# mlelarge/graph_neural_net

Measured on AMD Instinct MI355X. Metric: graph-pairs/sec FGNN fwd+bwd, N=50 regular pairs, higher is better.
Workload: dtype f32

## Files before the change

graph_neural_net_amd/_lib.py:

```python
import ctypes as C
import os

import torch

_HERE = os.path.dirname(os.path.abspath(__file__))
LIB_PATH = os.environ.get('FGNN_LIB') or os.path.join(_HERE, 'libfgnn_hip.so')

FGNN_H = 32
FGNN_TILE = 32
FGNN_MAX_DEPTH = 3
FGNN_RANGE_WG = 256
FGNN_LSAP_MAX_N = 2048
FGNN_MAX_LEVELS = 64
FGNN_QAP_MAX_N = 256
FGNN_QAPW_MAX_N = 256
FGNN_SPECTRAL_MAX_N = 256
FGNN_SPECTRAL_MAX_POWERS = 8
FGNN_PLANTED_MAX_N = 256
FGNN_SCORE_SPLIT = 4

c_float_p = C.c_void_p


class Slab(C.Structure):
    _fields_ = [('ptr', C.c_void_p), ('gstride', C.c_longlong), ('ldp', C.c_longlong), ('C', C.c_int),
                ('nrm', C.c_void_p), ('beta', C.c_void_p)]


class MlpFwdArgs(C.Structure):
    _fields_ = [('G', C.c_int), ('N', C.c_int), ('depth', C.c_int), ('nmlp', C.c_int),
                ('nvalid', C.c_void_p),
                ('a', Slab), ('b', Slab),
                ('W', (C.c_void_p * FGNN_MAX_DEPTH) * 2),
                ('bias', (C.c_void_p * FGNN_MAX_DEPTH) * 2),
                ('z', C.c_void_p * 2),
                ('ldz', C.c_longlong),
                ('part', C.c_void_p * 2),
                ('cnt', C.c_void_p), ('packed', C.c_void_p), ('xbits', C.c_void_p), ('xdeg', C.c_void_p),
                ('ranges', C.c_void_p), ('cu_share', C.c_int)]


class DwJob(C.Structure):
    _fields_ = [('dy', C.c_void_p), ('d_gstride', C.c_longlong), ('d_ld', C.c_longlong), ('relu_mask', C.c_void_p),
                ('x', C.c_void_p), ('x_gstride', C.c_longlong), ('x_ld', C.c_longlong), ('M', C.c_int), ('K', C.c_int)]


class ChainLayer(C.Structure):
    _fields_ = [('W', C.c_void_p), ('w_ostride', C.c_longlong), ('w_kstride', C.c_longlong), ('bias', C.c_void_p),
                ('M', C.c_int), ('K', C.c_int), ('relu', C.c_int), ('mask', C.c_void_p), ('out', C.c_void_p),
                ('o_gstride', C.c_longlong)]


class ChainArgs(C.Structure):
    _fields_ = [('x', C.c_void_p), ('x_gstride', C.c_longlong), ('x_ld', C.c_longlong), ('depth', C.c_int),
                ('layer', ChainLayer * 3), ('o_ld', C.c_longlong), ('nvalid', C.c_void_p), ('G', C.c_int), ('N', C.c_int)]


class Mlp64Args(C.Structure):
    _fields_ = [('x', C.c_void_p), ('x_gstride', C.c_longlong), ('x_ld', C.c_longlong), ('cin', C.c_int),
                ('xb', C.c_void_p), ('xb_gstride', C.c_longlong), ('xb_ld', C.c_longlong), ('cb', C.c_int),
                ('packed', C.c_void_p), ('nvalid', C.c_void_p), ('G', C.c_int), ('N', C.c_int),
                ('out', C.c_void_p), ('o_gstride', C.c_longlong), ('o_ld', C.c_longlong),
                ('dz', C.c_void_p), ('dz_gstride', C.c_longlong), ('dz_ld', C.c_longlong),
                ('dx', C.c_void_p), ('dx_gstride', C.c_longlong), ('dx_ld', C.c_longlong),
                ('dxb', C.c_void_p), ('dxb_gstride', C.c_longlong), ('dxb_ld', C.c_longlong),
                ('accumulate_dx', C.c_int), ('accumulate_dxb', C.c_int),
                ('wpart', C.c_void_p)]


class Mlp64PackJob(C.Structure):
    _fields_ = [('W', C.c_void_p * 3), ('bias', C.c_void_p * 3), ('cin', C.c_int), ('packed', C.c_void_p)]


class MlpBwdArgs(C.Structure):
    _fields_ = [('G', C.c_int), ('N', C.c_int), ('depth', C.c_int),
                ('nvalid', C.c_void_p),
                ('a', Slab), ('b', Slab),
                ('W', C.c_void_p * FGNN_MAX_DEPTH),
                ('bias', C.c_void_p * FGNN_MAX_DEPTH),
                ('dy', C.c_void_p), ('dgstride', C.c_longlong), ('ldd', C.c_longlong),
                ('z', C.c_void_p), ('zgstride', C.c_longlong), ('ldz', C.c_longlong),
                ('coef', C.c_void_p), ('s12', C.c_void_p), ('znrm', C.c_void_p),
                ('dxa', C.c_void_p), ('dxa_gstride', C.c_longlong), ('dxa_ld', C.c_longlong),
                ('dxb', C.c_void_p), ('dxb_gstride', C.c_longlong), ('dxb_ld', C.c_longlong),
                ('accumulate_a', C.c_int), ('accumulate_b', C.c_int),
                ('wpart', C.c_void_p), ('s12part', C.c_void_p), ('packed', C.c_void_p),
                ('s12tiles', C.c_void_p), ('s12_out', C.c_void_p), ('xbits', C.c_void_p), ('xdeg', C.c_void_p),
                ('ranges', C.c_void_p), ('cu_share', C.c_int)]


class Slab16(C.Structure):
    _fields_ = [('ptr', C.c_void_p), ('gstride', C.c_longlong), ('ldp', C.c_longlong), ('C', C.c_int),
                ('nrm', C.c_void_p), ('beta', C.c_void_p)]


class MlpFwd16Args(C.Structure):
    _fields_ = [('G', C.c_int), ('N', C.c_int), ('ldr', C.c_int), ('depth', C.c_int), ('nmlp', C.c_int),
                ('nvalid', C.c_void_p),
                ('a', Slab16), ('b', Slab16),
                ('z', C.c_void_p * 2), ('ldz', C.c_longlong),
                ('part', C.c_void_p * 2), ('cnt', C.c_void_p), ('packed', C.c_void_p), ('ranges', C.c_void_p)]


class MlpBwd16Args(C.Structure):
    _fields_ = [('G', C.c_int), ('N', C.c_int), ('ldr', C.c_int), ('depth', C.c_int),
                ('nvalid', C.c_void_p),
                ('a', Slab16), ('b', Slab16),
                ('dy', C.c_void_p), ('dgstride', C.c_longlong), ('ldd', C.c_longlong),
                ('z', C.c_void_p), ('zgstride', C.c_longlong), ('ldz', C.c_longlong),
                ('coef', C.c_void_p),
                ('dxa', C.c_void_p), ('dxa_gstride', C.c_longlong), ('dxa_ld', C.c_longlong),
                ('dxb', C.c_void_p), ('dxb_gstride', C.c_longlong), ('dxb_ld', C.c_longlong),
                ('accumulate_a', C.c_int), ('accumulate_b', C.c_int),
                ('wpart', C.c_void_p), ('s12part', C.c_void_p), ('packed', C.c_void_p), ('ranges', C.c_void_p)]


class GradJob(C.Structure):
    _fields_ = [('wpart', C.c_void_p), ('count', C.c_int), ('out', C.c_void_p), ('s12', C.c_void_p),
                ('nrm', C.c_void_p), ('dgn_w', C.c_void_p), ('dgn_b', C.c_void_p), ('rows', C.c_int), ('scale', C.c_float), ('scale_dev', C.c_void_p)]


class PackJob(C.Structure):
    _fields_ = [('kind', C.c_int), ('ca', C.c_int), ('cb', C.c_int), ('depth', C.c_int), ('nmlp', C.c_int),
                ('W', (C.c_void_p * FGNN_MAX_DEPTH) * 2), ('bias', (C.c_void_p * FGNN_MAX_DEPTH) * 2),
                ('out', C.c_void_p)]


class PairgenArgs(C.Structure):
    _fields_ = [('seed', C.c_ulonglong), ('first', C.c_longlong), ('B', C.c_int), ('N', C.c_int),
                ('family', C.c_int), ('noise_model', C.c_int), ('edge_density', C.c_double),
                ('thr_edge', C.c_ulonglong), ('thr_noise1', C.c_ulonglong), ('thr_noise2', C.c_ulonglong),
                ('thr_vertex', C.c_ulonglong), ('swaps_per_edge', C.c_int),
                ('bits1', C.c_void_p), ('bits2', C.c_void_p), ('nvalid', C.c_void_p)]


FGNN_GUARD_MAX_PARTS = 64
FGNN_GUARD_SKIP_NONFINITE = 1
FGNN_GUARD_NONFINITE = 1


class GuardRecord(C.Structure):
    _fields_ = [('max_norm', C.c_double), ('norm', C.c_double), ('coef', C.c_double),
                ('flags', C.c_int), ('skipped', C.c_int), ('arrivals', C.c_int), ('mode', C.c_int),
                ('partial', C.c_double * FGNN_GUARD_MAX_PARTS)]


class EvalRecord(C.Structure):
    _fields_ = [('ce_sum', C.c_double), ('nodes', C.c_longlong), ('correct_lsap', C.c_longlong), ('correct_max', C.c_longlong),
                ('pairs', C.c_longlong), ('steps', C.c_longlong)]


MAX_GRAD_JOBS = 16
MAX_PACK_JOBS = 24
_VP, _LL, _I, _F = C.c_void_p, C.c_longlong, C.c_int, C.c_float

_SIGNATURES = {
    'fgnn_last_error': [],
    'fgnn_version': [],
    'fgnn_tiles_per_graph': [_I],
    'fgnn_mlp_bwd_num_workgroups': [],
    'fgnn_pack_floats': [_I, _I, _I, _I, _I],
    'fgnn_pack_operands': [_VP, _I, _VP],
    'fgnn_mlp_fwd': [C.POINTER(MlpFwdArgs), _VP],
    'fgnn_pack_x3_floats': [_I, _I, _I, _I, _I],
    'fgnn_pack_x3_operands': [_VP, _I, _VP],
    'fgnn_mlp_fwd_x3': [C.POINTER(MlpFwdArgs), _VP],
    'fgnn_debug_mlp_fwd_masks': [C.POINTER(MlpFwdArgs), _VP, _VP, _VP],
    'fgnn_debug_mlp_fwd_x3_masks': [C.POINTER(MlpFwdArgs), _VP, _VP, _VP],
    'fgnn_debug_matmul_variant': [_I],
    'fgnn_gn_finalize': [_VP, _VP, _VP, _VP, _I, _I, _I, _F, _VP, _VP],
    'fgnn_gn_finalize2': [_VP, _VP, _VP, _VP, _VP, _VP, _I, _I, _I, _F, _VP, _VP, _VP],
    'fgnn_gn_plane_supported': [_I],
    'fgnn_gn_plane_fwd': [_VP, _LL, _LL, _VP, _VP, _VP, _I, _I, _I, _F, _VP, _LL, _LL, _VP, _VP],
    'fgnn_gn_plane_bwd': [_VP, _LL, _LL, _VP, _LL, _LL, _VP, _VP, _I, _I, _I, _VP, _LL, _LL, _VP, _VP, _VP, _VP],
    'fgnn_gn_stats': [_VP, _LL, _LL, _VP, _VP, _I, _I, _I, _F, _VP, _VP],
    'fgnn_gn_apply': [_VP, _LL, _LL, _VP, _VP, _VP, _I, _I, _I, _VP, _LL, _LL, _VP],
    'fgnn_ragged_tile_ranges': [_VP, _I, _I, _VP, _VP],
    'fgnn_ragged_tile_ranges_order': [_VP, _I, _I, _VP, _VP, _VP],
    'fgnn_ragged_tile_ranges16': [_VP, _I, _I, _I, _VP, _VP],
    'fgnn_conv1x1_dw_multi': [C.POINTER(DwJob), _I, _VP, _I, _I, _VP, _VP],
    'fgnn_conv_chain_supported': [_I, _I, C.POINTER(C.c_int)],
    'fgnn_conv_chain': [C.POINTER(ChainArgs), _VP],
    'fgnn_mlp64_supported': [_I, _I, _I],
    'fgnn_mlp64_num_workgroups': [],
    'fgnn_mlp64_param_count': [_I],
    'fgnn_mlp64_packed_floats': [_I],
    'fgnn_mlp64_pack': [_VP, _VP, _VP, _VP, _VP, _VP, _I, _VP, _VP],
    'fgnn_mlp64_pack_multi': [C.POINTER(Mlp64PackJob), _I, _VP],
    'fgnn_mlp64_fwd': [C.POINTER(Mlp64Args), _VP],
    'fgnn_mlp64_bwd': [C.POINTER(Mlp64Args), _VP],
    'fgnn_conv1x1': [_VP, _LL, _LL, _VP, _VP, _LL, _LL, _VP, _I, _VP, _I, _I, _I, _I, _VP, _LL, _LL, _VP],
    'fgnn_conv1x1_dw_chunks': [_I, _I],
    'fgnn_conv1x1_dw': [_VP, _LL, _LL, _VP, _VP, _LL, _LL, _VP, _I, _I, _I, _I, _VP, _VP],
    'fgnn_chan_matmul_fwd': [C.POINTER(Slab), C.POINTER(Slab), _VP, _I, _I, _VP, _LL, _LL, _VP],
    'fgnn_chan_matmul_fwd_ord': [C.POINTER(Slab), C.POINTER(Slab), _VP, _I, _I, _VP, _LL, _LL, _VP, _I, _VP],
    'fgnn_chan_matmul_fwd_fin_supported': [_I],
    'fgnn_chan_matmul_fwd_fin': [C.POINTER(Slab), C.POINTER(Slab), _VP, _VP, _VP, _VP, _VP, _F, _VP, _I, _I, _VP, _LL, _LL, _VP],
    'fgnn_chan_matmul_fwd_fin_ord': [C.POINTER(Slab), C.POINTER(Slab), _VP, _VP, _VP, _VP, _VP, _F, _VP, _I, _I, _VP, _LL, _LL, _VP, _I, _VP],
    'fgnn_colmax_fwd': [C.POINTER(Slab), _VP, _I, _I, _VP, _VP, _VP],
    'fgnn_colmax_fwd_fin_supported': [_I],
    'fgnn_colmax_fwd_fin': [C.POINTER(Slab), _VP, _VP, _VP, _F, _VP, _I, _I, _VP, _VP, _VP],
    'fgnn_score_ce_fwd': [_VP, _VP, _VP, _I, _I, _I, _VP, _VP, _VP, _VP],
    'fgnn_score_row_blocks': [_I, _I],
    'fgnn_score_ce_fwd_blocks': [_VP, _VP, _VP, _I, _I, _I, _I, _VP, _VP, _VP, _VP],
    'fgnn_score_ce_bwd': [_VP, _VP, _VP, _VP, _VP, _VP, _I, _I, _I, _VP, _VP, _VP],
    'fgnn_score_ce_fwd_blocks_labels': [_VP, _VP, _VP, _VP, _I, _I, _I, _I, _VP, _VP, _VP, _VP],
    'fgnn_score_ce_bwd_labels': [_VP, _VP, _VP, _VP, _VP, _VP, _VP, _I, _I, _I, _VP, _VP, _VP],
    'fgnn_ce_fwd_labels': [_VP, _VP, _VP, _I, _I, _VP, _VP, _VP],
    'fgnn_ce_bwd_labels': [_VP, _VP, _VP, _VP, _VP, _I, _I, _VP, _VP],
    'fgnn_inv_node_count': [_VP, _I, _VP, _VP],
    'fgnn_score_bwd': [_VP, _VP, _VP, _VP, _I, _I, _I, _VP, _VP, _VP],
    'fgnn_ce_fwd': [_VP, _VP, _I, _I, _VP, _VP, _VP],
    'fgnn_ce_bwd': [_VP, _VP, _VP, _VP, _I, _I, _VP, _VP],
    'fgnn_colmax_bwd': [_VP, _VP, _VP, _I, _I, _I, _VP, _LL, _LL, C.POINTER(Slab), _VP, _VP],
    'fgnn_gn_bwd_stats': [_VP, _LL, _LL, _VP, _LL, _LL, _VP, _VP, _I, _I, _I, _VP, _VP],
    'fgnn_gn_bwd_coef': [_VP, _VP, _VP, _I, _I, _I, _VP, _VP, _VP, _VP],
    'fgnn_gn_bwd_coef_tiles': [_VP, _VP, _VP, _I, _I, _I, _VP, _VP, _VP],
    'fgnn_grad_finalize': [_VP, _I, _I, _I, _I, _VP],
    'fgnn_gn_bwd_apply': [_VP, _LL, _LL, _VP, _LL, _LL, _VP, _VP, _I, _I, _I, _VP, _LL, _LL, _VP],
    'fgnn_mlp_bwd': [C.POINTER(MlpBwdArgs), _VP],
    'fgnn_mlp_bwd_x3': [C.POINTER(MlpBwdArgs), _VP],
    'fgnn_mlp_bwd_pair': [C.POINTER(MlpBwdArgs), C.POINTER(MlpBwdArgs), _VP],
    'fgnn_mlp_bwd_t16': [C.POINTER(MlpBwdArgs), _VP],
    'fgnn_mlp_bwd_t16_supported': [C.POINTER(MlpBwdArgs)],
    'fgnn_mlp_bwd_pair_t16': [C.POINTER(MlpBwdArgs), C.POINTER(MlpBwdArgs), _VP],
    'fgnn_mlp_bwd_pair_x3': [C.POINTER(MlpBwdArgs), C.POINTER(MlpBwdArgs), _VP],
    'fgnn_block1_struct_supported': [_I, _I, _I],
    'fgnn_block1_struct_table_floats': [_I],
    'fgnn_block1_struct_ws_floats': [_I, _I],
    'fgnn_block1_struct_rows': [_I, _I],
    'fgnn_block1_struct_fwd': [_VP, _VP, _I, _I, _VP, _VP, _VP, _VP, _VP, C.c_float, _VP, _VP, _VP, _LL, _LL, _VP, _VP, _VP, _VP, _VP, _VP, _VP],
    'fgnn_block1_struct_bwd': [_VP, _VP, _I, _I, _VP, _VP, _VP, _VP, _VP, _VP, _VP, _VP, _LL, _LL, _VP, _VP, _VP, _VP, _VP, _VP],
    'fgnn_block1_struct_fwd_pack': [_VP, _VP, _I, _I, _VP, _VP, _VP, _VP, _VP, C.c_float, _VP, _VP, _VP, _LL, _LL, _VP, _VP, _VP, _VP, _VP, _VP, _VP, _I, _VP],
    'fgnn_block1_struct_fwd16_pack': [_VP, _VP, _I, _I, _I, _VP, _VP, _VP, _VP, _VP, C.c_float, _VP, _VP, _VP, _LL, _LL, _VP, _VP, _VP, _VP, _VP, _VP, _VP, _I, _VP],
    'fgnn_block1_struct_fwd16': [_VP, _VP, _I, _I, _I, _VP, _VP, _VP, _VP, _VP, C.c_float, _VP, _VP, _VP, _LL, _LL, _VP, _VP, _VP, _VP, _VP, _VP, _VP],
    'fgnn_block1_struct_bwd16': [_VP, _VP, _I, _I, _I, _VP, _VP, _VP, _VP, _VP, _VP, _VP, _VP, _LL, _LL, _VP, _VP, _VP, _VP, _VP, _VP],
    'fgnn_mlp_bwd_coef_tiles_supported': [_I, _I],
    'fgnn_mlp_param_count': [_I, _I],
    'fgnn_reduce_partials': [_VP, _I, _I, _VP, _VP],
    'fgnn_chan_matmul_bwd': [C.POINTER(Slab), C.POINTER(Slab), _VP, _LL, _LL, _VP, _I, _I, _VP, _VP, _LL, _LL, _VP, _VP, _VP],
    'fgnn_chan_matmul_bwd_ord': [C.POINTER(Slab), C.POINTER(Slab), _VP, _LL, _LL, _VP, _I, _I, _VP, _VP, _LL, _LL, _VP, _VP, _VP, _I, _VP],
    'fgnn_sum_scale': [_VP, _I, _I, _F, _VP, _VP],
    'fgnn_adam_step': [_VP, _VP, _VP, _VP, _I, C.c_double, C.c_double, C.c_double, C.c_double, _I, C.c_double, _VP],
    'fgnn_adam_step_dev': [_VP, _VP, _VP, _VP, _I, _VP, _VP, _VP],
    'fgnn_grad_guard': [_VP, _I, _VP, _VP, _VP],
    'fgnn_adam_step_guarded': [_VP, _VP, _VP, _VP, _I, _VP, _VP, _VP, _VP],
    'fgnn_expand_adjacency': [_VP, _VP, _I, _I, _VP, _VP],
    'fgnn_pack_adjacency': [_VP, _VP, _I, _I, _VP, _VP, _VP],
    'fgnn_pack_adjacency_ld': [_VP, _VP, _I, _I, _I, _VP, _VP, _VP],
    'fgnn_pack_adjacency_pair': [_VP, _VP, _VP, _VP, _I, _I, _I, _VP, _VP, _VP, _VP, _VP],
    'fgnn_adjacency_degree': [_VP, _VP, _I, _I, _VP, _VP],
    'fgnn_accuracy_max': [_VP, _VP, _I, _I, _VP, _VP],
    'fgnn_lsap_accuracy': [_VP, _LL, _I, _VP, _I, _I, _VP, _VP, _VP],
    'fgnn_pairgen_supported': [_I, _I, _I],
    'fgnn_pairgen': [C.POINTER(PairgenArgs), _VP],
    'fgnn_pairgen_indexed': [C.POINTER(PairgenArgs), _VP, _VP],
    'fgnn_pairgen_levels': [C.POINTER(PairgenArgs), _VP, _VP, _I, _VP, _VP],
    'fgnn_epoch_index': [C.c_ulonglong, C.c_ulonglong, _LL, _LL, _LL, _VP, _VP],
    'fgnn_qap_objective': [_VP, _VP, _VP, _VP, _I, _I, _VP, _VP, _VP, _VP, _VP],
    'fgnn_qap_improve_cost': [_VP, _VP, _VP, _VP, _I, _I, _VP, _LL, _I, _VP],
    'fgnn_greedy_qap_ws_bytes': [_I, _I],
    'fgnn_greedy_qap': [_VP, _VP, _VP, _VP, _I, _I, _I, _VP, _LL, _VP, _VP, _VP, _VP, _VP],
    'fgnn_greedy_qap_labels': [_VP, _VP, _VP, _VP, _VP, _I, _I, _I, _VP, _LL, _VP, _VP, _VP, _VP, _VP],
    'fgnn_qapw_objective': [_VP, _VP, _LL, _I, _VP, _VP, _I, _I, _VP, _VP, _VP, _VP, _VP, _VP],
    'fgnn_qapw_improve_cost': [_VP, _VP, _LL, _I, _VP, _VP, _I, _I, _VP, _LL, _I, _VP],
    'fgnn_greedy_qapw_ws_bytes': [_I, _I],
    'fgnn_greedy_qapw': [_VP, _VP, _LL, _I, _VP, _VP, _I, _I, _I, _VP, _LL, _VP, _VP, _VP, _VP, _VP],
    'fgnn_greedy_qapw_labels': [_VP, _VP, _LL, _I, _VP, _VP, _VP, _I, _I, _I, _VP, _LL, _VP, _VP, _VP, _VP, _VP],
    'fgnn_planted_perm': [C.c_ulonglong, _LL, _VP, _VP, _I, _I, _VP, _VP],
    'fgnn_relabel_bits': [_VP, _VP, _VP, _I, _I, _VP, _VP],
    'fgnn_relabel_dense': [_VP, _VP, _VP, _I, _I, _I, _I, _VP, _VP],
    'fgnn_count_matches': [_VP, _VP, _VP, _I, _I, _VP, _VP],
    'fgnn_accuracy_max_labels': [_VP, _VP, _VP, _I, _I, _VP, _VP],
    'fgnn_spectral_features': [_VP, _VP, _I, _I, _I, _VP, _I, _VP],
    'fgnn_eval_pairs': [_VP, _VP, _VP, _I, _I, _VP, _LL, _I, _VP, _VP, _VP],
    'fgnn_eval_pairs_labels': [_VP, _VP, _VP, _I, _I, _VP, _LL, _I, _VP, _VP, _VP],
    'fgnn_eval_fold': [_VP, _VP, _VP, _VP, _I, _I, _I, _VP, _VP, _VP, _VP],
    'fgnn_eval_fold_bins': [_VP, _VP, _VP, _VP, _I, _I, _I, _VP, _I, _VP, _VP, _VP, _VP],
    'fgnn_tiles_per_graph16': [_I, _I],
    'fgnn_to_bf16': [_VP, _VP, _I, _I, _I, _I, _VP, _LL, _LL, _VP],
    'fgnn_from_bf16': [_VP, _LL, _LL, _I, _I, _I, _I, _VP, _VP],
    'fgnn_to_bf16_pad': [_VP, _VP, _I, _I, _I, _I, _I, _VP, _LL, _VP],
    'fgnn_pack16_floats': [_I, _I, _I, _I, _I],
    'fgnn_pack16_operands': [_VP, _I, _VP],
    'fgnn_mlp_fwd16': [C.POINTER(MlpFwd16Args), _VP],
    'fgnn_debug_mlp_fwd16_masks': [C.POINTER(MlpFwd16Args), _VP, _VP, _VP],
    'fgnn_gn_finalize_tpg': [_VP, _VP, _VP, _VP, _I, _I, _I, _I, _F, _VP, _VP],
    'fgnn_gn_finalize2_tpg': [_VP, _VP, _VP, _VP, _VP, _VP, _I, _I, _I, _I, _F, _VP, _VP, _VP],
    'fgnn_gn_bwd_coef_tiles_tpg': [_VP, _VP, _VP, _I, _I, _I, _I, _VP, _VP, _VP],
    'fgnn_chan_matmul_fwd16': [C.POINTER(Slab16), C.POINTER(Slab16), _VP, _I, _I, _I, _VP, _LL, _LL, _VP],
    'fgnn_chan_matmul_fwd16_fin': [C.POINTER(Slab16), C.POINTER(Slab16), _VP, _VP, _VP, _VP, _VP, _F, _I, _VP, _I, _I, _I, _VP, _LL,
                                   _LL, _VP],
    'fgnn_chan_matmul_bwd16': [C.POINTER(Slab16), C.POINTER(Slab16), _VP, _LL, _LL, _VP, _I, _I, _I, _VP, _VP, _LL, _LL, _VP, _VP, _VP],
    'fgnn_chan_matmul_bwd16_t': [C.POINTER(Slab16), C.POINTER(Slab16), _VP, _LL, _LL, _VP, _I, _VP, _I, _I, _I, _VP, _VP, _LL, _LL,
                                 _VP, _VP, _VP],
    'fgnn_chan_matmul_bwd16_tc': [C.POINTER(Slab16), C.POINTER(Slab16), _VP, _LL, _LL, _VP, _I, _VP, _I, _I, _I, _VP, _VP, _LL, _LL,
                                  _VP, _VP, _VP, _VP, _VP],
    'fgnn_colmax_bwd16_coef': [_VP, _VP, _VP, _I, _I, _I, _I, _VP, _LL, _LL, C.POINTER(Slab16), _VP, _VP, _VP],
    'fgnn_colmax_fwd16': [C.POINTER(Slab16), _VP, _I, _I, _I, _VP, _VP, _VP],
    'fgnn_colmax_bwd16': [_VP, _VP, _VP, _I, _I, _I, _I, _VP, _LL, _LL, C.POINTER(Slab16), _VP, _VP],
    'fgnn_mlp_bwd16': [C.POINTER(MlpBwd16Args), _VP],
    'fgnn_mlp_bwd16_pair': [C.POINTER(MlpBwd16Args), C.POINTER(MlpBwd16Args), _VP],
}
_RESTYPES = {'fgnn_last_error': C.c_char_p, 'fgnn_block1_struct_ws_floats': C.c_longlong, 'fgnn_greedy_qap_ws_bytes': C.c_longlong,
             'fgnn_greedy_qapw_ws_bytes': C.c_longlong}
EXPORTS = tuple(_SIGNATURES)

_lib = None


def load(allow_missing=False):
    global _lib
    if _lib is not None:
        return _lib
    if not os.path.exists(LIB_PATH):
        raise RuntimeError(
            'graph_neural_net_amd: %s is missing. Build it with '
            '`python -c "import __graft_entry__ as g; g.build()"` or `make -C graph_neural_net_amd/csrc`. '
            'There is no CPU fallback.' % LIB_PATH)
    lib = C.CDLL(LIB_PATH)
    for name, argtypes in _SIGNATURES.items():
        if allow_missing and not hasattr(lib, name):
            continue
        fn = getattr(lib, name)
        fn.argtypes = argtypes
        fn.restype = _RESTYPES.get(name, C.c_int)
    _lib = lib
    return lib


def last_error():
    return load().fgnn_last_error().decode('utf-8', 'replace')


PROFILE = None


def call(name, *args, tag=None):
    if PROFILE is not None:
        e0 = torch.cuda.Event(enable_timing=True)
        e1 = torch.cuda.Event(enable_timing=True)
        e0.record()
        rc = getattr(load(), name)(*args)
        e1.record()
        PROFILE.append((tag or name, e0, e1, name, args))
    else:
        rc = getattr(load(), name)(*args)
    if rc != 0:
        raise RuntimeError('%s failed (rc=%d): %s' % (name, rc, last_error()))


def relaunch(name, args):
    rc = getattr(load(), name)(*args[:-1], stream_ptr())
    if rc != 0:
        raise RuntimeError('%s failed (rc=%d): %s' % (name, rc, last_error()))


def stream_ptr():
    return C.c_void_p(torch.cuda.current_stream().cuda_stream)


def ptr(t):
    if t is None:
        return None
    if not t.is_cuda:
        raise RuntimeError('graph_neural_net_amd: expected a CUDA/HIP tensor, got device %s '
                           '(there is no CPU path)' % (t.device,))
    return C.c_void_p(t.data_ptr())


def make_slab(t, gstride, ldp, channels, nrm=None, beta=None):
    s = Slab()
    s.ptr = t.data_ptr() if t is not None else None
    s.gstride = gstride
    s.ldp = ldp
    s.C = channels
    s.nrm = nrm.data_ptr() if nrm is not None else None
    s.beta = beta.data_ptr() if beta is not None else None
    return s


def make_slab16(t, gstride, ldp, channels, nrm=None, beta=None):
    s = Slab16()
    s.ptr = t.data_ptr() if t is not None else None
    s.gstride = gstride
    s.ldp = ldp
    s.C = channels
    s.nrm = nrm.data_ptr() if nrm is not None else None
    s.beta = beta if isinstance(beta, int) else (beta.data_ptr() if beta is not None else None)
    return s


def tiles_per_graph(n):
    return (n * n + FGNN_TILE - 1) // FGNN_TILE
# ... 5 lines not shown
```

graph_neural_net_amd/csrc/fgnn_bwd32.h:

```cpp
#pragma once
#include "fgnn_common.h"

namespace {

constexpr int BWD_WG = 256;
constexpr int NW = 8;
constexpr int NP = 4;
static_assert(BWD_WG == FGNN_RANGE_WG, "fgnn_ragged_tile_ranges splits for the backward grid");

DEVI float4 coef_from_sums(const float4 n, const float2 sv, float nv) {
    const float m = nv * nv;
    float4 k;
    k.x = n.x;
    k.y = n.y;
    k.z = m > 0.f ? -n.y * sv.y * n.w / m : 0.f;
    k.w = m > 0.f ? -n.y * sv.x / m : 0.f;
    return k;
}
DEVI float4 coef_record(const fgnn_mlp_bwd_args &A, int g, int ch, int nv) {
    if (A.coef) return reinterpret_cast<const float4 *>(A.coef)[(long long)g * FGNN_H + ch];
    const float4 n = reinterpret_cast<const float4 *>(A.znrm)[(long long)g * FGNN_H + ch];
    const float2 sv = reinterpret_cast<const float2 *>(A.s12)[(long long)g * FGNN_H + ch];
    return coef_from_sums(n, sv, (float)nv);
}
DEVI float4 coef_record(const fgnn_mlp_bwd_args &A, int g, int ch) {
    if (A.coef) return reinterpret_cast<const float4 *>(A.coef)[(long long)g * FGNN_H + ch];
    const float4 n = reinterpret_cast<const float4 *>(A.znrm)[(long long)g * FGNN_H + ch];
    const float2 sv = reinterpret_cast<const float2 *>(A.s12)[(long long)g * FGNN_H + ch];
    return coef_from_sums(n, sv, (float)nvalid_of(A.nvalid, g, A.N));
}


struct PairArgs {
    fgnn_mlp_bwd_args m[2];
};

template <int PCOUNT, int NWV>
DEVI void sum_wave_partials(const float *smem, float *wpart) {
    static_assert(PCOUNT % 4 == 0, "partials are summed four at a time");
    float4 *out = reinterpret_cast<float4 *>(wpart + (long long)blockIdx.x * PCOUNT);
    const float4 *part4 = reinterpret_cast<const float4 *>(smem);
    for (int e = threadIdx.x; e < PCOUNT / 4; e += 64 * NWV) {
        float4 a = part4[e];
#pragma unroll
        for (int w = 1; w < NWV; ++w) {
            const float4 b = part4[w * (PCOUNT / 4) + e];
            a.x += b.x;
            a.y += b.y;
            a.z += b.z;
            a.w += b.w;
        }
        out[e] = a;
    }
}
template <int PCOUNT>
DEVI void sum_pair_partials(const float *smem, const PairArgs &P) {
    static_assert(PCOUNT % 4 == 0, "partials are summed four at a time");
    const float4 *part4 = reinterpret_cast<const float4 *>(smem);
    for (int e = threadIdx.x; e < 2 * (PCOUNT / 4); e += 64 * NW) {
        const int m = e >= PCOUNT / 4 ? 1 : 0, ee = e - m * (PCOUNT / 4);
        float4 a = part4[(4 * m) * (PCOUNT / 4) + ee];
#pragma unroll
        for (int w = 1; w < NP; ++w) {
            const float4 b = part4[(4 * m + w) * (PCOUNT / 4) + ee];
            a.x += b.x;
            a.y += b.y;
            a.z += b.z;
            a.w += b.w;
        }
        reinterpret_cast<float4 *>(P.m[m].wpart + (long long)blockIdx.x * PCOUNT)[ee] = a;
    }
}

inline int check_mlp_bwd_common(const fgnn_mlp_bwd_args *a, const char *fn, int tile_bits) {
    FGNN_CHECK(a->dy && a->z && a->wpart, "%s: missing dy/z/wpart", fn);
    FGNN_CHECK(a->coef || (a->s12 && a->znrm) || (a->s12tiles && a->znrm), "%s: need coef, or s12 + znrm, or s12tiles + znrm", fn);
    const long long lim = 0x7fffffffll / 4, G = a->G;
    FGNN_CHECK(G * a->a.gstride < lim && G * a->b.gstride < lim && G * a->dgstride < lim && G * a->zgstride < lim &&
               G * a->dxa_gstride < lim && G * a->dxb_gstride < lim,
               "%s: a tensor exceeds 2 GiB (32-bit buffer addressing); split the batch", fn);
    FGNN_CHECK(G * fgnn_tiles_per_graph(a->N) < (1ll << tile_bits), "%s: too many tiles", fn);
    FGNN_CHECK(BWD_WG == fgnn_mlp_bwd_num_workgroups(), "%s: workgroup count differs from fgnn_mlp_bwd", fn);
    return 0;
}
inline int check_pair_common(const fgnn_mlp_bwd_args *a1, const fgnn_mlp_bwd_args *a2, const char *fn, int tile_bits, bool dense_only) {
    FGNN_CHECK(a1 && a2, "%s: null args", fn);
    FGNN_CHECK(BWD_WG == fgnn_mlp_bwd_num_workgroups(), "%s: workgroup count differs from fgnn_mlp_bwd", fn);
    FGNN_CHECK(a1->G > 0 && a1->N > 0 && a1->G == a2->G && a1->N == a2->N && a1->depth == a2->depth,
               "%s: the two MLPs must share G, N and depth", fn);
    FGNN_CHECK((!dense_only || a1->a.ptr) && a1->a.ptr == a2->a.ptr && a1->a.C == a2->a.C && a1->a.gstride == a2->a.gstride &&
               a1->a.ldp == a2->a.ldp && a1->a.nrm == a2->a.nrm && a1->a.beta == a2->a.beta &&
               (dense_only || (a1->xbits == a2->xbits && a1->xdeg == a2->xdeg)) && a1->nvalid == a2->nvalid,
               "%s: the two MLPs must read the same input slab", fn);
    FGNN_CHECK(!a1->dxa && !a1->s12part, "%s: the input gradient and its tile sums belong to the SECOND argument block", fn);
    FGNN_CHECK(!a1->s12tiles && !a2->s12tiles, "%s: s12tiles is an mlp3 feature", fn);
    for (const fgnn_mlp_bwd_args *a : {a1, a2}) {
        FGNN_CHECK(a->dy && a->z && a->wpart, "%s: missing dy/z/wpart", fn);
        FGNN_CHECK(a->coef || (a->s12 && a->znrm), "%s: need coef, or s12 + znrm", fn);
        const long long lim = 0x7fffffffll / 4, G = a->G;
        FGNN_CHECK(G * a->a.gstride < lim && G * a->dgstride < lim && G * a->zgstride < lim && G * a->dxa_gstride < lim,
                   "%s: a tensor exceeds 2 GiB (32-bit buffer addressing); split the batch", fn);
    }
    FGNN_CHECK((long long)a1->G * fgnn_tiles_per_graph(a1->N) < (1ll << tile_bits), "%s: too many tiles", fn);
    return 0;
}

}
```

graph_neural_net_amd/csrc/fgnn_bwd_t16.h:

```cpp
#pragma once
#include "fgnn_t16.h"
#include "fgnn_pack.h"
#include "fgnn_bwd32.h"

namespace {

using namespace t16;

template <int CB, int IMAGES, int NSLOTS>
struct BwdT16Layout {
    static constexpr int DEPTH = 3;
    static constexpr PkBwd PK = pk_bwd(32, CB, DEPTH);
    static constexpr int OFF_W1 = PK.off_wh, OFF_WT1 = PK.off_wt, OFF_WT2 = PK.off_wt + 16;
    static constexpr int BIAS_F = PK.bias_f;
    static constexpr int WEIGHT_F = pk_pad_floats(PK.floats);
    static constexpr int NSLOT = NSLOTS;
    static constexpr int CIN = 32 + CB;
    static constexpr int PCOUNT = 32 * CIN + 32 + (DEPTH - 1) * (32 * 32 + 32);
    static constexpr int TILE_OFF = IMAGES * WEIGHT_F;
    static constexpr int TILE_END = TILE_OFF + NW * NSLOT * TILE_F;
    static constexpr int RED_F = NW * PCOUNT;
};


#define FGNN_T16_READ_RECORDS(norm)                                 \
    _Pragma("unroll") for (int s = 0; s < 8; ++s) {                 \
        const float4 k4 = rec[chan_s(s) + chan_q(q)];               \
        kx[s] = k4.x;                                               \
        ky[s] = k4.y;                                               \
        kz[s] = k4.z;                                               \
        kw[s] = k4.w;                                               \
        if (norm) {                                                 \
            const float4 n = rec[32 + chan_s(s) + chan_q(q)];       \
            mean[s] = n.x;                                          \
            av[s] = n.y;                                            \
        }                                                           \
    }

#define FGNN_T16_RECOMPUTE_HIDDEN(acc, h1, h2)                                              \
    _Pragma("unroll") for (int s = 0; s < 8; ++s) h1[s] = relu1(acc[s >> 2][s & 3]);        \
    stage8(S0, lane_base, h1);                                                              \
    load_bias(acc, wl + L::BIAS_F, 1, q);                                                   \
    gemm32<L::OFF_W1>(acc, wl, h1, lane);                                                   \
    _Pragma("unroll") for (int s = 0; s < 8; ++s) h2[s] = relu1(acc[s >> 2][s & 3]);        \
    stage8(S1, lane_base, h2);

#define FGNN_T16_DZ(dpre)                                                                                                   \
    _Pragma("unroll") for (int s = 0; s < 8; ++s) dpre[s] = fmaf(kz[s], zr[s] - kx[s], fmaf(ky[s], dyr[s], kw[s]));         \
    if (!full) {                                                                                                            \
        _Pragma("unroll") for (int s = 0; s < 8; ++s) dpre[s] = valid ? dpre[s] : 0.f;                                      \
    }

#define FGNN_T16_HIDDEN_BWD(OFF_WT, dpre, dW, db, Dt, In, h)                                                \
    {                                                                                                       \
        f32x4 a2[2];                                                                                        \
        a2[0] = a2[1] = zero4();                                                                            \
        gemm32<OFF_WT>(a2, wl, dpre, lane);                                                                 \
        wgrad16(dW, db, Dt, In, lane);                                                                      \
        _Pragma("unroll") for (int s = 0; s < 8; ++s) dpre[s] = h[s] > 0.f ? a2[s >> 2][s & 3] : 0.f;       \
    }

#define FGNN_T16_DB_BUTTERFLY(db0, db1, db2)            \
    _Pragma("unroll") for (int b = 0; b < 2; ++b) {     \
        db0[b] += __shfl_xor(db0[b], 16);               \
        db0[b] += __shfl_xor(db0[b], 32);               \
        db1[b] += __shfl_xor(db1[b], 16);               \
        db1[b] += __shfl_xor(db1[b], 32);               \
        db2[b] += __shfl_xor(db2[b], 16);               \
        db2[b] += __shfl_xor(db2[b], 32);               \
    }

}
```

graph_neural_net_amd/csrc/fgnn_norm.h:

```cpp
#pragma once
#include "fgnn_common.h"

DEVI float4 nrm_record(float mean, float m2, float m, float nv, float w, float eps) {
    const float var = m > 0.f ? m2 / m : 0.f;
    const float ve = var + eps;
    const float q = nv > 0.f ? 1.f / (2.f * sqrtf(nv * ve)) : 0.f;
    float4 o;
    o.x = mean;
    o.y = w * q;
    o.z = q;
    o.w = 1.f / ve;
    return o;
}

struct TilePartials {
    float nb[4], mb[4], qb[4];
};
DEVI TilePartials finalize_load(const float *part, const float *cnt, int g, int c, int C, int tpg, int lane, bool tr = false) {
    TilePartials p;
    const int ts = tr ? 1 : C, cs = tr ? tpg : 1;
#pragma unroll
    for (int k = 0; k < 4; ++k) {
        const int t = lane + WAVE * k;
        const bool ok = t < tpg;
        const int tc = ok ? t : 0;
        const float n = cnt[(long long)g * tpg + tc];
        const float2 pm = reinterpret_cast<const float2 *>(part)[(long long)g * tpg * C + (long long)tc * ts + (long long)c * cs];
        p.nb[k] = ok ? n : 0.f;
        p.mb[k] = pm.x;
        p.qb[k] = ok ? pm.y : 0.f;
    }
    return p;
}
DEVI float4 finalize_reduce(const TilePartials &p, float nv, float w, float eps) {
    float sn = 0.f, sm = 0.f;
#pragma unroll
    for (int k = 0; k < 4; ++k) {
        sn += p.nb[k];
        sm += p.nb[k] * p.mb[k];
    }
    sn = wave_sum(sn);
    sm = wave_sum(sm);
    const float mean = sn > 0.f ? sm / sn : 0.f;
    float m2 = 0.f;
#pragma unroll
    for (int k = 0; k < 4; ++k) {
        const float d = p.mb[k] - mean;
        m2 += p.qb[k] + p.nb[k] * d * d;
    }
    m2 = wave_sum(m2);
    return nrm_record(mean, m2, sn, nv, w, eps);
}

struct NormRec {
    float mean, a, beta;
    bool on;
};
DEVI NormRec norm_of(const fgnn_slab &s, int g, int c) {
    NormRec r;
    r.on = s.nrm != nullptr;
    if (r.on) {
        const float4 n = reinterpret_cast<const float4 *>(s.nrm)[(long long)g * s.C + c];
        r.mean = n.x;
        r.a = n.y;
        r.beta = s.beta ? s.beta[c] : 0.f;
    } else {
        r.mean = 0.f;
        r.a = 1.f;
        r.beta = 0.f;
    }
    return r;
}
DEVI NormRec norm_from(const float4 &n, const fgnn_slab &s, int c) {
    NormRec r;
    r.on = true;
    r.mean = n.x;
    r.a = n.y;
    r.beta = s.beta ? s.beta[c] : 0.f;
    return r;
}

DEVI float4 finalize_wave(const float *part, const float *cnt, int g, int c, int C, int tpg, float nv, float w, float eps,
                          int lane, bool tr = false) {
    return finalize_reduce(finalize_load(part, cnt, g, c, C, tpg, lane, tr), nv, w, eps);
}
DEVI float4 finalize_wave_any(const float *part, const float *cnt, int g, int c, int C, int tpg, float nv, float w, float eps, int lane,
                              bool tr = false) {
    if (tpg <= 4 * WAVE) return finalize_wave(part, cnt, g, c, C, tpg, nv, w, eps, lane, tr);
    constexpr int U = 8;
    float sn = 0.f, sm = 0.f;
    const float *cg = cnt + (long long)g * tpg;
    const int ts = tr ? 1 : C;
    const float2 *pg = reinterpret_cast<const float2 *>(part) + (long long)g * tpg * C + (long long)c * (tr ? tpg : 1);
    for (int t0 = lane; t0 < tpg; t0 += U * WAVE) {
        float n[U], x[U];
#pragma unroll
        for (int k = 0; k < U; ++k) {
            const int t = t0 + k * WAVE, tc = t < tpg ? t : 0;
            n[k] = t < tpg ? cg[tc] : 0.f;
            x[k] = pg[(long long)tc * ts].x;
        }
#pragma unroll
        for (int k = 0; k < U; ++k) {
            sn += n[k];
            sm += n[k] * x[k];
        }
    }
    sn = wave_sum(sn);
    sm = wave_sum(sm);
    const float mean = sn > 0.f ? sm / sn : 0.f;
    float m2 = 0.f;
    for (int t0 = lane; t0 < tpg; t0 += U * WAVE) {
        float n[U];
        float2 pm[U];
#pragma unroll
        for (int k = 0; k < U; ++k) {
            const int t = t0 + k * WAVE, tc = t < tpg ? t : 0;
            n[k] = t < tpg ? cg[tc] : 0.f;
            pm[k] = pg[(long long)tc * ts];
            if (t >= tpg) pm[k].y = 0.f;
        }
#pragma unroll
        for (int k = 0; k < U; ++k) {
            const float d = pm[k].x - mean;
            m2 += pm[k].y + n[k] * d * d;
        }
    }
    m2 = wave_sum(m2);
    return nrm_record(mean, m2, sn, nv, w, eps);
}
```

graph_neural_net_amd/csrc/matmul.hip:

```cpp
#include "fgnn_common.h"
#include "fgnn_norm.h"

namespace {

constexpr int TM = 64;
constexpr int LDS_LD = 65;

DEVI void stage_tile(float *lds, const float *mat, int N, int nv, int row0, int col0, const NormRec &nr, int tid) {
    if (row0 == 0 && col0 == 0 && N <= TM) {
        for (int e = tid; e < TM * TM; e += 256) lds[(e >> 6) * LDS_LD + (e & 63)] = 0.f;
        __syncthreads();
        const int P = N * N;
        for (int e = tid; e < P; e += 256) {
            const int r = e / N, c = e - r * N;
            float v = mat[e];
            const bool ok = r < nv && c < nv;
            v = ok ? (nr.on ? (v - nr.mean) * nr.a + nr.beta : v) : 0.f;
            lds[r * LDS_LD + c] = v;
        }
    } else {
        for (int e = tid; e < TM * TM; e += 256) {
            const int r = e >> 6, c = e & 63;
            const int gr = row0 + r, gc = col0 + c;
            float v = 0.f;
// ... 50 lines not shown
    const int qi = wave >> 1, qj = wave & 1;
    const int j = lane & 31, h = lane >> 5;
    const float *A = ya.ptr + (long long)g * ya.gstride + (long long)c * ya.ldp;
    const float *B = yb.ptr + (long long)g * yb.gstride + (long long)c * yb.ldp;
    const NormRec na = norm_of(ya, g, c), nb = norm_of(yb, g, c);
    float *O = out + (long long)g * ogstride + (long long)c * ldo;

    f32x16 acc;
#pragma unroll
    for (int r = 0; r < 16; ++r) acc[r] = 0.f;
    const bool live = (row0 + 32 * qi < N) && (col0 + 32 * qj < N);

    for (int k0 = 0; k0 < N; k0 += TM) {
        if (k0) __syncthreads();
        stage_tile(As, A, N, nv, row0, k0, na, tid);
        stage_tile(Bs, B, N, nv, k0, col0, nb, tid);
        __syncthreads();
        if (live) {
            const int kmax = (N - k0 < TM ? N - k0 : TM);
            const float *ap = As + (32 * qi + j) * LDS_LD + h;
            const float *bp = Bs + h * LDS_LD + 32 * qj + j;
            for (int k = 0; k < kmax; k += 2) acc = mfma32(ap[k], bp[k * LDS_LD], acc);
        }
    }
    if (live) store_quadrant(O, N, row0 + 32 * qi, col0 + 32 * qj, acc, lane);
}

__global__ __launch_bounds__(256) void chan_matmul_bwd_kernel(const fgnn_slab ya, const fgnn_slab yb,
                                                              const float *dm, long long dmg, long long ldm,
                                                              const int *nvalid, int N, float *da, float *db,
                                                              long long ogstride, long long ldo, float *s12a,
                                                              float *s12b) {
    __shared__ float Xs[TM * LDS_LD];
    __shared__ float Ds[TM * LDS_LD];
    __shared__ float red[4][4];
    const int C = ya.C;
    const int gc = blockIdx.z;
    const int g = gc / C, c = gc - g * C;
    const int nv = nvalid_of(nvalid, g, N);
    const int row0 = blockIdx.y * TM, col0 = blockIdx.x * TM;
    const int tid = threadIdx.x, lane = tid & 63, wave = tid >> 6;
    const int qi = wave >> 1, qj = wave & 1;
    const int j = lane & 31, h = lane >> 5;
    const float *A = ya.ptr + (long long)g * ya.gstride + (long long)c * ya.ldp;
    const float *B = yb.ptr + (long long)g * yb.gstride + (long long)c * yb.ldp;
    const float *D = dm + (long long)g * dmg + (long long)c * ldm;
    const NormRec na = norm_of(ya, g, c), nb = norm_of(yb, g, c);
    NormRec none;
    none.on = false; none.mean = 0.f; none.a = 1.f; none.beta = 0.f;
    float *OA = da + (long long)g * ogstride + (long long)c * ldo;
    float *OB = db + (long long)g * ogstride + (long long)c * ldo;
    const bool live = (row0 + 32 * qi < N) && (col0 + 32 * qj < N);

    f32x16 acc;
#pragma unroll
    for (int r = 0; r < 16; ++r) acc[r] = 0.f;
    for (int j0 = 0; j0 < N; j0 += TM) {
        if (j0) __syncthreads();
        stage_tile(Ds, D, N, nv, row0, j0, none, tid);
        stage_tile(Xs, B, N, nv, col0, j0, nb, tid);
        __syncthreads();
        if (live) {
            const int kmax = (N - j0 < TM ? N - j0 : TM);
            const float *ap = Ds + (32 * qi + j) * LDS_LD + h;
            const float *bp = Xs + (32 * qj + j) * LDS_LD + h;
            for (int k = 0; k < kmax; k += 2) acc = mfma32(ap[k], bp[k], acc);
        }
    }
    if (live) store_quadrant(OA, N, row0 + 32 * qi, col0 + 32 * qj, acc, lane);
    float sa1 = 0.f, sa2 = 0.f, sb1 = 0.f, sb2 = 0.f;
    if (s12a && live) {
        const int col = col0 + 32 * qj + j;
#pragma unroll
        for (int r = 0; r < 16; ++r) {
            const int row = row0 + 32 * qi + ch_of(r, h);
            if (row < nv && col < nv) {
                sa1 += acc[r];
                sa2 += acc[r] * (A[(long long)row * N + col] - na.mean);
            }
        }
    }

#pragma unroll
    for (int r = 0; r < 16; ++r) acc[r] = 0.f;
    for (int i0 = 0; i0 < N; i0 += TM) {
        __syncthreads();
        stage_tile(Xs, A, N, nv, i0, row0, na, tid);
        stage_tile(Ds, D, N, nv, i0, col0, none, tid);
        __syncthreads();
        if (live) {
            const int kmax = (N - i0 < TM ? N - i0 : TM);
            const float *ap = Xs + h * LDS_LD + 32 * qi + j;
            const float *bp = Ds + h * LDS_LD + 32 * qj + j;
            for (int k = 0; k < kmax; k += 2) acc = mfma32(ap[k * LDS_LD], bp[k * LDS_LD], acc);
        }
    }
    if (live) store_quadrant(OB, N, row0 + 32 * qi, col0 + 32 * qj, acc, lane);
    if (s12a) {
        if (live) {
            const int col = col0 + 32 * qj + j;
#pragma unroll
            for (int r = 0; r < 16; ++r) {
                const int row = row0 + 32 * qi + ch_of(r, h);
                if (row < nv && col < nv) {
                    sb1 += acc[r];
                    sb2 += acc[r] * (B[(long long)row * N + col] - nb.mean);
                }
            }
        }
        s12_epilogue(red, sa1, sa2, sb1, sb2, s12a, s12b, gc, tid);
    }
}

template <bool WANT_U>
DEVI void load_tile_regs(float (&v)[16], float (&u)[16], const float *mat, int N, int nv, const NormRec &nr, int tid) {
#pragma unroll
    for (int k = 0; k < 16; ++k) {
        const int e = tid + 256 * k;
        const int r = e >> 6, c = e & 63;
        const bool ok = r < nv && c < nv;
        const float x = mat[ok ? r * N + c : 0];
        const float d = x - nr.mean;
        v[k] = ok ? (nr.on ? d * nr.a + nr.beta : x) : 0.f;
        if (WANT_U) u[k] = ok ? d : 0.f;
    }
}
DEVI void store_tile_lds(float *lds, const float (&v)[16], int tid) {
#pragma unroll
    for (int k = 0; k < 16; ++k) {
        const int e = tid + 256 * k;
        lds[(e >> 6) * LDS_LD + (e & 63)] = v[k];
    }
}
DEVI void frag_to_lds(float *lds, int row0, int col0, const f32x16 &acc, int lane) {
    const int j = lane & 31, h = lane >> 5;
#pragma unroll
    for (int r = 0; r < 16; ++r) lds[(row0 + ch_of(r, h)) * LDS_LD + col0 + j] = acc[r];
}
template <bool WANT_S>
DEVI void tile_to_global(const View &ov, int mat_off4, const float *lds, int N, const float (&u)[16], float &s1,
                         float &s2, int tid) {
    const int c = tid & 63, r0 = __builtin_amdgcn_readfirstlane(tid >> 6);
    const int voff = c < N ? (r0 * N + c) * 4 : OOB_OFF;
    const float *lp = lds + r0 * LDS_LD + c;
#pragma unroll
    for (int k = 0; k < 16; ++k) {
        const float t = lp[4 * k * LDS_LD];
        buf_store(t, ov, r0 + 4 * k < N ? voff : OOB_OFF, mat_off4 + k * 16 * N);
        if (WANT_S) {
            s1 += t;
            s2 += t * u[k];
        }
    }
}

DEVI void load_tile_raw(float (&x)[16], const View &v, int mat_off4, int N, int nv, int tid) {
    const int c = tid & 63, r0 = __builtin_amdgcn_readfirstlane(tid >> 6);
    const int voff = c < nv ? (r0 * N + c) * 4 : OOB_OFF;
#pragma unroll
    for (int k = 0; k < 16; ++k) {
        const int r = r0 + 4 * k;
        x[k] = buf_load(v, r < nv ? voff : OOB_OFF, mat_off4 + k * 16 * N);
    }
}
template <bool WANT_U>
DEVI void finish_tile(float (&v)[16], float (&u)[16], const float (&x)[16], int nv, const NormRec &nr, int tid) {
#pragma unroll
    for (int k = 0; k < 16; ++k) {
        const int e = tid + 256 * k;
        const int r = e >> 6, c = e & 63;
        const bool ok = r < nv && c < nv;
        const float d = x[k] - nr.mean;
        v[k] = ok ? (nr.on ? d * nr.a + nr.beta : x[k]) : 0.f;
        if (WANT_U) u[k] = ok ? d : 0.f;
    }
}

struct FinArgs {
    const float *part_a, *part_b, *cnt, *gw_a, *gw_b;
    float *nrm_a, *nrm_b;
    float eps;
    int tpg;
};
template <bool FIN>
__global__ __launch_bounds__(256, 4) void chan_matmul_fwd1_kernel(const fgnn_slab ya, const fgnn_slab yb,
                                                               const int *nvalid, int N, int M, float *out,
                                                               long long ogstride, long long ldo, const FinArgs F) {
    __shared__ float As[TM * LDS_LD];
    __shared__ float Bs[TM * LDS_LD];
    __shared__ float4 fin_rec[2];
    const int C = ya.C;
    const int tid = threadIdx.x, lane = tid & 63, wave = tid >> 6;
    const int qi = wave >> 1, qj = wave & 1;
    const int j = lane & 31, h = lane >> 5;
    float xa[16], xb[16], dummy[16];
    const int G = M / C;
    const View vA = make_view(ya.ptr, ya.gstride, ya.ldp, G), vB = make_view(yb.ptr, yb.gstride, yb.ldp, G);
    const View vO = make_view(out, ogstride, ldo, G);
    const int gc = blockIdx.x;
    {
        const int g = gc / C, c = gc - g * C;
        const int nv = nvalid_of(nvalid, g, N);
        TilePartials tp;
        if (FIN && wave < 2) tp = finalize_load(wave ? F.part_b : F.part_a, F.cnt, g, c, C, F.tpg, lane);
        load_tile_raw(xa, vA, g * vA.gs4 + c * vA.ld4, N, nv, tid);
        load_tile_raw(xb, vB, g * vB.gs4 + c * vB.ld4, N, nv, tid);
        NormRec na, nb;
        if (FIN) {
            if (wave < 2) {
                const float4 r = finalize_reduce(tp, (float)nv, (wave ? F.gw_b : F.gw_a) ? (wave ? F.gw_b : F.gw_a)[c] : 1.f, F.eps);
                if (lane == 0) {
                    fin_rec[wave] = r;
                    reinterpret_cast<float4 *>(wave ? F.nrm_b : F.nrm_a)[gc] = r;
                }
            }
            __syncthreads();
            const float4 ra = fin_rec[0], rb = fin_rec[1];
            na = norm_from(ra, ya, c);
            nb = norm_from(rb, yb, c);
        } else {
            na = norm_of(ya, g, c);
            nb = norm_of(yb, g, c);
        }
        const int o_off = g * vO.gs4 + c * vO.ld4;
        {
            float va[16], vb[16];
            finish_tile<false>(va, dummy, xa, nv, na, tid);
            finish_tile<false>(vb, dummy, xb, nv, nb, tid);
            store_tile_lds(As, va, tid);
            store_tile_lds(Bs, vb, tid);
        }
        __syncthreads();
        f32x16 acc;
#pragma unroll
        for (int r = 0; r < 16; ++r) acc[r] = 0.f;
        if (32 * qi < N && 32 * qj < N) {
            const float *ap = As + (32 * qi + j) * LDS_LD + h;
            const float *bp = Bs + h * LDS_LD + 32 * qj + j;
            for (int k = 0; k < N; k += 2) acc = mfma32(ap[k], bp[k * LDS_LD], acc);
        }
        __syncthreads();
        frag_to_lds(As, 32 * qi, 32 * qj, acc, lane);
        __syncthreads();
        float s1 = 0.f, s2 = 0.f;
        tile_to_global<false>(vO, o_off, As, N, dummy, s1, s2, tid);
    }
}

__global__ __launch_bounds__(256, 4) void chan_matmul_bwd1_kernel(const fgnn_slab ya, const fgnn_slab yb,
                                                               const float *dm, long long dmg, long long ldm,
                                                               const int *nvalid, int N, int M, float *da, float *db,
                                                               long long ogstride, long long ldo, float *s12a,
                                                               float *s12b) {
    __shared__ float Bs[TM * LDS_LD];
    __shared__ float Ds[TM * LDS_LD];
    __shared__ float red[4][4];
    const int C = ya.C;
    const int tid = threadIdx.x, lane = tid & 63, wave = tid >> 6;
    const int qi = wave >> 1, qj = wave & 1;
    const int j = lane & 31, h = lane >> 5;
    NormRec none;
    none.on = false; none.mean = 0.f; none.a = 1.f; none.beta = 0.f;
    float xa[16], xb[16], xd[16], dummy[16];
    const int G = M / C;
    const View vA = make_view(ya.ptr, ya.gstride, ya.ldp, G), vB = make_view(yb.ptr, yb.gstride, yb.ldp, G);
    const View vD = make_view(dm, dmg, ldm, G);
    const View vOA = make_view(da, ogstride, ldo, G), vOB = make_view(db, ogstride, ldo, G);
    const int gc = blockIdx.x;
    {
        const int g = gc / C, c = gc - g * C;
        const int nv = nvalid_of(nvalid, g, N);
        load_tile_raw(xa, vA, g * vA.gs4 + c * vA.ld4, N, nv, tid);
        load_tile_raw(xb, vB, g * vB.gs4 + c * vB.ld4, N, nv, tid);
        load_tile_raw(xd, vD, g * vD.gs4 + c * vD.ld4, N, nv, tid);
        const NormRec na = norm_of(ya, g, c), nb = norm_of(yb, g, c);
        const int o_off = g * vOA.gs4 + c * vOA.ld4;
        float ua[16], ub[16], va[16];
        finish_tile<true>(va, ua, xa, nv, na, tid);
        {
            float vb[16], vd[16];
            finish_tile<true>(vb, ub, xb, nv, nb, tid);
            finish_tile<false>(vd, dummy, xd, nv, none, tid);
            store_tile_lds(Bs, vb, tid);
            store_tile_lds(Ds, vd, tid);
        }
        __syncthreads();
        const bool live = 32 * qi < N && 32 * qj < N;
        f32x16 accA, accB;
#pragma unroll
        for (int r = 0; r < 16; ++r) {
            accA[r] = 0.f;
            accB[r] = 0.f;
        }
        if (live) {
            const float *ap = Ds + (32 * qi + j) * LDS_LD + h;
            const float *bp = Bs + (32 * qj + j) * LDS_LD + h;
            for (int k = 0; k < N; k += 2) accA = mfma32(ap[k], bp[k], accA);
        }
        __syncthreads();
        store_tile_lds(Bs, va, tid);
        __syncthreads();
        if (live) {
            const float *ap = Bs + h * LDS_LD + 32 * qi + j;
            const float *bp = Ds + h * LDS_LD + 32 * qj + j;
            for (int k = 0; k < N; k += 2) accB = mfma32(ap[k * LDS_LD], bp[k * LDS_LD], accB);
        }
        __syncthreads();
        frag_to_lds(Ds, 32 * qi, 32 * qj, accA, lane);
        frag_to_lds(Bs, 32 * qi, 32 * qj, accB, lane);
        __syncthreads();
        float sa1 = 0.f, sa2 = 0.f, sb1 = 0.f, sb2 = 0.f;
        if (s12a) {
            tile_to_global<true>(vOA, o_off, Ds, N, ua, sa1, sa2, tid);
            tile_to_global<true>(vOB, o_off, Bs, N, ub, sb1, sb2, tid);
            s12_epilogue(red, sa1, sa2, sb1, sb2, s12a, s12b, gc, tid);
        } else {
            tile_to_global<false>(vOA, o_off, Ds, N, dummy, sa1, sa2, tid);
            tile_to_global<false>(vOB, o_off, Bs, N, dummy, sb1, sb2, tid);
        }
    }
}


int g_mm_wave_variant = 1;
inline bool mm_wave_variant() { return (g_mm_wave_variant & 1) != 0; }
inline bool mm_narrow() { return (g_mm_wave_variant & 8) != 0; }
constexpr int WLD = 68;
constexpr int W_WAVES = 2;

DEVI rsrc_t mat_rsrc(const float *p, int bytes) {
    return __builtin_amdgcn_make_buffer_rsrc(const_cast<float *>(p), 0, bytes, 0x00020000);
}
DEVI float rsrc_load(rsrc_t r, int voff, int soff) {
    return __builtin_bit_cast(float, __builtin_amdgcn_raw_buffer_load_b32(r, voff, soff, 0));
}
DEVI void rsrc_store(float x, rsrc_t r, int voff, int soff) {
    __builtin_amdgcn_raw_buffer_store_b32(__builtin_bit_cast(unsigned, x), r, voff, soff, 0);
}
DEVI float2 rsrc_load2(rsrc_t r, int voff, int soff) {
    typedef unsigned u2 __attribute__((ext_vector_type(2)));
    const u2 v = __builtin_amdgcn_raw_buffer_load_b64(r, voff, soff, 0);
    const unsigned a = v.x, b = v.y;
    return make_float2(__builtin_bit_cast(float, a), __builtin_bit_cast(float, b));
}
DEVI void rsrc_store2(float x, float y, rsrc_t r, int voff, int soff) {
    typedef unsigned u2 __attribute__((ext_vector_type(2)));
    u2 v;
    v.x = __builtin_bit_cast(unsigned, x);
    v.y = __builtin_bit_cast(unsigned, y);
    __builtin_amdgcn_raw_buffer_store_b64(v, r, voff, soff, 0);
}

#define FGNN_W_CONTEXT(LDS_FLOATS)                                                                                       \
    __shared__ __attribute__((aligned(16))) float lds[W_WAVES * (LDS_FLOATS)];                                           \
    const int lane = threadIdx.x & 63, wv = __builtin_amdgcn_readfirstlane(threadIdx.x >> 6);                            \
    const int gc = xcd_swizzle(blockIdx.x, gridDim.x) * W_WAVES + wv;                                                    \
    if (gc >= M) return;                                                                                                 \
    const int C = ya.C;                                                                                                  \
    const int g = gc / C, c = gc - g * C;                                                                                \
    const int nv = __builtin_amdgcn_readfirstlane(nvalid_of(nvalid, g, N));                                              \
    const int j = lane & 31, h = lane >> 5;                                                                              \
    float *As = lds + wv * (LDS_FLOATS);                                                                                 \
    const rsrc_t rA = mat_rsrc(ya.ptr + (long long)g * ya.gstride + (long long)c * ya.ldp, nv * N * 4);                  \
    const rsrc_t rB = mat_rsrc(yb.ptr + (long long)g * yb.gstride + (long long)c * yb.ldp, nv * N * 4);                  \
    const rsrc_t rO = mat_rsrc(out + (long long)g * ogstride + (long long)c * ldo, N * N * 4);
#define FGNN_W_PRODUCTS(NB_, BVAL)                                                                                       \
    f32x16 acc[NB_][NB_];                                                                                                \
    _Pragma("unroll") for (int rb = 0; rb < NB_; ++rb)                                                                   \
        _Pragma("unroll") for (int cb = 0; cb < NB_; ++cb)                                                               \
            _Pragma("unroll") for (int r = 0; r < 16; ++r) acc[rb][cb][r] = 0.f;                                         \
    _Pragma("unroll") for (int q = 0; q < KQ; ++q) {                                                                     \
        float4 af[NB_];                                                                                                  \
        _Pragma("unroll") for (int rb = 0; rb < NB_; ++rb)                                                               \
            af[rb] = *reinterpret_cast<const float4 *>(As + (32 * rb + j) * WLD + h * 32 + 4 * q);                       \
        _Pragma("unroll") for (int t = 0; t < 4; ++t) {                                                                  \
            const int s = 4 * q + t;                                                                                     \
            if (q == KQ - 1 && 2 * s >= N) break;                                                                        \
            float bv[NB_];                                                                                               \
            BVAL                                                                                                         \
            _Pragma("unroll") for (int rb = 0; rb < NB_; ++rb) {                                                         \
                const float a = t == 0 ? af[rb].x : (t == 1 ? af[rb].y : (t == 2 ? af[rb].z : af[rb].w));               \
                _Pragma("unroll") for (int cb = 0; cb < NB_; ++cb) acc[rb][cb] = mfma32(a, bv[cb], acc[rb][cb]);         \
            }                                                                                                            \
        }                                                                                                                \
    }
#define FGNN_W_RECORDS                                                                                                   \
    float meanA, aA, meanB, aB;                                                                                          \
    if (FIN) {                                                                                                           \
        const float4 ra = finalize_reduce(ta, (float)nv, F.gw_a ? F.gw_a[c] : 1.f, F.eps);                               \
        const float4 rb = finalize_reduce(tb, (float)nv, F.gw_b ? F.gw_b[c] : 1.f, F.eps);                               \
        if (lane == 0) {                                                                                                 \
            reinterpret_cast<float4 *>(F.nrm_a)[gc] = ra;                                                                \
            reinterpret_cast<float4 *>(F.nrm_b)[gc] = rb;                                                                \
        }                                                                                                                \
        meanA = ra.x; aA = ra.y; meanB = rb.x; aB = rb.y;                                                                \
    } else {                                                                                                             \
        const NormRec na = norm_of(ya, g, c), nb = norm_of(yb, g, c);                                                    \
        meanA = na.mean; aA = na.a; meanB = nb.mean; aB = nb.a;                                                          \
    }                                                                                                                    \
    const bool onA = FIN || ya.nrm != nullptr, onB = FIN || yb.nrm != nullptr;                                           \
    const float betaA = (onA && ya.beta) ? ya.beta[c] : 0.f, betaB = (onB && yb.beta) ? yb.beta[c] : 0.f;
DEVI constexpr int wave_row_off(int rb, int r, int N) { return (32 * rb + (r & 3) + 8 * (r >> 2)) * N * 4; }

template <int KQ>
DEVI void wave_rows_load(float (&x)[8 * KQ], rsrc_t r, int N, int voff) {
#pragma unroll
    for (int i = 0; i < 8 * KQ; ++i) x[i] = rsrc_load(r, voff, i < N ? i * N * 4 : 0);
}
template <int KQ>
DEVI void wave_rows_stage(float *T, const float (&x)[8 * KQ], float mean, float a_eff, float b_eff, int nv, int N, int lane) {
    if (nv < N) {
#pragma unroll
        for (int i = 0; i < 8 * KQ; ++i) {
            const float v = (x[i] - mean) * a_eff + b_eff;
            T[i * WLD + lane] = i < nv ? v : 0.f;
        }
    } else {
#pragma unroll
        for (int i = 0; i < 8 * KQ; ++i) T[i * WLD + lane] = (x[i] - mean) * a_eff + b_eff;
    }
}

template <int KQ, bool FIN>
__global__ __launch_bounds__(64 * W_WAVES, 2) void chan_matmul_fwd_w_kernel(const fgnn_slab ya, const fgnn_slab yb,
                                                                           const int *nvalid, int N, int M, float *out,
                                                                           long long ogstride, long long ldo,
                                                                           const FinArgs F) {
    constexpr int KH = 4 * KQ;
    constexpr bool TWO = KQ > 4;
    constexpr int NB = TWO ? 2 : 1;
    FGNN_W_CONTEXT(32 * NB * WLD)

    TilePartials ta, tb;
    if (FIN) {
        ta = finalize_load(F.part_a, F.cnt, g, c, C, F.tpg, lane);
        tb = finalize_load(F.part_b, F.cnt, g, c, C, F.tpg, lane);
    }
    float xa[8 * KQ], xb[NB][KH];
    wave_rows_load<KQ>(xa, rA, N, lane < nv ? lane * 4 : OOB_OFF);
    int voffB[NB];
#pragma unroll
    for (int cb = 0; cb < NB; ++cb) {
        const int col = 32 * cb + j;
        voffB[cb] = col < nv ? (h * N + col) * 4 : OOB_OFF;
    }
#pragma unroll
    for (int s = 0; s < KH; ++s)
#pragma unroll
        for (int cb = 0; cb < NB; ++cb) xb[cb][s] = rsrc_load(rB, voffB[cb] + s * 2 * N * 4, 0);
    FGNN_W_RECORDS
    {
        const bool okc = lane < nv;
        wave_rows_stage<KQ>(As, xa, meanA, okc ? aA : 0.f, okc ? betaA : 0.f, nv, N, (lane & 1) * 32 + (lane >> 1));
    }
    float aeB[NB], beB[NB];
#pragma unroll
    for (int cb = 0; cb < NB; ++cb) {
        const bool okc = 32 * cb + j < nv;
        aeB[cb] = okc ? aB : 0.f;
        beB[cb] = okc ? betaB : 0.f;
    }
    FGNN_W_PRODUCTS(NB, _Pragma("unroll") for (int cb = 0; cb < NB; ++cb) bv[cb] = (xb[cb][s] - meanB) * aeB[cb] + beB[cb];)
#pragma unroll
    for (int cb = 0; cb < NB; ++cb) {
        const int col = 32 * cb + j;
// ... 378 lines not shown
    const BigSrc D = big_src_plain(dm, dmg, ldm, G, g, c);
    const View vOA = make_view(da, ogstride, ldo, G), vOB = make_view(db, ogstride, ldo, G);
    const int o_off = g * vOA.gs4 + c * vOA.ld4;
    if (do_a) big_zero_fill(vOA, o_off, N, nv, 32 * ntv, tid, fill != 0);
    if (do_b) big_zero_fill(vOB, o_off, N, nv, 32 * ntv, tid, fill != 0);
    float sa1 = 0.f, sa2 = 0.f, sb1 = 0.f, sb2 = 0.f;
    if (ntv > 0) {
        f32x16 acc[BigCfg<NT>::MAXT];
        if (do_a) {
            big_gemm<NT, true, true>(acc, D, B, big_lds, N, nv, ntv, tid);
            if (s12a) big_store<NT, true>(acc, vOA, o_off, A, N, nv, ntv, sa1, sa2, tid);
            else big_store<NT, false>(acc, vOA, o_off, A, N, nv, ntv, sa1, sa2, tid);
        }
        if (do_b) {
            big_gemm<NT, false, false>(acc, A, D, big_lds, N, nv, ntv, tid);
            if (s12a) big_store<NT, true>(acc, vOB, o_off, B, N, nv, ntv, sb1, sb2, tid);
            else big_store<NT, false>(acc, vOB, o_off, B, N, nv, ntv, sb1, sb2, tid);
        }
    }
    if (s12a) {
        sa1 = wave_sum(sa1);
        sa2 = wave_sum(sa2);
        sb1 = wave_sum(sb1);
        sb2 = wave_sum(sb2);
        if (lane == 0) {
            red[wv][0] = sa1;
            red[wv][1] = sa2;
            red[wv][2] = sb1;
            red[wv][3] = sb2;
        }
        __syncthreads();
        if (tid < 4 && (tid < 2 ? do_a : do_b)) {
            float v = 0.f;
#pragma unroll
            for (int w = 0; w < BIG_NW; ++w) v += red[w][tid];
            float *dst = (tid < 2 ? s12a : s12b) + (long long)gc * 2 + (tid & 1);
            *dst = v;
        }
    }
}

inline bool big_path(int N) { return N > TM && N <= 256; }

}

template <int MT, bool FIN>
static void launch_fwd_big(const fgnn_slab *ya, const fgnn_slab *yb, const int *nvalid, int N, int G, float *out, long long ogstride,
                           long long ldo, const int *order, const FinArgs &F, int fill, hipStream_t st) {
    static LdsAttrCache attr_cache;
    (void)fgnn_raise_lds(attr_cache, (const void *)chan_matmul_fwd_big_kernel<MT, FIN>, BigCfg<MT>::LDS_BYTES);
    hipLaunchKernelGGL((chan_matmul_fwd_big_kernel<MT, FIN>), dim3(G * ya->C), dim3(BIG_THREADS), BigCfg<MT>::LDS_BYTES, st, *ya, *yb, nvalid, N, G, out,
                       ogstride, ldo, order, F, fill);
}

static int check_2gib(const char *name, int G, long long s0, long long s1, long long s2 = 0, long long s3 = 0) {
    FGNN_CHECK((long long)G * s0 < 0x7fffffffll / 4 && (long long)G * s1 < 0x7fffffffll / 4 && (long long)G * s2 < 0x7fffffffll / 4 &&
               (long long)G * s3 < 0x7fffffffll / 4,
               "%s: a tensor exceeds 2 GiB (32-bit buffer addressing); split the batch", name);
    return 0;
}

template <bool FIN>
static int chan_matmul_fwd_dispatch(const char *name, const fgnn_slab *ya, const fgnn_slab *yb, const int *nvalid, int G, int N,
                                    float *out, long long ogstride, long long ldo, const int *order, int fill, const FinArgs &F,
                                    hipStream_t st) {
    const int M = G * ya->C;
    if (FIN || big_path(N)) {
        if (check_2gib(name, G, ya->gstride, yb->gstride, ogstride)) return 1;
    } else if (N <= TM) {
        if (check_2gib(name, G, ya->gstride, yb->gstride)) return 1;
        FGNN_CHECK((long long)G * ogstride < 0x7fffffffll / 4, "%s: output exceeds 2 GiB", name);
    }
    if (N <= TM) {
        if (mm_wave_variant()) launch_fwd_w<FIN>(ya, yb, nvalid, N, M, out, ogstride, ldo, F, st);
        else hipLaunchKernelGGL(chan_matmul_fwd1_kernel<FIN>, dim3(M), dim3(256), 0, st, *ya, *yb, nvalid, N, M, out, ogstride, ldo, F);
    } else if (big_path(N)) {
        if (N <= 128) launch_fwd_big<4, FIN>(ya, yb, nvalid, N, G, out, ogstride, ldo, order, F, fill, st);
        else launch_fwd_big<8, FIN>(ya, yb, nvalid, N, G, out, ogstride, ldo, order, F, fill, st);
    } else if constexpr (!FIN) {
        const int t = (N + TM - 1) / TM;
        hipLaunchKernelGGL(chan_matmul_fwd_kernel, dim3(t, t, M), dim3(256), 0, st, *ya, *yb, nvalid, N, out, ogstride, ldo);
    }
    FGNN_LAUNCH_CHECK();
    return 0;
}

extern "C" int fgnn_chan_matmul_fwd(const fgnn_slab *ya, const fgnn_slab *yb, const int *nvalid, int G, int N,
                                    float *out, long long ogstride, long long ldo, void *stream) {
    return fgnn_chan_matmul_fwd_ord(ya, yb, nvalid, G, N, out, ogstride, ldo, nullptr, 0, stream);
}

extern "C" int fgnn_chan_matmul_fwd_ord(const fgnn_slab *ya, const fgnn_slab *yb, const int *nvalid, int G, int N,
                                        float *out, long long ogstride, long long ldo, const int *order, int fill, void *stream) {
    FGNN_CHECK(!order || nvalid, "fgnn_chan_matmul_fwd_ord: an order needs the nvalid it was derived from");
    FGNN_CHECK(ya && yb && out && ya->ptr && yb->ptr, "fgnn_chan_matmul_fwd: null argument");
    FGNN_CHECK(ya->C == yb->C && ya->C > 0 && G > 0 && N > 0, "fgnn_chan_matmul_fwd: bad shapes");
    FGNN_CHECK((long long)G * ya->C <= 65535 * 1024ll, "fgnn_chan_matmul_fwd: G*C too large");
    return chan_matmul_fwd_dispatch<false>("fgnn_chan_matmul_fwd", ya, yb, nvalid, G, N, out, ogstride, ldo, order, fill, FinArgs{},
                                           (hipStream_t)stream);
}

extern "C" int fgnn_chan_matmul_fwd_fin_supported(int N) { return (N <= TM || big_path(N)) ? 1 : 0; }

extern "C" int fgnn_debug_matmul_variant(int wave_per_matrix) {
    FGNN_CHECK((wave_per_matrix & ~9) == 0, "fgnn_debug_matmul_variant: bits 0 and 3 only (got %d)", wave_per_matrix);
    g_mm_wave_variant = wave_per_matrix;
    return 0;
}

extern "C" int fgnn_chan_matmul_fwd_fin(const fgnn_slab *ya, const fgnn_slab *yb, const float *part_a, const float *part_b,
                                        const float *cnt, const float *gn_weight_a, const float *gn_weight_b, float eps,
                                        const int *nvalid, int G, int N, float *out, long long ogstride, long long ldo,
                                        void *stream) {
    return fgnn_chan_matmul_fwd_fin_ord(ya, yb, part_a, part_b, cnt, gn_weight_a, gn_weight_b, eps, nvalid, G, N, out, ogstride, ldo, nullptr, 0, stream);
}

extern "C" int fgnn_chan_matmul_fwd_fin_ord(const fgnn_slab *ya, const fgnn_slab *yb, const float *part_a, const float *part_b,
                                            const float *cnt, const float *gn_weight_a, const float *gn_weight_b, float eps,
                                            const int *nvalid, int G, int N, float *out, long long ogstride, long long ldo,
                                            const int *order, int fill, void *stream) {
    FGNN_CHECK(!order || nvalid, "fgnn_chan_matmul_fwd_fin_ord: an order needs the nvalid it was derived from");
    FGNN_CHECK(ya && yb && out && ya->ptr && yb->ptr && part_a && part_b && cnt, "fgnn_chan_matmul_fwd_fin: null argument");
    FGNN_CHECK(ya->nrm && yb->nrm, "fgnn_chan_matmul_fwd_fin: the slabs must carry the record buffers to fill");
    FGNN_CHECK(ya->C == yb->C && ya->C > 0 && G > 0 && N > 0, "fgnn_chan_matmul_fwd_fin: bad shapes");
    FGNN_CHECK(N <= TM || big_path(N), "fgnn_chan_matmul_fwd_fin: N=%d > 256 (use fgnn_gn_finalize2 + fgnn_chan_matmul_fwd)", N);
    const FinArgs F = {part_a, part_b, cnt, gn_weight_a, gn_weight_b, const_cast<float *>(ya->nrm), const_cast<float *>(yb->nrm), eps,
                       fgnn_tiles_per_graph(N)};
    return chan_matmul_fwd_dispatch<true>("fgnn_chan_matmul_fwd_fin", ya, yb, nvalid, G, N, out, ogstride, ldo, order, fill, F,
                                          (hipStream_t)stream);
}

extern "C" int fgnn_chan_matmul_bwd(const fgnn_slab *ya, const fgnn_slab *yb, const float *dm, long long dmgstride,
                                    long long ldm, const int *nvalid, int G, int N, float *da, float *db,
                                    long long ogstride, long long ldo, float *s12a, float *s12b, void *stream) {
    return fgnn_chan_matmul_bwd_ord(ya, yb, dm, dmgstride, ldm, nvalid, G, N, da, db, ogstride, ldo, s12a, s12b, nullptr,
                                    0, stream);
}

extern "C" int fgnn_chan_matmul_bwd_ord(const fgnn_slab *ya, const fgnn_slab *yb, const float *dm, long long dmgstride,
                                        long long ldm, const int *nvalid, int G, int N, float *da, float *db,
                                        long long ogstride, long long ldo, float *s12a, float *s12b, const int *order,
                                        int fill, void *stream) {
    FGNN_CHECK(!order || nvalid, "fgnn_chan_matmul_bwd_ord: an order needs the nvalid it was derived from");
    FGNN_CHECK(ya && yb && dm && da && db && ya->ptr && yb->ptr, "fgnn_chan_matmul_bwd: null argument");
    FGNN_CHECK(ya->C == yb->C && ya->C > 0 && G > 0 && N > 0, "fgnn_chan_matmul_bwd: bad shapes");
    FGNN_CHECK((s12a == nullptr) == (s12b == nullptr), "fgnn_chan_matmul_bwd: s12a and s12b come together");
    FGNN_CHECK(!s12a || (ya->nrm && yb->nrm), "fgnn_chan_matmul_bwd: s12 outputs need normalised slabs");
    const int t = (N + TM - 1) / TM;
    const bool fused = s12a && t == 1;
    if (t == 1) {
        if (check_2gib("fgnn_chan_matmul_bwd", G, ya->gstride, yb->gstride, dmgstride)) return 1;
        FGNN_CHECK((long long)G * ogstride < 0x7fffffffll / 4, "fgnn_chan_matmul_bwd: output exceeds 2 GiB");
        const int M = G * ya->C;
        hipLaunchKernelGGL(chan_matmul_bwd1_kernel, dim3(M), dim3(256), 0, (hipStream_t)stream, *ya, *yb, dm,
                           dmgstride, ldm, nvalid, N, M, da, db, ogstride, ldo, s12a, s12b);
        FGNN_LAUNCH_CHECK();
        return 0;
    }
    if (big_path(N)) {
        if (check_2gib("fgnn_chan_matmul_bwd", G, ya->gstride, yb->gstride, dmgstride, ogstride)) return 1;
#define FGNN_BIG_BWD(MT)                                                                                              \
    {                                                                                                                 \
        static LdsAttrCache attr_cache;                                                                           \
        (void)fgnn_raise_lds(attr_cache, (const void *)chan_matmul_bwd_big_kernel<MT>, BigCfg<MT>::LDS_BYTES);                   \
        hipLaunchKernelGGL(chan_matmul_bwd_big_kernel<MT>, dim3(G * ya->C * (split ? 2 : 1)), dim3(BIG_THREADS),      \
                           BigCfg<MT>::LDS_BYTES, (hipStream_t)stream, *ya, *yb, dm, dmgstride, ldm, nvalid, N, G, da, \
                           db, ogstride, ldo, s12a, s12b, order, split, fill);                                            \
    }
        const int split = (order && (long long)G * ya->C <= BIG_SPLIT_MAX_MATRICES) ? 1 : 0;
        if (N <= 128) FGNN_BIG_BWD(4)
        else FGNN_BIG_BWD(8)
#undef FGNN_BIG_BWD
        FGNN_LAUNCH_CHECK();
        return 0;
    }
    hipLaunchKernelGGL(chan_matmul_bwd_kernel, dim3(t, t, G * ya->C), dim3(256), 0, (hipStream_t)stream, *ya, *yb, dm,
                       dmgstride, ldm, nvalid, N, da, db, ogstride, ldo, fused ? s12a : nullptr, fused ? s12b : nullptr);
    FGNN_LAUNCH_CHECK();
    if (s12a && !fused) {
        int rc = fgnn_gn_bwd_stats(da, ogstride, ldo, ya->ptr, ya->gstride, ya->ldp, ya->nrm, nvalid, G, ya->C, N, s12a, stream);
        if (rc) return rc;
        rc = fgnn_gn_bwd_stats(db, ogstride, ldo, yb->ptr, yb->gstride, yb->ldp, yb->nrm, nvalid, G, yb->C, N, s12b, stream);
        if (rc) return rc;
    }
    return 0;
}
```

graph_neural_net_amd/csrc/mlp_bwd.hip:

```cpp
#include "fgnn_tile.h"
#include "fgnn_pack.h"
#include "fgnn_bwd32.h"

#ifdef FGNN_PHASES
__device__ unsigned long long *g_phase_buf = nullptr;
__device__ int g_phase_sel = 0;
#define PH_DECL unsigned long long ph_[16] = {0, 0, 0, 0, 0, 0, 0, 0, 0, 0, 0, 0, 0, 0, 0, 0}; unsigned long long ph_last_ = __builtin_amdgcn_s_memtime();
#define PH(k) { const unsigned long long t_ = __builtin_amdgcn_s_memtime(); ph_[k] += t_ - ph_last_; ph_last_ = t_; }
#define PH_FLUSH if (g_phase_buf && g_phase_sel == CA * 100 + CB && (threadIdx.x & 63) == 0) { for (int k_ = 0; k_ < 16; ++k_) g_phase_buf[((long long)blockIdx.x * NW + wv) * 16 + k_] = ph_[k_]; }
#else
#define PH_DECL
#define PH(k) __builtin_amdgcn_sched_barrier(0);
#define PH_FLUSH
#endif

namespace {

template <int CA, int CB, int DEPTH>
struct BwdLayout {
    static constexpr int SA = CA / 2, SB = CB / 2;
    static constexpr int pad4(int x) { return (x + 3) & ~3; }
    static constexpr PkBwd PK = pk_bwd(CA, CB, DEPTH);
    static constexpr int OFF_W1A = PK.off_w1a;
    static constexpr int OFF_W1B = PK.off_w1b;
// ... 395 lines not shown
                        if (h == 0) {
                            float2 o;
                            o.x = s1;
                            o.y = s2;
                            reinterpret_cast<float2 *>(A.s12part)[((long long)c.g * tpg + c.tt) * FGNN_H + j] = o;
                        }
                    }
                }
            }
            if constexpr (CB > 0) {
                if (A.dxb) {
                    const int voff = lane_off<4>(vdxb, c, h);
                    const int s0 = c.g * vdxb.gs4;
                    float vb2[16];
#pragma unroll
                    for (int r = 0; r < 16; ++r) vb2[r] = dxb_acc[r];
                    if (A.accumulate_b) {
#pragma unroll
                        for (int r = 0; r < 16; ++r)
                            vb2[r] += buf_load(vdxb, ch_of(r, h) < CB ? voff : OOB_OFF, s0 + ((r & 3) + 8 * (r >> 2)) * vdxb.ld4);
                    }
#pragma unroll
                    for (int r = 0; r < 16; ++r)
                        buf_store(vb2[r], vdxb, ch_of(r, h) < CB ? voff : OOB_OFF, s0 + ((r & 3) + 8 * (r >> 2)) * vdxb.ld4);
                }
            }
            if constexpr (CA == 32 && CB == 0) {
#pragma unroll
                for (int s = 0; s < SA; ++s) xa[s] = nxa[s];
            }
            PH(8)
        }
    }

    if constexpr (SKIP) {
        if (emit) {
            for (int t = T0 + wv; t < T1; t += NW) {
                const TileCtx c = decode_tile(t, true, tpg, A.N, P, j);
                if (tile_live(c.tt, A.N, A.nvalid[c.g])) continue;
                if (h == 0)
                    reinterpret_cast<float2 *>(A.s12part)[((long long)c.g * tpg + c.tt) * FGNN_H + j] = make_float2(0.f, 0.f);
            }
        }
    }

    constexpr int PCOUNT = L::PCOUNT;
#pragma unroll
    for (int l = 0; l < DEPTH; ++l) db[l] += __shfl_xor(db[l], 32);
    if constexpr (VW0) {
#pragma unroll
        for (int r = 0; r < 32; ++r) w0v[r] = half_sum(w0v[r]);
#pragma unroll
        for (int r = 0; r < 16; ++r) b0v[r] = half_sum(b0v[r]);
    }
    auto put_partials = [&](float *red) {
#pragma unroll
        for (int r = 0; r < 16; ++r) {
            const int o = ch_of(r, h);
            if constexpr (VW0) {
                if (j == 0) {
                    red[o * CIN] = w0v[2 * r];
                    red[o * CIN + 1] = w0v[2 * r + 1];
                    red[32 * CIN + o] = b0v[r];
                }
            } else {
                if (j < CA) red[o * CIN + j] = dW0a[r];
                if (CB > 0 && j < CB) red[o * CIN + CA + j] = dW0b[r];
            }
        }
        int off = 32 * CIN;
#pragma unroll
        for (int l = 0; l < DEPTH; ++l) {
            if (l > 0) {
#pragma unroll
                for (int r = 0; r < 16; ++r) red[off + ch_of(r, h) * 32 + j] = dWh[l - 1][r];
                off += 1024;
            }
            if (h == 0 && !(VW0 && l == 0)) red[off + j] = db[l];
            off += 32;
        }
    };
    __syncthreads();
    PH(10)
    put_partials(smem + wv * PCOUNT);
    __syncthreads();
    sum_wave_partials<PCOUNT, NW>(smem, A.wpart);
    PH(11)
    PH_FLUSH
}

template <int CA, int CB, int DEPTH, bool PK = false, bool SKIP = false>
int launch_bwd_impl(const fgnn_mlp_bwd_args *a, int tpg, int total, hipStream_t st) {
    constexpr int LDS = BwdLayout<CA, CB, DEPTH>::LDS_F * 4;
    static_assert(LDS <= 160 * 1024, "LDS budget");
    static LdsAttrCache attr_cache;
    (void)fgnn_raise_lds(attr_cache, (const void *)mlp_bwd_kernel<CA, CB, DEPTH, PK, SKIP>, LDS);
    hipLaunchKernelGGL((mlp_bwd_kernel<CA, CB, DEPTH, PK, SKIP>), dim3(a->cu_share == 2 && !SKIP ? BWD_WG / 2 : BWD_WG), dim3(64 * NW), LDS, st,
                       *a, tpg, total);
    FGNN_LAUNCH_CHECK();
    return 0;
}
template <int CA, int CB, int DEPTH, bool PK = false>
int launch_bwd(const fgnn_mlp_bwd_args *a, int tpg, int total, hipStream_t st) {
    if (a->ranges) return launch_bwd_impl<CA, CB, DEPTH, PK, true>(a, tpg, total, st);
    return launch_bwd_impl<CA, CB, DEPTH, PK, false>(a, tpg, total, st);
}

template <int DEPTH>
int dispatch_c(const fgnn_mlp_bwd_args *a, int tpg, int total, hipStream_t st) {
    const int ca = a->a.C, cb = a->b.C;
    if (a->xbits) {
        if constexpr (DEPTH == 3) {
            if (ca == 2 && cb == 0) return launch_bwd<2, 0, DEPTH, true>(a, tpg, total, st);
            if (ca == 32 && cb == 2) return launch_bwd<32, 2, DEPTH, true>(a, tpg, total, st);
        }
        fgnn_set_error("fgnn_mlp_bwd: xbits needs depth 3 and a 2-channel slab (2 or 32+2 input channels), got depth %d, %d + %d",
                       DEPTH, ca, cb);
        return 1;
    }
#define FGNN_CASE(A_, B_) \
    if (ca == A_ && cb == B_) return launch_bwd<A_, B_, DEPTH>(a, tpg, total, st);
    FGNN_CASE(2, 0)
    FGNN_CASE(16, 0)
    FGNN_CASE(32, 0)
    FGNN_CASE(32, 2)
    FGNN_CASE(32, 32)
#undef FGNN_CASE
    fgnn_set_error("fgnn_mlp_bwd: unsupported input channels (%d + %d); built for 2, 16, 32, 32+2, 32+32", ca, cb);
    return 1;
}

}

#ifdef FGNN_PHASES
extern "C" int fgnn_debug_phase_buffer(void *p, int ca, int cb) {
    const int sel = ca * 100 + cb;
    if (hipMemcpyToSymbol(HIP_SYMBOL(g_phase_sel), &sel, sizeof(sel)) != hipSuccess) return 1;
    return hipMemcpyToSymbol(HIP_SYMBOL(g_phase_buf), &p, sizeof(p)) == hipSuccess ? 0 : 1;
}
#endif

extern "C" int fgnn_mlp_bwd_num_workgroups(void) { return BWD_WG; }

extern "C" int fgnn_mlp_bwd_coef_tiles_supported(int G, int N) {
    const long long tpg = fgnn_tiles_per_graph(N), total = (long long)G * tpg;
    const long long per_wg = (total + BWD_WG - 1) / BWD_WG;
    return (per_wg + tpg - 2) / tpg + 1 <= FGNN_BWD_COEF_GRAPHS ? 1 : 0;
}

extern "C" int fgnn_mlp_param_count(int Cin, int depth) { return 32 * Cin + 32 + (depth - 1) * (32 * 32 + 32); }

extern "C" int fgnn_mlp_bwd(const fgnn_mlp_bwd_args *a, void *stream) {
    FGNN_CHECK(a != nullptr, "fgnn_mlp_bwd: null args");
    FGNN_CHECK(a->G > 0 && a->N > 0, "fgnn_mlp_bwd: bad G=%d N=%d", a->G, a->N);
    FGNN_CHECK(a->depth >= 1 && a->depth <= FGNN_MAX_DEPTH, "fgnn_mlp_bwd: depth %d not in 1..%d", a->depth, FGNN_MAX_DEPTH);
    const bool pk_a = a->xbits && a->a.C == 2, pk_b = a->xbits && a->b.C == 2;
    FGNN_CHECK((a->a.ptr || pk_a) && a->a.C > 0, "fgnn_mlp_bwd: slab a missing");
    FGNN_CHECK(a->b.C == 0 || a->b.ptr || pk_b, "fgnn_mlp_bwd: slab b has channels but no pointer");
    FGNN_CHECK(!a->xbits || a->xdeg, "fgnn_mlp_bwd: xbits without xdeg (fgnn_adjacency_degree)");
    FGNN_CHECK(!(pk_a && a->dxa) && !(pk_b && a->dxb), "fgnn_mlp_bwd: no gradient with respect to the packed adjacency");
    if (check_mlp_bwd_common(a, "fgnn_mlp_bwd", 30)) return 1;
    for (int l = 0; l < a->depth; ++l) FGNN_CHECK(a->W[l] && a->bias[l], "fgnn_mlp_bwd: missing weights layer %d", l);
    const int tpg = fgnn_tiles_per_graph(a->N);
    const long long total = (long long)a->G * tpg;
    FGNN_CHECK(!a->ranges || (a->nvalid && !a->s12tiles), "fgnn_mlp_bwd: ranges need nvalid and exclude s12tiles");
    FGNN_CHECK(!a->s12tiles || a->b.C > 0, "fgnn_mlp_bwd: s12tiles is built into the two-slab kernels only; use fgnn_gn_bwd_coef_tiles");
    FGNN_CHECK(!a->s12tiles || fgnn_mlp_bwd_coef_tiles_supported(a->G, a->N),
               "fgnn_mlp_bwd: s12tiles needs a workgroup's tile range to span <= %d graphs (G=%d N=%d); "
               "use fgnn_gn_bwd_coef_tiles", FGNN_BWD_COEF_GRAPHS, a->G, a->N);
    hipStream_t st = (hipStream_t)stream;
    if (a->depth == 1) return dispatch_c<1>(a, tpg, (int)total, st);
    if (a->depth == 2) return dispatch_c<2>(a, tpg, (int)total, st);
    return dispatch_c<3>(a, tpg, (int)total, st);
}
```

graph_neural_net_amd/csrc/mlp_bwd_pair_t16.hip:

```cpp
#include "fgnn_bwd_t16.h"

#ifdef FGNN_PHASES
__device__ unsigned long long *g_phase16_buf = nullptr;
#define PH_DECL unsigned long long ph_[16] = {0, 0, 0, 0, 0, 0, 0, 0, 0, 0, 0, 0, 0, 0, 0, 0}; unsigned long long ph_last_ = __builtin_amdgcn_s_memtime();
#define PH(k) { const unsigned long long t_ = __builtin_amdgcn_s_memtime(); ph_[k] += t_ - ph_last_; ph_last_ = t_; }
#define PH_FLUSH if (g_phase16_buf && (threadIdx.x & 63) == 0) { for (int k_ = 0; k_ < 16; ++k_) g_phase16_buf[((long long)blockIdx.x * NW + wv) * 16 + k_] = ph_[k_]; }
#else
#define PH_DECL
#define PH(k)
#define PH_FLUSH
#endif

namespace {

struct PairLayout16 : BwdT16Layout<0, 2, 4> {
    static constexpr int OFF_W0 = PK.off_w1a, OFF_WT0 = PK.off_wt0a;
    static constexpr int XCH_OFF = TILE_END;
    static constexpr int FLAG_OFF = XCH_OFF + NP * 1024;
    static constexpr int REC_OFF = FLAG_OFF + 4 * NP;
    static constexpr int LIVE_OFF = REC_OFF + NW * 256;
    static constexpr int MAIN_F = LIVE_OFF + LIVE_LIST_CAP + NW;
    static constexpr int LDS_F = MAIN_F > RED_F ? MAIN_F : RED_F;
};

template <bool SKIP, bool HAS_DX>
__global__ __launch_bounds__(64 * NW, 2) void mlp_bwd_pair_t16_kernel(const PairArgs P, const int tpg, const int total_tiles) {
    extern __shared__ __attribute__((aligned(16))) float smem[];
    using L = PairLayout16;
    const int lane = threadIdx.x & 63, wv = __builtin_amdgcn_readfirstlane(threadIdx.x >> 6);
    const int role = wv >> 2, pair = wv & 3;
    const int px = lane & 15, q = lane >> 4;
    const fgnn_mlp_bwd_args &A = P.m[role];
    const int P2 = A.N * A.N;
    const View va = make_view(A.a.ptr, A.a.gstride, A.a.ldp, A.G);
    const View vdy = make_view(A.dy, A.dgstride, A.ldd, A.G);
    const View vz = make_view(A.z, A.zgstride, A.ldz, A.G);
    const View vdx = make_view(P.m[1].dxa, P.m[1].dxa_gstride, P.m[1].dxa_ld, P.m[1].G);

    PH_DECL
    if (role == 1) __builtin_amdgcn_s_setprio(1);
    float *wl = smem + role * L::WEIGHT_F;
    float *my = smem + L::TILE_OFF + wv * (L::NSLOT * TILE_F);
    float *XA = my, *S0 = my + TILE_F, *S1 = my + 2 * TILE_F, *S2 = my + 3 * TILE_F;
    float *XCH = smem + L::XCH_OFF + pair * 1024;
    int *flags = reinterpret_cast<int *>(smem + L::FLAG_OFF) + 4 * pair;
    const int lane_base = tile_lane_base(px, q);

    f32x4 dW0[4], dW1[4], dW2[4];
    float db0[2] = {0.f, 0.f}, db1[2] = {0.f, 0.f}, db2[2] = {0.f, 0.f};
#pragma unroll
    for (int k = 0; k < 4; ++k) dW0[k] = dW1[k] = dW2[k] = zero4();

    int T0, T1;
    wg_tile_range<SKIP>(A.ranges, total_tiles, T0, T1);
    const bool normA = A.a.nrm != nullptr;
    constexpr bool has_dx = HAS_DX;
    const bool emit = role == 1 && normA && has_dx && P.m[1].s12part != nullptr;
    const bool rmw = has_dx && P.m[1].accumulate_a;
    const bool ragged = A.nvalid != nullptr;
    const rsrc_t rnv = __builtin_amdgcn_make_buffer_rsrc(const_cast<int *>(A.nvalid), 0, ragged ? A.G * 4 : 0, 0x00020000);
    const float rcpN = 1.f / (float)A.N;

    PH(14)
    pk_glds<NW>(smem, P.m[0].packed, L::WEIGHT_F, wv, lane);
    pk_glds<NW>(smem + L::WEIGHT_F, P.m[1].packed, L::WEIGHT_F, wv, lane);
    PH(15)

    float mean[8], av[8], beta[8], kx[8], ky[8], kz[8], kw[8];
#pragma unroll
    for (int s = 0; s < 8; ++s) {
        mean[s] = 0.f;
        av[s] = 1.f;
        beta[s] = normA && A.a.beta ? A.a.beta[chan(s, 0) + chan_q(q)] : 0.f;
        kx[s] = ky[s] = kz[s] = kw[s] = 0.f;
    }
    float4 *rec = reinterpret_cast<float4 *>(smem + L::REC_OFF) + wv * 64;
    auto fetch_records = [&](int g, int nv) {
        if (lane < 32) {
            rec[lane] = coef_record(A, g, lane, nv);
            if (normA) rec[32 + lane] = reinterpret_cast<const float4 *>(A.a.nrm)[(long long)g * A.a.C + lane];
        }
    };
    auto read_records = [&]() { FGNN_T16_READ_RECORDS(normA) };

    float xa[8], dyr[8], zr[8], oldr[8];
#pragma unroll
    for (int s = 0; s < 8; ++s) oldr[s] = 0.f;
    int cached_g = -1, cur_nv = A.N;
    int tile = T0 + pair;
    int live_cnt = 0;
    if constexpr (SKIP) tile = __builtin_amdgcn_readfirstlane(next_owned_live_tile_p(T0, T1, live_cnt, pair, NP, tpg, FGNN_TILE, A.N, A.nvalid));
    int hf = 0;
    {
        const bool act = tile < T1;
        const int g = __builtin_amdgcn_readfirstlane(act ? tile / tpg : 0);
        const int p = (act ? tile - g * tpg : 0) * 32 + px;
        const bool inb0 = act && p < P2;
        load8(xa, va, lane_voff(va, q, p, inb0), g * va.gs4);
        if (act) {
            cur_nv = graph_nv(rnv, ragged, g, A.N);
            fetch_records(g, cur_nv);
            cached_g = g;
        }
    }
    PH(12)
    if (threadIdx.x < 4 * NP) reinterpret_cast<int *>(smem + L::FLAG_OFF)[threadIdx.x] = 0;
    PH(13)
    int *live_list = reinterpret_cast<int *>(smem + L::LIVE_OFF);
    int nlive = 0, li = pair;
    if constexpr (SKIP) nlive = build_live_list(live_list, live_list + LIVE_LIST_CAP, T0, T1, tpg, FGNN_TILE, A.N, A.nvalid, threadIdx.x, 64 * NW);
    const bool use_list = SKIP && nlive <= LIVE_LIST_CAP;
    __syncthreads();
    {
        const bool act = tile < T1;
        const int g = __builtin_amdgcn_readfirstlane(act ? tile / tpg : 0);
        const int p = (act ? tile - g * tpg : 0) * 32 + px;
        const bool inb0 = act && p < P2;
        load8(dyr, vdy, lane_voff(vdy, q, p, inb0), g * vdy.gs4);
        load8(zr, vz, lane_voff(vz, q, p, inb0), g * vz.gs4);
        if (has_dx) load8(oldr, vdx, lane_voff(vdx, q, p, inb0 && rmw && role == 0), g * vdx.gs4);
    }
    if (cached_g >= 0) read_records();
    PH(9)

    int hk = 0;
    float es1[8], es2[8];
#pragma unroll
    for (int s = 0; s < 8; ++s) es1[s] = es2[s] = 0.f;
    while (tile < T1) {
        int tnext = tile + NP;
        if constexpr (SKIP) {
            if (hf == 1) {
                if (use_list) {
                    li += NP;
                    tnext = __builtin_amdgcn_readfirstlane(li < nlive ? live_list[li] : T1);
                } else {
                    tnext = __builtin_amdgcn_readfirstlane(next_owned_live_tile_p(tile + 1, T1, live_cnt, pair, NP, tpg, FGNN_TILE, A.N, A.nvalid));
                }
            }
        }
        const int g = __builtin_amdgcn_readfirstlane(tile / tpg), tt = tile - g * tpg;
        const int p = tt * 32 + 16 * hf + px;
        const bool inb = p < P2;
        if (g != cached_g) {
            cur_nv = graph_nv(rnv, ragged, g, A.N);
            fetch_records(g, cur_nv);
            read_records();
            cached_g = g;
        }
        bool valid = inb;
        if (ragged) {
            int i, jj;
            row_col(p, A.N, rcpN, i, jj);
            valid = inb && i < cur_nv && jj < cur_nv;
        }
        const unsigned long long vmask = __ballot(valid);
        const bool full = vmask == ~0ull;

        const int ntile = hf == 0 ? tile : tnext, nhf = hf ^ 1;
        int np, ng;
        bool ninb;
        {
            const bool act = ntile < T1;
            ng = __builtin_amdgcn_readfirstlane(act ? ntile / tpg : 0);
            np = (act ? ntile - ng * tpg : 0) * 32 + 16 * nhf + px;
            ninb = act && np < P2;
        }

        {
            f32x4 dx[2];
            const int dvoff = lane_voff(vdx, q, p, inb), ds0 = g * vdx.gs4;

            float h1[8], h2[8], u[8];
            {
                float ya[8];
#pragma unroll
                for (int s = 0; s < 8; ++s) {
                    u[s] = xa[s] - mean[s];
                    ya[s] = u[s] * av[s] + beta[s];
                }
                stage8(XA, lane_base, ya);
                f32x4 acc[2];
                load_bias(acc, wl + L::BIAS_F, 0, q);
                gemm32<L::OFF_W0>(acc, wl, ya, lane);
                FGNN_T16_RECOMPUTE_HIDDEN(acc, h1, h2)
            }
            PH(1)
            float dpre[8];
            FGNN_T16_DZ(dpre)
            stage8(S2, lane_base, dpre);
            load8(dyr, vdy, lane_voff(vdy, q, np, ninb), ng * vdy.gs4);
            load8(zr, vz, lane_voff(vz, q, np, ninb), ng * vz.gs4);
            PH(2)
            __builtin_amdgcn_sched_barrier(0);
            FGNN_T16_HIDDEN_BWD(L::OFF_WT2, dpre, dW2, db2, S2, S1, h2)
            PH(3)
            __builtin_amdgcn_sched_barrier(0);
            stage8(S1, lane_base, dpre);
            FGNN_T16_HIDDEN_BWD(L::OFF_WT1, dpre, dW1, db1, S1, S0, h1)
            PH(4)
            __builtin_amdgcn_sched_barrier(0);
            stage8(S2, lane_base, dpre);
            __builtin_amdgcn_sched_barrier(0);
#pragma unroll
            for (int s = 0; s < 8; ++s) dx[s >> 2][s & 3] = oldr[s];
            load8(xa, va, lane_voff(va, q, np, ninb), ng * va.gs4);
            if (has_dx) load8(oldr, vdx, lane_voff(vdx, q, np, ninb && rmw && role == 0), ng * vdx.gs4);
            if (role == 0 && has_dx) gemm32<L::OFF_WT0>(dx, wl, dpre, lane);
            wgrad16(dW0, db0, S2, XA, lane);
            PH(5)
            if (role == 0) {
                if (has_dx) {
                    if (hk >= 2)
                        while (__hip_atomic_load(&flags[1], __ATOMIC_ACQUIRE, __HIP_MEMORY_SCOPE_WORKGROUP) < hk - 1) __builtin_amdgcn_s_sleep(1);
                    PH(6)
                    float *slot = XCH + (hk & 1) * 512;
#pragma unroll
                    for (int s = 0; s < 8; ++s) slot[s * 64 + lane] = dx[s >> 2][s & 3];
                    __hip_atomic_store(&flags[0], hk + 1, __ATOMIC_RELEASE, __HIP_MEMORY_SCOPE_WORKGROUP);
                }
            } else {
                if (has_dx) {
                    while (__hip_atomic_load(&flags[0], __ATOMIC_ACQUIRE, __HIP_MEMORY_SCOPE_WORKGROUP) < hk + 1) __builtin_amdgcn_s_sleep(1);
                    PH(6)
                    const float *slot = XCH + (hk & 1) * 512;
#pragma unroll
                    for (int s = 0; s < 8; ++s) dx[s >> 2][s & 3] = slot[s * 64 + lane];
                    __hip_atomic_store(&flags[1], hk + 1, __ATOMIC_RELEASE, __HIP_MEMORY_SCOPE_WORKGROUP);
                    gemm32<L::OFF_WT0>(dx, wl, dpre, lane);
                    float v[8];
#pragma unroll
                    for (int s = 0; s < 8; ++s) v[s] = dx[s >> 2][s & 3];
                    store8(v, vdx, dvoff, ds0);
                    if (emit) {
                        if (!full) {
#pragma unroll
                            for (int s = 0; s < 8; ++s) v[s] = valid ? v[s] : 0.f;
                        }
#pragma unroll
                        for (int s = 0; s < 8; ++s) {
                            es1[s] += v[s];
                            es2[s] = fmaf(v[s], u[s], es2[s]);
                        }
                    }
                }
            }
            ++hk;
        }
        PH(7)
        if (emit && hf == 1) {
            float t1 = 0.f, t2 = 0.f;
            if (ntile >= T1 || ng != g) {
                stage8(S0, lane_base, es1);
                stage8(S1, lane_base, es2);
                const int ch = lane & 31, hh = lane >> 5;
                const float4 *vp = reinterpret_cast<const float4 *>(S0 + ch * TLD + 8 * hh);
                const float4 *up = reinterpret_cast<const float4 *>(S1 + ch * TLD + 8 * hh);
#pragma unroll
                for (int k = 0; k < 2; ++k) {
                    const float4 a = vp[k], b = up[k];
                    t1 += (a.x + a.y) + (a.z + a.w);
                    t2 += (b.x + b.y) + (b.z + b.w);
                }
                t1 += __shfl_xor(t1, 32);
                t2 += __shfl_xor(t2, 32);
#pragma unroll
                for (int s = 0; s < 8; ++s) es1[s] = es2[s] = 0.f;
            }
            if (lane < 32) reinterpret_cast<float2 *>(P.m[1].s12part)[((long long)g * tpg + tt) * FGNN_H + row_chan(lane)] = make_float2(t1, t2);
        }
        tile = ntile;
        hf = nhf;
        PH(8)
    }

    if constexpr (SKIP) {
        if (emit) {
            for (int t = T0 + pair; t < T1; t += NP) {
                const int g = t / tpg, tt = t - g * tpg;
                if (tile_live(tt, A.N, A.nvalid[g])) continue;
                if (lane < 32) reinterpret_cast<float2 *>(P.m[1].s12part)[((long long)g * tpg + tt) * FGNN_H + lane] = make_float2(0.f, 0.f);
            }
        }
    }

    constexpr int PCOUNT = L::PCOUNT;
    static_assert(PCOUNT == 3 * 1056, "put() below: three layers of 32 x 32 + 32");
    FGNN_T16_DB_BUTTERFLY(db0, db1, db2)
    __syncthreads();
    PH(10)
    {
        float *red = smem + wv * PCOUNT;
        auto put = [&](int off, const f32x4 (&dW)[4], const float (&db)[2]) {
#pragma unroll
            for (int mb = 0; mb < 2; ++mb)
#pragma unroll
                for (int nb = 0; nb < 2; ++nb)
#pragma unroll
                    for (int r = 0; r < 4; ++r) red[off + row_chan(16 * mb + 4 * q + r) * 32 + row_chan(16 * nb + px)] = dW[2 * mb + nb][r];
            if (q == 0) {
                red[off + 1024 + row_chan(px)] = db[0];
                red[off + 1024 + row_chan(16 + px)] = db[1];
            }
        };
        put(0, dW0, db0);
        put(1056, dW1, db1);
        put(2112, dW2, db2);
    }
    __syncthreads();
    sum_pair_partials<PCOUNT>(smem, P);
    PH(11)
    PH_FLUSH
}

template <bool SKIP, bool HAS_DX>
int launch_pair16(const fgnn_mlp_bwd_args *a1, const fgnn_mlp_bwd_args *a2, int tpg, int total, hipStream_t st) {
    constexpr int LDS = PairLayout16::LDS_F * 4;
    static_assert(LDS <= 160 * 1024, "LDS budget");
    static LdsAttrCache attr_cache;
    (void)fgnn_raise_lds(attr_cache, (const void *)mlp_bwd_pair_t16_kernel<SKIP, HAS_DX>, LDS);
    PairArgs P;
    P.m[0] = *a1;
    P.m[1] = *a2;
    hipLaunchKernelGGL((mlp_bwd_pair_t16_kernel<SKIP, HAS_DX>), dim3(a1->cu_share == 2 && !SKIP ? BWD_WG / 2 : BWD_WG), dim3(64 * NW), LDS, st, P, tpg,
                       total);
    FGNN_LAUNCH_CHECK();
    return 0;
}

}

#ifdef FGNN_PHASES
extern "C" int fgnn_debug_phase_buffer_t16(void *p) { return hipMemcpyToSymbol(HIP_SYMBOL(g_phase16_buf), &p, sizeof(p)) == hipSuccess ? 0 : 1; }
#endif

extern "C" int fgnn_mlp_bwd_pair_t16(const fgnn_mlp_bwd_args *a1, const fgnn_mlp_bwd_args *a2, void *stream) {
    if (check_pair_common(a1, a2, "fgnn_mlp_bwd_pair_t16", 29, true)) return 1;
    FGNN_CHECK(a1->depth == 3 && a1->a.C == 32 && a1->b.C == 0 && a2->b.C == 0 && !a1->xbits && !a2->xbits,
               "fgnn_mlp_bwd_pair_t16: built for depth 3 and ONE dense input slab of 32 channels (got depth %d, %d + %d); use fgnn_mlp_bwd_pair",
               a1->depth, a1->a.C, a1->b.C);
    FGNN_CHECK(a1->ranges == a2->ranges && (!a1->ranges || a1->nvalid), "fgnn_mlp_bwd_pair_t16: both MLPs take the same ranges (with nvalid)");
    FGNN_CHECK(a1->packed && a2->packed, "fgnn_mlp_bwd_pair_t16: needs both operand images (fgnn_pack_operands, kind 5)");
    FGNN_CHECK(a1->N <= 256, "fgnn_mlp_bwd_pair_t16: N <= 256 (division-free pixel decode)");
    const int tpg = fgnn_tiles_per_graph(a1->N);
    const long long total = (long long)a1->G * tpg;
    hipStream_t st = (hipStream_t)stream;
    if (a2->dxa) return a1->ranges ? launch_pair16<true, true>(a1, a2, tpg, (int)total, st) : launch_pair16<false, true>(a1, a2, tpg, (int)total, st);
    return a1->ranges ? launch_pair16<true, false>(a1, a2, tpg, (int)total, st) : launch_pair16<false, false>(a1, a2, tpg, (int)total, st);
}
```

graph_neural_net_amd/csrc/mlp_bwd_t16.hip:

```cpp
#include "fgnn_bwd_t16.h"

namespace {

template <int CB>
struct Layout16 : BwdT16Layout<CB, 1, 5> {
    using B = BwdT16Layout<CB, 1, 5>;
    static constexpr int OFF_W0A = B::PK.off_w1a, OFF_W0B = B::PK.off_w1b, OFF_WT0A = B::PK.off_wt0a, OFF_WT0B = B::PK.off_wt0b;
    static constexpr int REC_OFF = B::TILE_END;
    static constexpr int WGK_OFF = REC_OFF + NW * 256;
    static constexpr int LIVE_OFF = WGK_OFF + FGNN_BWD_COEF_GRAPHS * 128;
    static constexpr int MAIN_F = LIVE_OFF + LIVE_LIST_CAP + NW;
    static constexpr int LDS_F = MAIN_F > B::RED_F ? MAIN_F : B::RED_F;
};

template <int CB, bool PKD, bool SKIP, bool DXB>
__global__ __launch_bounds__(64 * NW, 2) void mlp_bwd_t16_kernel(const fgnn_mlp_bwd_args A, const int tpg, const int total_tiles) {
    extern __shared__ __attribute__((aligned(16))) float smem[];
    using L = Layout16<CB>;
    constexpr bool NB = CB == 32;
    const int lane = threadIdx.x & 63, wv = __builtin_amdgcn_readfirstlane(threadIdx.x >> 6);
    const int px = lane & 15, q = lane >> 4;
    const int P2 = A.N * A.N, hpg = 2 * tpg;
    const View va = make_view(A.a.ptr, A.a.gstride, A.a.ldp, A.G);
    const View vb = make_view(A.b.ptr, A.b.gstride, A.b.ldp, A.G);
// ... 187 lines not shown
    if (cached_g >= 0) read_records();

    while (h < H1) {
        const int hn = next_half(SKIP ? h + 1 : h + NW);
        const int g = __builtin_amdgcn_readfirstlane(h / hpg), hh = h - g * hpg;
        const int p = hh * 16 + px;
        const bool inb = p < P2;
        if (g != cached_g) {
            cur_nv = graph_nv(rnv, ragged, g, A.N);
            fetch_records(g, cur_nv);
            read_records();
            cached_g = g;
        }
        bool valid = inb;
        if (ragged) {
            int i, jj;
            row_col(p, A.N, rcpN, i, jj);
            valid = inb && i < cur_nv && jj < cur_nv;
        }
        const bool full = __ballot(valid) == ~0ull;

        float h1[8], h2[8];
        {
            float yb[NXB];
            if constexpr (NB) {
#pragma unroll
                for (int s = 0; s < 8; ++s) yb[s] = (xb[s] - mean[s]) * av[s] + beta[s];
            } else {
                yb[0] = xb[0];
            }
            stage8(XA, lane_base, xa);
            if constexpr (CB == 32) {
                stage8(XB, lane_base, yb);
            } else {
                if (q < 2) XB[8 * q * TLD + px] = yb[0];
            }
            f32x4 acc[2];
            load_bias(acc, wl + L::BIAS_F, 0, q);
            gemm32<L::OFF_W0A>(acc, wl, xa, lane);
            if constexpr (CB == 32) gemm32<L::OFF_W0B>(acc, wl, yb, lane);
            else gemm2<L::OFF_W0B>(acc, wl, q < 2 ? yb[0] : 0.f, lane);
            load_x(hn);
            FGNN_T16_RECOMPUTE_HIDDEN(acc, h1, h2)
        }
        float dpre[8];
        FGNN_T16_DZ(dpre)
        stage8(S2, lane_base, dpre);
        load_dyz(hn);
        __builtin_amdgcn_sched_barrier(0);
        FGNN_T16_HIDDEN_BWD(L::OFF_WT2, dpre, dW2, db2, S2, S1, h2)
        __builtin_amdgcn_sched_barrier(0);
        stage8(S1, lane_base, dpre);
        FGNN_T16_HIDDEN_BWD(L::OFF_WT1, dpre, dW1, db1, S1, S0, h1)
        __builtin_amdgcn_sched_barrier(0);
        stage8(S2, lane_base, dpre);
        __builtin_amdgcn_sched_barrier(0);
        {
            f32x4 dx[2];
            float v[8];
            dx[0] = dx[1] = zero4();
            gemm32<L::OFF_WT0A>(dx, wl, dpre, lane);
            wgrad16(dW0a, db0, S2, XA, lane);
#pragma unroll
            for (int s = 0; s < 8; ++s) v[s] = dx[s >> 2][s & 3];
            store8(v, vdxa, lane_voff(vdxa, q, p, inb), g * vdxa.gs4);
            if constexpr (DXB) {
                dx[0] = dx[1] = zero4();
                gemm32<L::OFF_WT0B>(dx, wl, dpre, lane);
            }
            if constexpr (CB == 32) {
                wgrad16(dW0b, dbx, S2, XB, lane);
            } else {
                const int i = lane & 15;
                const float4 a0 = *reinterpret_cast<const float4 *>(S2 + i * TLD + 4 * q);
                const float4 a1 = *reinterpret_cast<const float4 *>(S2 + (16 + i) * TLD + 4 * q);
                const float4 b0 = *reinterpret_cast<const float4 *>(XB + i * TLD + 4 * q);
                dW0b[0] = mfma16(a0.x, b0.x, dW0b[0]);
                dW0b[2] = mfma16(a1.x, b0.x, dW0b[2]);
                dW0b[0] = mfma16(a0.y, b0.y, dW0b[0]);
                dW0b[2] = mfma16(a1.y, b0.y, dW0b[2]);
                dW0b[0] = mfma16(a0.z, b0.z, dW0b[0]);
                dW0b[2] = mfma16(a1.z, b0.z, dW0b[2]);
                dW0b[0] = mfma16(a0.w, b0.w, dW0b[0]);
                dW0b[2] = mfma16(a1.w, b0.w, dW0b[2]);
            }
            if constexpr (DXB) {
#pragma unroll
                for (int s = 0; s < 8; ++s) v[s] = dx[s >> 2][s & 3];
                store8(v, vdxb, lane_voff(vdxb, q, p, inb), g * vdxb.gs4);
            }
        }
        h = hn;
    }

    constexpr int PCOUNT = L::PCOUNT, CIN = L::CIN;
    FGNN_T16_DB_BUTTERFLY(db0, db1, db2)
    (void)dbx;
    __syncthreads();
    {
        float *red = smem + wv * PCOUNT;
#pragma unroll
        for (int mb = 0; mb < 2; ++mb)
#pragma unroll
            for (int nb = 0; nb < 2; ++nb)
#pragma unroll
                for (int r = 0; r < 4; ++r) {
                    const int o = row_chan(16 * mb + 4 * q + r), c = row_chan(16 * nb + px);
                    red[o * CIN + c] = dW0a[2 * mb + nb][r];
                    if (c < CB) red[o * CIN + 32 + c] = dW0b[2 * mb + nb][r];
                    red[32 * CIN + 32 + o * 32 + c] = dW1[2 * mb + nb][r];
                    red[32 * CIN + 32 + 1056 + o * 32 + c] = dW2[2 * mb + nb][r];
                }
        if (q == 0) {
            const int c0 = row_chan(px), c1 = row_chan(16 + px);
            red[32 * CIN + c0] = db0[0];
            red[32 * CIN + c1] = db0[1];
            red[32 * CIN + 32 + 1024 + c0] = db1[0];
            red[32 * CIN + 32 + 1024 + c1] = db1[1];
            red[32 * CIN + 32 + 1056 + 1024 + c0] = db2[0];
            red[32 * CIN + 32 + 1056 + 1024 + c1] = db2[1];
        }
    }
    __syncthreads();
    sum_wave_partials<PCOUNT, NW>(smem, A.wpart);
}

template <int CB, bool PKD, bool SKIP, bool DXB>
int launch16(const fgnn_mlp_bwd_args *a, int tpg, int total, hipStream_t st) {
    constexpr int LDS = Layout16<CB>::LDS_F * 4;
    static_assert(LDS <= 160 * 1024, "LDS budget");
    static LdsAttrCache attr_cache;
    (void)fgnn_raise_lds(attr_cache, (const void *)mlp_bwd_t16_kernel<CB, PKD, SKIP, DXB>, LDS);
    hipLaunchKernelGGL((mlp_bwd_t16_kernel<CB, PKD, SKIP, DXB>), dim3(a->cu_share == 2 && !SKIP ? BWD_WG / 2 : BWD_WG), dim3(64 * NW), LDS, st, *a,
                       tpg, total);
    FGNN_LAUNCH_CHECK();
    return 0;
}
template <int CB, bool PKD, bool DXB>
int launch16s(const fgnn_mlp_bwd_args *a, int tpg, int total, hipStream_t st) {
    return a->ranges ? launch16<CB, PKD, true, DXB>(a, tpg, total, st) : launch16<CB, PKD, false, DXB>(a, tpg, total, st);
}

}

extern "C" int fgnn_mlp_bwd_t16_supported(const fgnn_mlp_bwd_args *a) {
    if (!a || a->depth != 3 || a->a.C != 32 || a->a.nrm || !a->dxa || a->accumulate_a || a->accumulate_b || !a->packed || a->N > 256) return 0;
    if (a->b.C == 32) return (a->b.nrm && a->dxb && !a->xbits) ? 1 : 0;
    if (a->b.C == 2) return (!a->b.nrm && !a->dxb) ? 1 : 0;
    return 0;
}

extern "C" int fgnn_mlp_bwd_t16(const fgnn_mlp_bwd_args *a, void *stream) {
    FGNN_CHECK(a != nullptr, "fgnn_mlp_bwd_t16: null args");
    FGNN_CHECK(fgnn_mlp_bwd_t16_supported(a), "fgnn_mlp_bwd_t16: built for depth 3, slab a = 32 raw channels with dx stored, slab b = 32 normalised "
               "channels with dx stored or 2 raw channels without dx, an operand image of kind 5, N <= 256; use fgnn_mlp_bwd");
    FGNN_CHECK(a->G > 0 && a->N > 0 && a->a.ptr && (a->b.ptr || (a->xbits && a->b.C == 2)), "fgnn_mlp_bwd_t16: bad G / N / slabs");
    FGNN_CHECK(!a->xbits || a->xdeg, "fgnn_mlp_bwd_t16: xbits without xdeg (fgnn_adjacency_degree)");
    if (check_mlp_bwd_common(a, "fgnn_mlp_bwd_t16", 29)) return 1;
    for (int l = 0; l < a->depth; ++l) FGNN_CHECK(a->W[l] && a->bias[l], "fgnn_mlp_bwd_t16: missing weights layer %d", l);
    const int tpg = fgnn_tiles_per_graph(a->N);
    const long long total = (long long)a->G * tpg;
    FGNN_CHECK(!a->ranges || (a->nvalid && !a->s12tiles), "fgnn_mlp_bwd_t16: ranges need nvalid and exclude s12tiles");
    FGNN_CHECK(!a->s12tiles || fgnn_mlp_bwd_coef_tiles_supported(a->G, a->N), "fgnn_mlp_bwd_t16: s12tiles needs a workgroup's tile range to span <= %d graphs",
               FGNN_BWD_COEF_GRAPHS);
    hipStream_t st = (hipStream_t)stream;
    if (a->b.C == 32) return launch16s<32, false, true>(a, tpg, (int)total, st);
    if (a->xbits) return launch16s<2, true, false>(a, tpg, (int)total, st);
    return launch16s<2, false, false>(a, tpg, (int)total, st);
}
```

graph_neural_net_amd/csrc/mlp_bwd_x3.hip:

```cpp
#include "fgnn_tile.h"
#include "fgnn_pack.h"
#include "fgnn_x3.h"
#include "fgnn_bwd32.h"

namespace {


template <int CA, int CB, int NWT>
struct BwdX3Layout {
    static constexpr int NW = NWT;
    static constexpr int DEPTH = 3;
    static constexpr PkX3 PK = pkx3_layout(1, CA, CB, DEPTH);
    static constexpr int PD = PK.part_dw;
    static constexpr int OFF_W0A = PK.p.off_w0a, OFF_W0B = PK.p.off_w0b;
    static constexpr int OFF_W1 = PK.p.off_wh;
    static constexpr int OFF_W2T = PK.p.off_wt, OFF_W1T = PK.p.off_wt + 2;
    static constexpr int OFF_WT0A = PK.p.off_wt0a, OFF_WT0B = PK.p.off_wt0b;
    static constexpr int STEPS_A = pk16_steps(CA), STEPS_B = pk16_steps(CB);
    static constexpr int BIAS_F = PK.bias_off;
    static constexpr int WEIGHT_F = PK.floats;
    static constexpr bool TWO_SLOT = CB > 0;
    static constexpr int NSLOT = TWO_SLOT ? 2 : 3;
    static constexpr int REC_F = (CB > 0 ? 3 : 2) * 32 * 4;
    static constexpr int PCOUNT = 32 * (CA + CB) + 32 + (DEPTH - 1) * (32 * 32 + 32);
// ... 335 lines not shown
            if constexpr (CB > 0) {
                float yb[SB > 0 ? SB : 1];
                norm_slab<SB>(yb, xb, recB, normB, c_valid, h);
                if constexpr (CB < 32) {
#pragma unroll
                    for (int r = 0; r < 16; ++r) SX[ch_of(r, h) * TLD + j] = 0.f;
                }
#pragma unroll
                for (int s = 0; s < SB; ++s) SX[slab_ch<SB>(s, h) * TLD + j] = yb[s];
                X3 XT;
                float dummy = 0.f;
                load_wgrad_operand<false>(XT, SX, dummy, lane, negI);
                dW0b = gemm_x3_rr<X3_BWD_TERMS>(dW0b, DT, XT);
                const TileCtx cn = decode_tile(tnext, tnext < T1, tpg, A.N, P, j);
                load_slab<SB, PK>(xb, vb, ps, cn, h);
            }
        }
        if constexpr (CA == 32) {
            if (A.dxa) {
                const int voff = lane_off<4>(vdxa, c, h);
                const int s0 = c.g * vdxa.gs4;
                float v[16];
#pragma unroll
                for (int r = 0; r < 16; ++r) v[r] = dxa_acc[r];
                if (A.accumulate_a) {
#pragma unroll
                    for (int r = 0; r < 16; ++r) v[r] += buf_load(vdxa, voff, s0 + ((r & 3) + 8 * (r >> 2)) * vdxa.ld4);
                }
#pragma unroll
                for (int r = 0; r < 16; ++r) buf_store(v[r], vdxa, voff, s0 + ((r & 3) + 8 * (r >> 2)) * vdxa.ld4);
                if constexpr (CB == 0) {
                    if (emit) {
#pragma unroll
                        for (int r = 0; r < 16; ++r) {
                            const int ch = ch_of(r, h);
                            const float mean = reinterpret_cast<const float4 *>(recA)[ch].x;
                            S1[ch * TLD + j] = c_valid ? v[r] : 0.f;
                            S2[ch * TLD + j] = xa[r] - mean;
                        }
                        const float4 *vp = reinterpret_cast<const float4 *>(S1 + j * TLD + 16 * h);
                        const float4 *up = reinterpret_cast<const float4 *>(S2 + j * TLD + 16 * h);
                        float s1 = 0.f, s2 = 0.f;
#pragma unroll
                        for (int k = 0; k < 4; ++k) {
                            const float4 a = vp[k], b = up[k];
                            s1 += (a.x + a.y) + (a.z + a.w);
                            s2 += (a.x * b.x + a.y * b.y) + (a.z * b.z + a.w * b.w);
                        }
                        s1 += __shfl_xor(s1, 32);
                        s2 += __shfl_xor(s2, 32);
                        if (h == 0) {
                            float2 o;
                            o.x = s1;
                            o.y = s2;
                            reinterpret_cast<float2 *>(A.s12part)[((long long)c.g * tpg + c.tt) * FGNN_H + j] = o;
                        }
                    }
                }
            }
        }
        if constexpr (CB == 32) {
            if (A.dxb) {
                const int voff = lane_off<4>(vdxb, c, h);
                const int s0 = c.g * vdxb.gs4;
                float vb2[16];
#pragma unroll
                for (int r = 0; r < 16; ++r) vb2[r] = dxb_acc[r];
                if (A.accumulate_b) {
#pragma unroll
                    for (int r = 0; r < 16; ++r) vb2[r] += buf_load(vdxb, voff, s0 + ((r & 3) + 8 * (r >> 2)) * vdxb.ld4);
                }
#pragma unroll
                for (int r = 0; r < 16; ++r) buf_store(vb2[r], vdxb, voff, s0 + ((r & 3) + 8 * (r >> 2)) * vdxb.ld4);
            }
        }
        if constexpr (CA == 32 && CB == 0) {
#pragma unroll
            for (int s = 0; s < SA; ++s) xa[s] = nxa[s];
        }
    }

    constexpr int PCOUNT = L::PCOUNT;
#pragma unroll
    for (int l = 0; l < DEPTH; ++l) db[l] += __shfl_xor(db[l], 32);
    if constexpr (VW0) {
#pragma unroll
        for (int r = 0; r < 32; ++r) w0v[r] = half_sum(w0v[r]);
#pragma unroll
        for (int r = 0; r < 16; ++r) b0v[r] = half_sum(b0v[r]);
    }
    __syncthreads();
    {
        float *red = smem + wv * PCOUNT;
#pragma unroll
        for (int r = 0; r < 16; ++r) {
            const int o = ch_of(r, h);
            if constexpr (VW0) {
                if (j == 0) {
                    red[o * CIN] = w0v[2 * r];
                    red[o * CIN + 1] = w0v[2 * r + 1];
                    red[32 * CIN + o] = b0v[r];
                }
            } else {
                if (j < CA) red[o * CIN + j] = dW0a[r];
                if (CB > 0 && j < CB) red[o * CIN + CA + j] = dW0b[r];
            }
        }
        int off = 32 * CIN;
#pragma unroll
        for (int l = 0; l < DEPTH; ++l) {
            if (l > 0) {
#pragma unroll
                for (int r = 0; r < 16; ++r) red[off + ch_of(r, h) * 32 + j] = dWh[l - 1][r];
                off += 1024;
            }
            if (h == 0 && !(VW0 && l == 0)) red[off + j] = db[l];
            off += 32;
        }
    }
    __syncthreads();
    static_assert(PCOUNT % 4 == 0, "partials are summed four at a time");
    float4 *out = reinterpret_cast<float4 *>(A.wpart + (long long)blockIdx.x * PCOUNT);
    const float4 *part4 = reinterpret_cast<const float4 *>(smem);
    for (int e = threadIdx.x; e < PCOUNT / 4; e += 64 * NW) {
        float4 a = part4[e];
#pragma unroll
        for (int w = 1; w < NW; ++w) {
            const float4 b = part4[w * (PCOUNT / 4) + e];
            a.x += b.x;
            a.y += b.y;
            a.z += b.z;
            a.w += b.w;
        }
        out[e] = a;
    }
}

template <int CA, int CB, bool PK, int NWT = 8>
int launch_bwd_x3(const fgnn_mlp_bwd_args *a, int tpg, int total, hipStream_t st) {
    constexpr int LDS = BwdX3Layout<CA, CB, NWT>::LDS_F * 4;
    constexpr int NW = NWT;
    static_assert(LDS <= 160 * 1024, "LDS budget");
    static LdsAttrCache attr_cache;
    (void)fgnn_raise_lds(attr_cache, (const void *)mlp_bwd_x3_kernel<CA, CB, PK, NWT>, LDS);
    hipLaunchKernelGGL((mlp_bwd_x3_kernel<CA, CB, PK, NWT>), dim3(a->cu_share == 2 ? BWD_WG / 2 : BWD_WG), dim3(64 * NW), LDS, st, *a, tpg, total);
    FGNN_LAUNCH_CHECK();
    return 0;
}

}

extern "C" int fgnn_mlp_bwd_x3(const fgnn_mlp_bwd_args *a, void *stream) {
    FGNN_CHECK(a != nullptr, "fgnn_mlp_bwd_x3: null args");
    FGNN_CHECK(a->G > 0 && a->N > 0, "fgnn_mlp_bwd_x3: bad G=%d N=%d", a->G, a->N);
    FGNN_CHECK(mlp_x3_supported(a->a.C, a->b.C, a->depth, 1),
               "fgnn_mlp_bwd_x3: built for depth 3 and 2, 32, 32+2, 32+32 input channels (got depth %d, %d + %d); use fgnn_mlp_bwd",
               a->depth, a->a.C, a->b.C);
    FGNN_CHECK(a->packed, "fgnn_mlp_bwd_x3: needs the operand image of fgnn_pack_x3_operands (kind 1)");
    FGNN_CHECK(!a->ranges, "fgnn_mlp_bwd_x3: no padding-tile skipping (ranges); use fgnn_mlp_bwd for ragged batches");
    const bool pk_a = a->xbits && a->a.C == 2, pk_b = a->xbits && a->b.C == 2;
    FGNN_CHECK((a->a.ptr || pk_a) && (a->b.C == 0 || a->b.ptr || pk_b), "fgnn_mlp_bwd_x3: slab pointer missing");
    FGNN_CHECK(!a->xbits || a->xdeg, "fgnn_mlp_bwd_x3: xbits without xdeg (fgnn_adjacency_degree)");
    FGNN_CHECK(!(a->a.C != 32 && a->dxa) && !(a->b.C != 32 && a->b.C != 0 && a->dxb),
               "fgnn_mlp_bwd_x3: input gradients exist for 32-channel slabs only; use fgnn_mlp_bwd");
    if (check_mlp_bwd_common(a, "fgnn_mlp_bwd_x3", 30)) return 1;
    const int tpg = fgnn_tiles_per_graph(a->N);
    const long long total = (long long)a->G * tpg;
    FGNN_CHECK(!a->s12tiles || a->b.C > 0, "fgnn_mlp_bwd_x3: s12tiles is built into the two-slab kernels only");
    FGNN_CHECK(!a->s12tiles || fgnn_mlp_bwd_coef_tiles_supported(a->G, a->N),
               "fgnn_mlp_bwd_x3: s12tiles needs a workgroup's tile range to span <= %d graphs (G=%d N=%d)", FGNN_BWD_COEF_GRAPHS, a->G, a->N);
    hipStream_t st = (hipStream_t)stream;
    const int ca = a->a.C, cb = a->b.C;
    if (a->xbits) {
        if (ca == 2 && cb == 0) return launch_bwd_x3<2, 0, true>(a, tpg, (int)total, st);
        if (ca == 32 && cb == 2) return launch_bwd_x3<32, 2, true>(a, tpg, (int)total, st);
        fgnn_set_error("fgnn_mlp_bwd_x3: xbits needs a 2-channel slab (2 or 32+2 input channels)");
        return 1;
    }
    if (ca == 2 && cb == 0) return launch_bwd_x3<2, 0, false>(a, tpg, (int)total, st);
    if (ca == 32 && cb == 0) return launch_bwd_x3<32, 0, false>(a, tpg, (int)total, st);
    if (ca == 32 && cb == 2) return launch_bwd_x3<32, 2, false>(a, tpg, (int)total, st);
    return launch_bwd_x3<32, 32, false>(a, tpg, (int)total, st);
}
```

graph_neural_net_amd/engine.py:

```python
import ctypes as C
import os

import torch

from . import _lib
from .engine_base import EngineBase

EPS = 1e-05


class ParamLayout:

    def __init__(self, original_features_num=2, num_blocks=4, in_features=32, out_features=32, depth_of_mlp=3):
        if in_features != _lib.FGNN_H or out_features != _lib.FGNN_H:
            raise RuntimeError('the fused engine is built for in_features = out_features = 32 (got %d, %d); other widths '
                               'run through the per-layer modules (layers.MlpBlock_Real)' % (in_features, out_features))
        if not 1 <= depth_of_mlp <= _lib.FGNN_MAX_DEPTH:
            raise RuntimeError('depth_of_mlp must be in 1..%d' % _lib.FGNN_MAX_DEPTH)
        if original_features_num not in (2, 32):
            raise RuntimeError('the fused engine is built for original_features_num = 2 or 32 (got %d); other widths run '
                               'through the per-layer modules (layers.MlpBlock_Real)' % original_features_num)
        self.c0 = original_features_num
        self.num_blocks = num_blocks
        self.depth = depth_of_mlp
        self.entries = []
        self.mlp = {}
        off = 0
        last = original_features_num
        for blk in range(1, num_blocks + 1):
            for j, cin in ((1, last), (2, last), (3, last + 32)):
                pfx = 'ne_bm_block%d_mlp%d.' % (blk, j)
                rec = {'off': off, 'cin': cin, 'w': [], 'b': []}
                c = cin
                for i in range(depth_of_mlp):
                    self.entries.append((pfx + 'convs.%d.weight' % i, off, (32, c, 1, 1)))
                    rec['w'].append(off)
                    off += 32 * c
                    self.entries.append((pfx + 'convs.%d.bias' % i, off, (32,)))
                    rec['b'].append(off)
                    off += 32
                    c = 32
                self.entries.append((pfx + 'gn.weight', off, (1, 32, 1, 1)))
                rec['gn_w'] = off
                off += 32
                self.entries.append((pfx + 'gn.bias', off, (1, 32, 1, 1)))
                rec['gn_b'] = off
                off += 32
                rec['count'] = _lib.mlp_param_count(cin, depth_of_mlp)
                self.mlp[(blk, j)] = rec
            last = 32
        self.total = off

    def flatten(self, state_dict, device):
        flat = torch.empty(self.total, dtype=torch.float32, device=device)
        for name, off, shape in self.entries:
            key = name if name in state_dict else 'node_embedder.' + name
            t = state_dict[key]
            n = t.numel()
            flat[off:off + n].copy_(t.reshape(-1).to(torch.float32))
        return flat

    def init_flat(self, seed, device):
        gen = torch.Generator().manual_seed(seed)
        flat = torch.zeros(self.total, dtype=torch.float32)
        for name, off, shape in self.entries:
            n = _numel(shape)
            if name.endswith('.weight') and '.convs.' in name:
                fan_out, fan_in = shape[0], shape[1]
                bound = (6.0 / (fan_in + fan_out)) ** 0.5
                flat[off:off + n] = (torch.rand(n, generator=gen) * 2 - 1) * bound
            elif name.endswith('gn.weight'):
                flat[off:off + n] = 1.0
        return flat.to(device)

    def unflatten(self, flat):
        return {name: flat[off:off + _numel(shape)].view(shape) for name, off, shape in self.entries}


def _numel(shape):
    n = 1
    for s in shape:
        n *= s
    return n


def _round_up(x, m):
    return (x + m - 1) // m * m


class EngineCache:

    def __init__(self, budget):
        import collections
        self.budget = budget
        self._items = collections.OrderedDict()

    @staticmethod
    def engine_bytes(G, N, num_blocks, elt=4):
        ldp = -(-N * N // 32) * 32
        return (4 * num_blocks + 5) * G * 32 * ldp * elt

    def get(self, key, factory, nbytes):
        hit = self._items.get(key)
        if hit is not None:
            self._items.move_to_end(key)
            return hit[0], []
        eng = factory()
        self._items[key] = (eng, nbytes)
        evicted = []
        while self.used() > self.budget and len(self._items) > 1:
            k, _ = self._items.popitem(last=False)
            evicted.append(k)
        return eng, evicted

    def used(self):
        return sum(b for _, b in self._items.values())

    def keys(self):
        return list(self._items)

    def clear(self):
        self._items.clear()

    def __len__(self):
        return len(self._items)

    def __iter__(self):
        return iter(list(self._items))

    def values(self):
        return [e for e, _ in self._items.values()]


class FgnnEngine(EngineBase):
    SKIP_PADDING_TILES = True
    MM_ORDER = True
    PAIR_BWD = os.environ.get('FGNN_PAIR_BWD', '1') != '0'
    PACK_IN_STRUCT = os.environ.get('FGNN_PACK_IN_STRUCT', '1') != '0'
    T16 = os.environ.get('FGNN_T16', 'pair,bwd')

    MFMA = os.environ.get('FGNN_MFMA', 'f32')

    BLOCK1 = os.environ.get('FGNN_BLOCK1', 'generic')
    GN_FINALIZE = ('fgnn_gn_finalize', 'fgnn_gn_finalize2')

    def __init__(self, layout, G, N, device, ragged=False, cu_share=0, mfma=None, block1=None):
        _lib.load()
        self.T16 = type(self).T16
        self.cu_share = int(cu_share)
        mfma = self.MFMA if mfma is None else mfma
        if mfma not in ('f32', 'x3'):
            raise ValueError("mfma must be 'f32' or 'x3' (got %r)" % (mfma,))
        self.x3 = (mfma == 'x3' and not ragged and layout.depth == 3 and layout.c0 in (2, 32))
        block1 = self.BLOCK1 if block1 is None else block1
        if block1 not in ('generic', 'structured'):
            raise ValueError("block1 must be 'generic' or 'structured' (got %r)" % (block1,))
        self.struct1 = (block1 == 'structured' and cu_share == 0
                        and bool(_lib.load().fgnn_block1_struct_supported(N, layout.depth, layout.c0)))
        super().__init__(layout, G, N, device, ragged)
        self.P = N * N
        self.ldp = _round_up(self.P, 32)
        self.tpg = _lib.tiles_per_graph(N)
        self._gn_args = (EPS,)
        K = layout.num_blocks
        f32 = dict(dtype=torch.float32, device=device)
        self._act = act = lambda: torch.empty(G * 32 * self.ldp, **f32)
        self.z = {(k, j): act() for k in range(1, K + 1) for j in (1, 2, 3)}
        self.mult = {k: act() for k in range(1, K + 1)}
        self.part = [torch.empty(G * self.tpg * 32 * 2, **f32) for _ in range(2)]
        self.cnt = torch.empty(G * 2 * self.tpg, **f32)
        self.mm_order = (torch.empty(G, dtype=torch.int32, device=device)
                         if self.ranges is not None and self.MM_ORDER and 64 < N <= 256 else None)
        self.x = None
        self.xdeg = None
        self._packs = {}
        self._pack_entry = 'fgnn_pack_x3_operands' if self.x3 else 'fgnn_pack_operands'
        for k in range(1, K + 1):
            cin = layout.c0 if k == 1 else 32
            fl = _lib.load().fgnn_pack_x3_floats if self.x3 else _lib.load().fgnn_pack_floats
            f12, b12 = 0, (5 if self._t16_pair(cin) else 1)
            f3 = 2 if self.x3 else 0
            b3 = 5 if self._t16_bwd3(cin) else (3 if self.x3 else 1)
            self._packs[('f', k, 12)] = (f12, cin, 0, 2, torch.empty(fl(f12, cin, 0, layout.depth, 2), **f32))
            self._packs[('f', k, 3)] = (f3, 32, cin, 1, torch.empty(fl(f3, 32, cin, layout.depth, 1), **f32))
            for j in (1, 2):
                self._packs[('b', k, j)] = (b12, cin, 0, 1, torch.empty(fl(b12, cin, 0, layout.depth, 1), **f32))
            self._packs[('b', k, 3)] = (b3, 32, cin, 1, torch.empty(fl(b3, 32, cin, layout.depth, 1), **f32))

    def _t16(self, what):
        return self.T16 not in ('0', '') and what in self.T16.split(',')

    def _t16_pair(self, cin):
        return (self._t16('pair') and self.PAIR_BWD and not self.x3 and self.layout.depth == 3 and cin == 32 and self.N <= 256)

    def _t16_bwd3(self, cin):
        return self._t16('bwd') and not self.x3 and self.layout.depth == 3 and cin in (2, 32) and self.N <= 256

    def _slab_in(self, k, params):
        if k == 1:
            if self.xbits is not None:
                s = _lib.Slab()
                s.gstride, s.ldp, s.C = self.layout.c0 * self.P, self.P, self.layout.c0
                return s
            return _lib.make_slab(self.x, self.layout.c0 * self.P, self.P, self.layout.c0)
        rec = self.layout.mlp[(k - 1, 3)]
        s = _lib.make_slab(self.z[(k - 1, 3)], 32 * self.ldp, self.ldp, 32, nrm=self.nrm[(k - 1, 3)])
        s.beta = self._w(params, rec['gn_b'])
        return s

    def _slab_z(self, k, j, params):
        rec = self.layout.mlp[(k, j)]
        s = _lib.make_slab(self.z[(k, j)], 32 * self.ldp, self.ldp, 32, nrm=self.nrm[(k, j)])
        s.beta = self._w(params, rec['gn_b'])
        return s

    def _slab_raw(self, t):
        return _lib.make_slab(t, 32 * self.ldp, self.ldp, 32)

    def _mlp_fwd(self, params, k, js, a, b, finalize=True):
        L = self.layout
        args = _lib.MlpFwdArgs()
        args.G, args.N, args.depth, args.nmlp = self.G, self.N, L.depth, len(js)
        args.nvalid = self.nvalid.data_ptr() if self.nvalid is not None else None
        args.a = a
        if b is not None:
            args.b = b
        for m, j in enumerate(js):
            rec = L.mlp[(k, j)]
            for l in range(L.depth):
                args.W[m][l] = self._w(params, rec['w'][l])
                args.bias[m][l] = self._w(params, rec['b'][l])
            args.z[m] = self.z[(k, j)].data_ptr()
            args.part[m] = self.part[m].data_ptr()
        args.ldz = self.ldp
        args.cnt = self.cnt.data_ptr()
        args.packed = self._packs[('f', k, 12 if len(js) == 2 else 3)][4].data_ptr()
        self._packed_input(args, k)
        if self.ranges is not None:
            args.ranges = self.ranges.data_ptr()
        args.cu_share = self.cu_share
        st = _lib.stream_ptr()
        entry = 'fgnn_mlp_fwd_x3' if (self.x3 and len(js) == 2) else 'fgnn_mlp_fwd'
        _lib.call(entry, C.byref(args), st, tag='mlp_fwd[cin=%d,nmlp=%d]' % (a.C + (b.C if b is not None else 0), len(js)))
        if self.decisions is not None:
            bufs = [torch.zeros(self.G * (L.depth - 1) * 32 * self.tpg, dtype=torch.int32, device=self.device) for _ in js]
            _lib.call('fgnn_debug_mlp_fwd_x3_masks' if (self.x3 and len(js) == 2) else 'fgnn_debug_mlp_fwd_masks', C.byref(args),
                      _lib.ptr(bufs[0]), _lib.ptr(bufs[1]) if len(js) == 2 else None, st)
            for j, buf in zip(js, bufs):
                self.decisions[(k, j)] = buf
        if finalize:
            self._gn_finalize(params, k, js)

    def _packed_input(self, args, k):
        if k == 1 and self.xbits is not None:
            args.xbits = self.xbits.data_ptr()
            args.xdeg = self.xdeg.data_ptr()

    def embed(self, params, x, nvalid=None, bits=None, pack=True):
        L = self.layout
        self._adopt_nvalid(nvalid)
        st = _lib.stream_ptr()
        if self.ranges is not None:
            _lib.call('fgnn_ragged_tile_ranges_order', _lib.ptr(self.nvalid), self.G, self.N, _lib.ptr(self.ranges),
                      _lib.ptr(self.mm_order) if self.mm_order is not None else None, st, tag='fgnn_ragged_tile_ranges')
        if bits is not None:
            if x is not None or L.c0 != 2 or L.depth != 3:
                raise RuntimeError('FgnnEngine.embed: bits= replaces x and needs original_features_num = 2, depth_of_mlp = 3')
            self._check_bits(bits)
            if self.xdeg is None:
                self.xdeg = torch.empty(self.G * self.N, dtype=torch.float32, device=self.device)
            self.x, self.xbits = None, bits
            if not self.struct1:
                _lib.call('fgnn_adjacency_degree', _lib.ptr(bits), self._nv(), self.G, self.N, _lib.ptr(self.xdeg), st)
        else:
            if x.shape != (self.G, L.c0, self.N, self.N) or not x.is_contiguous() or x.dtype != torch.float32:
                raise RuntimeError('FgnnEngine.embed: expected contiguous fp32 %s, got %s %s'
                                   % ((self.G, L.c0, self.N, self.N), tuple(x.shape), x.dtype))
            self.x, self.xbits = x, None
        struct_now = self.struct1 and self.xbits is not None
        pack_in_struct = pack and struct_now and self.PACK_IN_STRUCT and not self.x3 and len(self._packs) <= _lib.MAX_PACK_JOBS
        if pack and not pack_in_struct:
            self.pack_operands(params)
        for k in range(1, L.num_blocks + 1):
            sin = self._slab_in(k, params)
            if k == 1 and struct_now:
                self._struct_fwd(params, with_pack=pack_in_struct)
                pool_fin = L.num_blocks == 1 and bool(_lib.load().fgnn_colmax_fwd_fin_supported(self.N))
                self._mlp_fwd(params, 1, (3,), self._slab_raw(self.mult[1]), sin, finalize=not pool_fin)
                continue
            fin = bool(_lib.load().fgnn_chan_matmul_fwd_fin_supported(self.N)) and self.G * 32 <= 4096
            self._mlp_fwd(params, k, (1, 2), sin, None, finalize=not fin)
            ya, yb = self._slab_z(k, 1, params), self._slab_z(k, 2, params)
            if fin:
                r1, r2 = L.mlp[(k, 1)], L.mlp[(k, 2)]
                _lib.call('fgnn_chan_matmul_fwd_fin_ord', C.byref(ya), C.byref(yb), _lib.ptr(self.part[0]), _lib.ptr(self.part[1]),
                          _lib.ptr(self.cnt), C.c_void_p(self._w(params, r1['gn_w'])), C.c_void_p(self._w(params, r2['gn_w'])),
                          EPS, self._nv(), self.G, self.N, _lib.ptr(self.mult[k]), 32 * self.ldp, self.ldp,
                          _lib.ptr(self.mm_order) if self.mm_order is not None else None, self._fill(), st, tag='fgnn_chan_matmul_fwd')
            else:
                _lib.call('fgnn_chan_matmul_fwd_ord', C.byref(ya), C.byref(yb), self._nv(), self.G, self.N,
                          _lib.ptr(self.mult[k]), 32 * self.ldp, self.ldp,
                          _lib.ptr(self.mm_order) if self.mm_order is not None else None, self._fill(), st, tag='fgnn_chan_matmul_fwd')
            pool_fin = k == L.num_blocks and bool(_lib.load().fgnn_colmax_fwd_fin_supported(self.N))
            self._mlp_fwd(params, k, (3,), self._slab_raw(self.mult[k]), sin, finalize=not pool_fin)
        out = self._slab_z(L.num_blocks, 3, params)
        if pool_fin:
            rec = L.mlp[(L.num_blocks, 3)]
            _lib.call('fgnn_colmax_fwd_fin', C.byref(out), _lib.ptr(self.part[0]), _lib.ptr(self.cnt),
                      C.c_void_p(self._w(params, rec['gn_w'])), EPS, self._nv(), self.G, self.N, _lib.ptr(self.E),
                      _lib.ptr(self.idx), st, tag='fgnn_colmax_fwd')
        else:
            _lib.call('fgnn_colmax_fwd', C.byref(out), self._nv(), self.G, self.N, _lib.ptr(self.E), _lib.ptr(self.idx), st)
        return self.E

    def _fill(self):
        return 1 if self.ranges is not None else 0

    def _struct_fwd(self, params, with_pack=False):
        S = self._struct_ws()
        st = _lib.stream_ptr()
        (w1, b1), (w2, b2) = self._w3(params, 1), self._w3(params, 2)
        r1, r2 = self.layout.mlp[(1, 1)], self.layout.mlp[(1, 2)]
        args = [_lib.ptr(self.xbits), self._nv(), self.G, self.N, _lib.ptr(S['tab']),
                C.c_void_p(self._w(params, r1['gn_w'])), C.c_void_p(self._w(params, r1['gn_b'])),
                C.c_void_p(self._w(params, r2['gn_w'])), C.c_void_p(self._w(params, r2['gn_b'])), EPS,
                _lib.ptr(self.nrm[(1, 1)]), _lib.ptr(self.nrm[(1, 2)]), _lib.ptr(self.mult[1]), 32 * self.ldp, self.ldp,
                _lib.ptr(self.xdeg), _lib.ptr(S['ws']), w1, b1, w2, b2]
        if with_pack:
            items = list(self._packs.items())
            _lib.call('fgnn_block1_struct_fwd_pack', *args, self._pack_jobs(params, items), len(items), st)
        else:
            _lib.call('fgnn_block1_struct_fwd', *args, st)

    def _struct_bwd(self, params):
        S, W = self._struct_ws(), self._bwd
        W['struct_rows'] = int(_lib.load().fgnn_block1_struct_rows(self.G, self.N))
        (w1, _), (w2, _) = self._w3(params, 1), self._w3(params, 2)
        r1, r2 = self.layout.mlp[(1, 1)], self.layout.mlp[(1, 2)]
        _lib.call('fgnn_block1_struct_bwd', _lib.ptr(self.xbits), self._nv(), self.G, self.N, _lib.ptr(S['tab']), w1, w2,
                  _lib.ptr(self.nrm[(1, 1)]), _lib.ptr(self.nrm[(1, 2)]),
                  C.c_void_p(self._w(params, r1['gn_b'])), C.c_void_p(self._w(params, r2['gn_b'])),
                  _lib.ptr(W['dmult']), 32 * self.ldp, self.ldp, _lib.ptr(S['ws']),
                  _lib.ptr(W['wpart'][(1, 1)]), _lib.ptr(W['wpart'][(1, 2)]), _lib.ptr(W['s12'][(1, 1)]), _lib.ptr(W['s12'][(1, 2)]),
                  _lib.stream_ptr())

    def _partial_rows(self):
        nwg = super()._partial_rows()
        if self.cu_share == 2 and self.ranges is None:
            nwg //= 2
        return nwg

    def _coef(self, kj, slot):
        W = self._bwd
        _lib.call('fgnn_gn_bwd_coef', _lib.ptr(W['s12'][kj]), _lib.ptr(self.nrm[kj]), self._nv(), self.G, 32, self.N,
                  _lib.ptr(W['coef'][slot]), None, None, _lib.stream_ptr())

    def _mlp_bwd(self, params, k, j, a, b, dy, coef, dxa, dxb, acc_a, acc_b, emit=False, dx_strides=None):
        args = self._mlp_bwd_args(params, k, j, a, b, dy, coef, dxa, dxb, acc_a, acc_b, emit, dx_strides)
        entry = 'fgnn_mlp_bwd_x3' if (self.x3 and j != 3) else 'fgnn_mlp_bwd'
        if j == 3 and b is not None and self._t16_bwd3(b.C) and _lib.load().fgnn_mlp_bwd_t16_supported(C.byref(args)):
            entry = 'fgnn_mlp_bwd_t16'
        elif self._packs[('b', k, j)][0] == 5:
            args.packed = None
        _lib.call(entry, C.byref(args), _lib.stream_ptr(),
                  tag='mlp_bwd[cin=%d,dx=%d]' % (a.C + (b.C if b is not None else 0),
                                                (a.C if dxa is not None else 0) + (b.C if (b is not None and dxb is not None) else 0)))

    def _mlp_bwd_pair(self, params, k, sin, din, emit):
        W = self._bwd
        a1 = self._mlp_bwd_args(params, k, 1, sin, None, W['dy1'], None, None, None, False, False, False, None)
        a2 = self._mlp_bwd_args(params, k, 2, sin, None, W['dy2'], None, din, None, True, False, emit, None)
        entry = 'fgnn_mlp_bwd_pair_x3' if self.x3 else ('fgnn_mlp_bwd_pair_t16' if self._t16_pair(sin.C) else 'fgnn_mlp_bwd_pair')
        _lib.call(entry, C.byref(a1), C.byref(a2), _lib.stream_ptr(),
                  tag='mlp_bwd_pair[cin=%d,dx=%d]' % (sin.C, sin.C if din is not None else 0))

    def _mlp_bwd_args(self, params, k, j, a, b, dy, coef, dxa, dxb, acc_a, acc_b, emit, dx_strides):
        L = self.layout
        W = self._bwd
        rec = L.mlp[(k, j)]
        gs = 32 * self.ldp
        args = _lib.MlpBwdArgs()
        args.G, args.N, args.depth = self.G, self.N, L.depth
        args.nvalid = self.nvalid.data_ptr() if self.nvalid is not None else None
        args.a = a
        if b is not None:
            args.b = b
        for l in range(L.depth):
            args.W[l] = self._w(params, rec['w'][l])
            args.bias[l] = self._w(params, rec['b'][l])
        args.dy, args.dgstride, args.ldd = dy.data_ptr(), gs, self.ldp
        args.z, args.zgstride, args.ldz = self.z[(k, j)].data_ptr(), gs, self.ldp
        if isinstance(coef, str):
            args.s12tiles = W['s12part'].data_ptr()
            args.s12_out = W['s12'][(k, j)].data_ptr()
            args.znrm = self.nrm[(k, j)].data_ptr()
        elif coef is not None:
            args.coef = coef.data_ptr()
        else:
            args.s12 = W['s12'][(k, j)].data_ptr()
            args.znrm = self.nrm[(k, j)].data_ptr()
        dgs, dld = (gs, self.ldp) if dx_strides is None else dx_strides
        if dxa is not None:
            args.dxa, args.dxa_gstride, args.dxa_ld = dxa.data_ptr(), (gs if (b is not None and dx_strides is not None) else dgs), \
                (self.ldp if (b is not None and dx_strides is not None) else dld)
        if dxb is not None:
            args.dxb, args.dxb_gstride, args.dxb_ld = dxb.data_ptr(), dgs, dld
        args.accumulate_a, args.accumulate_b = int(acc_a), int(acc_b)
        args.wpart = W['wpart'][(k, j)].data_ptr()
        args.packed = self._packs[('b', k, j)][4].data_ptr()
        self._packed_input(args, k)
        if self.ranges is not None:
            args.ranges = self.ranges.data_ptr()
        args.cu_share = self.cu_share
        if emit:
            args.s12part = W['s12part'].data_ptr()
        return args

    def backward_from_dE(self, params, grads, dE, finalize=True, dx=None):
        L = self.layout
        W = self._alloc_bwd()
        st = _lib.stream_ptr()
        gs = 32 * self.ldp
        K = L.num_blocks
        in_prologue = bool(_lib.load().fgnn_mlp_bwd_coef_tiles_supported(self.G, self.N)) and self.ranges is None
        dy = W['dy'][0]
        out = self._slab_z(K, 3, params)
        _lib.call('fgnn_colmax_bwd', _lib.ptr(dE), _lib.ptr(self.idx), self._nv(), self.G, 32, self.N,
                  _lib.ptr(dy), gs, self.ldp, C.byref(out), _lib.ptr(W['s12'][(K, 3)]), st)
        for k in range(K, 0, -1):
            sin = self._slab_in(k, params)
            first = (k == 1)
            din = None if first else W['dy'][(K - k + 1) % 2]
            dxs = None
            if first and dx is not None:
                if self.xbits is not None or self.x3 or tuple(dx.shape) != (self.G, L.c0, self.N, self.N) or dx.dtype != torch.float32 \
                        or not dx.is_contiguous():
                    raise RuntimeError('FgnnEngine: the input gradient needs a dense fp32 input, the fp32-MFMA kernels (mfma="f32") '
                                       'and a contiguous (G, c0, N, N) fp32 dx')
                din, dxs = dx, (L.c0 * self.P, self.P)
            self._mlp_bwd(params, k, 3, self._slab_raw(self.mult[k]), sin, dy,
                          None if k == K else ('tiles' if in_prologue else W['coef'][2]), W['dmult'], din, False, False, dx_strides=dxs)
            if first and self.struct1 and self.xbits is not None and dxs is None:
                self._struct_bwd(params)
                dy = din
                continue
            ya, yb = self._slab_z(k, 1, params), self._slab_z(k, 2, params)
            _lib.call('fgnn_chan_matmul_bwd_ord', C.byref(ya), C.byref(yb), _lib.ptr(W['dmult']), gs, self.ldp,
                      self._nv(), self.G, self.N, _lib.ptr(W['dy1']), _lib.ptr(W['dy2']), gs, self.ldp,
                      _lib.ptr(W['s12'][(k, 1)]), _lib.ptr(W['s12'][(k, 2)]),
                      _lib.ptr(self.mm_order) if self.mm_order is not None else None, self._fill(), st, tag='fgnn_chan_matmul_bwd')
            if first:
                W['struct_rows'] = 0
            if self.PAIR_BWD and dxs is None and L.depth == 3 and sin.C in (2, 32):
                self._mlp_bwd_pair(params, k, sin, din, emit=not first)
            else:
                self._mlp_bwd(params, k, 1, sin, None, W['dy1'], None, din, None, True, False, dx_strides=dxs)
                self._mlp_bwd(params, k, 2, sin, None, W['dy2'], None, din, None, True, False, emit=not first, dx_strides=dxs)
            if not first and not in_prologue:
                _lib.call('fgnn_gn_bwd_coef_tiles', _lib.ptr(W['s12part']), _lib.ptr(self.nrm[(k - 1, 3)]), self._nv(),
                          self.G, 32, self.N, _lib.ptr(W['s12'][(k - 1, 3)]), _lib.ptr(W['coef'][2]), st)
            dy = din
        if finalize:
            self.grad_finalize(grads)
        return grads

    def relu_decisions(self, params=None):
        L, G, N, P = self.layout, self.G, self.N, self.P
        out = {}
        bit = torch.arange(32, device=self.device, dtype=torch.int32)
        for (k, j), buf in self.decisions.items():
            w = buf.view(G, L.depth - 1, 32, self.tpg)
            m = ((w.unsqueeze(-1) >> bit) & 1).reshape(G, L.depth - 1, 32, self.tpg * 32)[..., :P].reshape(G, L.depth - 1, 32, N, N)
            for l in range(L.depth - 1):
                out[(k, j, l)] = m[:, l].bool()
        if self.struct1 and self.xbits is not None and (1, 1) not in self.decisions:
            nc = 2 + 2 * (N + 1)
            tab = self._struct['tab'].view(2, nc, 4, 32)
            words = (N + 31) // 32
            b = self.xbits.view(G, N, words).to(torch.int64) & 0xffffffff
            col = torch.arange(N, device=self.device)
            wmat = ((b[:, :, col // 32] >> (col % 32)) & 1)
            if self.nvalid is not None:
                nv = self.nvalid.to(torch.int64)
                inside = (col[None, :] < nv[:, None])
                wmat = wmat * (inside[:, :, None] & inside[:, None, :])
            deg = wmat.sum(-1)
            eye = torch.eye(N, device=self.device, dtype=torch.bool)
            diag_cls = 2 + 2 * deg + torch.diagonal(wmat, dim1=1, dim2=2)
            cls = torch.where(eye[None], diag_cls[:, :, None].expand(G, N, N), wmat)
            for j in (1, 2):
                for l in range(2):
                    hv = tab[j - 1, :, l, :] > 0
                    out[(1, j, l)] = hv[cls].permute(0, 3, 1, 2).contiguous()
        return out


    def normalized(self, k, j, params):
        rec = self.layout.mlp[(k, j)]
        y = torch.empty(self.G, 32, self.N, self.N, dtype=torch.float32, device=self.device)
        _lib.call('fgnn_gn_apply', _lib.ptr(self.z[(k, j)]), 32 * self.ldp, self.ldp, _lib.ptr(self.nrm[(k, j)]),
                  C.c_void_p(self._w(params, rec['gn_b'])), self._nv(), self.G, 32, self.N,
                  _lib.ptr(y), 32 * self.P, self.P, _lib.stream_ptr())
        return y

    def unpadded(self, buf):
        return buf.view(self.G, 32, self.ldp)[:, :, :self.P].reshape(self.G, 32, self.N, self.N).clone()
```

include/fgnn_hip.h:

```cpp
#ifndef FGNN_HIP_H
#define FGNN_HIP_H

#ifdef __cplusplus
extern "C" {
#endif

#define FGNN_H 32
#define FGNN_TILE 32
#define FGNN_MAX_DEPTH 3

typedef struct {
    const float *ptr;
    long long gstride;
    long long ldp;
    int C;
    const float *nrm;
    const float *beta;
} fgnn_slab;

const char *fgnn_last_error(void);
int fgnn_version(void);
int fgnn_tiles_per_graph(int N);
int fgnn_mlp_bwd_num_workgroups(void);

// ... 56 lines not shown
                    long long x_gstride, long long x_ld, const int *nvalid, int G, int N, int M, int K, float *wpart,
                    void *stream);

#define FGNN_DW_MAX_JOBS 4
typedef struct {
    const float *dy; long long d_gstride, d_ld;
    const float *relu_mask;
    const float *x; long long x_gstride, x_ld;
    int M, K;
} fgnn_dw_job;
int fgnn_conv1x1_dw_multi(const fgnn_dw_job *jobs, int njobs, const int *nvalid, int G, int N, float *wpart, void *stream);

typedef struct {
    const float *W;
    long long w_ostride, w_kstride;
    const float *bias;
    int M, K;
    int relu;
    const float *mask;
    float *out;
    long long o_gstride;
} fgnn_chain_layer;
typedef struct {
    const float *x;
    long long x_gstride, x_ld;
    int depth;
    fgnn_chain_layer layer[3];
    long long o_ld;
    const int *nvalid;
    int G, N;
} fgnn_chain_args;
int fgnn_conv_chain_supported(int depth, int K0, const int *M );
int fgnn_conv_chain(const fgnn_chain_args *args, void *stream);

typedef struct {
    const float *x;
    long long x_gstride, x_ld;
    int cin;
    const float *xb;
    long long xb_gstride, xb_ld;
    int cb;
    const float *packed;
    const int *nvalid;
    int G, N;
    float *out;
    long long o_gstride, o_ld;
    const float *dz;
    long long dz_gstride, dz_ld;
    float *dx;
    long long dx_gstride, dx_ld;
    float *dxb;
    long long dxb_gstride, dxb_ld;
    int accumulate_dx, accumulate_dxb;
    float *wpart;
} fgnn_mlp64_args;
int fgnn_mlp64_supported(int cin, int depth, int width);
int fgnn_mlp64_num_workgroups(void);
int fgnn_mlp64_param_count(int cin);
int fgnn_mlp64_packed_floats(int cin);
int fgnn_mlp64_pack(const float *W0, const float *W1, const float *W2, const float *b0, const float *b1, const float *b2, int cin,
                    float *packed, void *stream);
typedef struct {
    const float *W[3];
    const float *bias[3];
    int cin;
    float *packed;
} fgnn_mlp64_pack_job;
int fgnn_mlp64_pack_multi(const fgnn_mlp64_pack_job *jobs, int njobs, void *stream);
int fgnn_mlp64_fwd(const fgnn_mlp64_args *args, void *stream);
int fgnn_mlp64_bwd(const fgnn_mlp64_args *args, void *stream);

int fgnn_chan_matmul_fwd(const fgnn_slab *ya, const fgnn_slab *yb, const int *nvalid, int G, int N,
                         float *out, long long ogstride, long long ldo, void *stream);
int fgnn_chan_matmul_fwd_ord(const fgnn_slab *ya, const fgnn_slab *yb, const int *nvalid, int G, int N,
                             float *out, long long ogstride, long long ldo, const int *order, int fill, void *stream);
int fgnn_chan_matmul_fwd_fin_supported(int N);
int fgnn_chan_matmul_fwd_fin(const fgnn_slab *ya, const fgnn_slab *yb, const float *part_a, const float *part_b,
                             const float *cnt, const float *gn_weight_a, const float *gn_weight_b, float eps,
                             const int *nvalid, int G, int N, float *out, long long ogstride, long long ldo, void *stream);
int fgnn_chan_matmul_fwd_fin_ord(const fgnn_slab *ya, const fgnn_slab *yb, const float *part_a, const float *part_b,
                                 const float *cnt, const float *gn_weight_a, const float *gn_weight_b, float eps,
                                 const int *nvalid, int G, int N, float *out, long long ogstride, long long ldo,
                                 const int *order , int fill, void *stream);

int fgnn_colmax_fwd(const fgnn_slab *y, const int *nvalid, int G, int N, float *e ,
                    int *idx , void *stream);
int fgnn_colmax_fwd_fin_supported(int N);
int fgnn_colmax_fwd_fin(const fgnn_slab *y, const float *part, const float *cnt, const float *gn_weight, float eps,
                        const int *nvalid, int G, int N, float *e, int *idx, void *stream);

#define FGNN_SCORE_SPLIT 4
int fgnn_score_ce_fwd(const float *e1, const float *e2, const int *nvalid, int B, int C, int N,
                      float *scores, float *lse, float *pair_loss, void *stream);
int fgnn_score_row_blocks(int B, int N);
int fgnn_score_ce_fwd_blocks(const float *e1, const float *e2, const int *nvalid, int B, int C, int N, int row_blocks,
                             float *scores, float *lse, float *pair_loss, void *stream);
int fgnn_score_ce_bwd(const float *e1, const float *e2, const float *scores, const float *lse,
                      const int *nvalid, const float *gscale, int B, int C, int N,
                      float *de1, float *de2, void *stream);

int fgnn_score_ce_fwd_blocks_labels(const float *e1, const float *e2, const int *nvalid, const int *labels, int B, int C, int N,
                                    int row_blocks, float *scores, float *lse, float *pair_loss, void *stream);
int fgnn_score_ce_bwd_labels(const float *e1, const float *e2, const float *scores, const float *lse, const int *nvalid,
                             const int *labels, const float *gscale, int B, int C, int N, float *de1, float *de2, void *stream);
int fgnn_ce_fwd_labels(const float *scores, const int *nvalid, const int *labels, int B, int N, float *lse, float *pair_loss,
                       void *stream);
int fgnn_ce_bwd_labels(const float *scores, const float *lse, const int *nvalid, const int *labels, const float *gscale, int B, int N,
                       float *dscores, void *stream);

int fgnn_ce_fwd(const float *scores, const int *nvalid, int B, int N, float *lse, float *pair_loss, void *stream);
int fgnn_ce_bwd(const float *scores, const float *lse, const int *nvalid, const float *gscale, int B, int N,
                float *dscores, void *stream);
int fgnn_score_bwd(const float *e1, const float *e2, const float *dscores, const int *nvalid,
                   int B, int C, int N, float *de1, float *de2, void *stream);

int fgnn_colmax_bwd(const float *de, const int *idx, const int *nvalid, int G, int C, int N,
                    float *dy, long long gstride, long long ldp, const fgnn_slab *y, float *s12, void *stream);

int fgnn_gn_bwd_stats(const float *dy, long long dgstride, long long ldd,
                      const float *z, long long zgstride, long long ldz, const float *nrm,
                      const int *nvalid, int G, int C, int N, float *s12 , void *stream);
int fgnn_gn_bwd_coef(const float *s12, const float *nrm, const int *nvalid, int G, int C, int N,
                     float *coef , float *dgn_w , float *dgn_b ,
                     void *stream);
int fgnn_gn_bwd_coef_tiles(const float *s12part, const float *nrm, const int *nvalid, int G, int C, int N,
                           float *s12, float *coef, void *stream);
int fgnn_gn_bwd_apply(const float *dy, long long dgstride, long long ldd,
                      const float *z, long long zgstride, long long ldz, const float *coef,
                      const int *nvalid, int G, int C, int N, float *dz, long long ogstride, long long ldo, void *stream);

typedef struct {
    int G, N, depth;
    const int *nvalid;
    fgnn_slab a, b;
    const float *W[FGNN_MAX_DEPTH];
    const float *bias[FGNN_MAX_DEPTH];
    const float *dy;  long long dgstride, ldd;
    const float *z;   long long zgstride, ldz;
    const float *coef;
    const float *s12;
    const float *znrm;
    float *dxa; long long dxa_gstride, dxa_ld;
    float *dxb; long long dxb_gstride, dxb_ld;
    int accumulate_a, accumulate_b;
    float *wpart;
    float *s12part;
    const float *packed;
    const float *s12tiles;
    float *s12_out;
    const unsigned *xbits;
    const float *xdeg;
    const int *ranges;
    int cu_share;
} fgnn_mlp_bwd_args;
int fgnn_mlp_bwd(const fgnn_mlp_bwd_args *args, void *stream);
int fgnn_mlp_bwd_x3(const fgnn_mlp_bwd_args *args, void *stream);
int fgnn_mlp_bwd_pair(const fgnn_mlp_bwd_args *m1, const fgnn_mlp_bwd_args *m2, void *stream);
int fgnn_mlp_bwd_pair_x3(const fgnn_mlp_bwd_args *m1, const fgnn_mlp_bwd_args *m2, void *stream);
int fgnn_mlp_bwd_t16_supported(const fgnn_mlp_bwd_args *args);
int fgnn_mlp_bwd_t16(const fgnn_mlp_bwd_args *args, void *stream);
int fgnn_mlp_bwd_pair_t16(const fgnn_mlp_bwd_args *m1, const fgnn_mlp_bwd_args *m2, void *stream);
#define FGNN_BWD_COEF_GRAPHS 4
int fgnn_mlp_bwd_coef_tiles_supported(int G, int N);
int fgnn_mlp_param_count(int Cin, int depth);
int fgnn_reduce_partials(const float *wpart, int num_wg, int count, float *out, void *stream);

#define FGNN_MAX_GRAD_JOBS 16
typedef struct {
    const float *wpart; int count; float *out;
    const float *s12; const float *nrm; float *dgn_w; float *dgn_b;
    int rows;
    float scale;
    const float *scale_dev;
} fgnn_grad_job;
int fgnn_grad_finalize(const fgnn_grad_job *jobs, int njobs, int num_wg, int G, int C, void *stream);
int fgnn_inv_node_count(const int *nvalid, int B, float *out, void *stream);

int fgnn_chan_matmul_bwd(const fgnn_slab *ya, const fgnn_slab *yb, const float *dm, long long dmgstride, long long ldm,
                         const int *nvalid, int G, int N,
                         float *da, float *db, long long ogstride, long long ldo,
                         float *s12a ,
                         float *s12b , void *stream);
int fgnn_chan_matmul_bwd_ord(const fgnn_slab *ya, const fgnn_slab *yb, const float *dm, long long dmgstride, long long ldm,
                             const int *nvalid, int G, int N, float *da, float *db, long long ogstride, long long ldo,
                             float *s12a, float *s12b, const int *order, int fill , void *stream);

int fgnn_adam_step(float *params, const float *grads, float *exp_avg, float *exp_avg_sq, int n, double lr,
                   double beta1, double beta2, double eps, int step, double grad_scale, void *stream);
int fgnn_adam_step_dev(float *params, const float *grads, float *exp_avg, float *exp_avg_sq, int n,
                       const double *hp, int *state, void *stream);
#define FGNN_GUARD_MAX_PARTS 64
#define FGNN_GUARD_SKIP_NONFINITE 1
#define FGNN_GUARD_NONFINITE 1
typedef struct {
    double max_norm;
    double norm;
    double coef;
    int flags;
    int skipped;
    int arrivals;
    int mode;
    double partial[FGNN_GUARD_MAX_PARTS];
} fgnn_guard_record;
int fgnn_grad_guard(const float *grads, int n, const double *hp, fgnn_guard_record *guard, void *stream);
int fgnn_adam_step_guarded(float *params, const float *grads, float *exp_avg, float *exp_avg_sq, int n, const double *hp,
                           int *state, const fgnn_guard_record *guard, void *stream);
int fgnn_accuracy_max(const float *scores, const int *nvalid, int B, int N, int *correct, void *stream);
#define FGNN_LSAP_MAX_N 2048
int fgnn_lsap_accuracy(const float *cost, long long bstride, int ld, const int *nvalid, int B, int N, int *correct,
                       int *assign , void *stream);

int fgnn_block1_struct_supported(int N, int depth, int original_features_num);
int fgnn_block1_struct_table_floats(int N);
long long fgnn_block1_struct_ws_floats(int G, int N);
int fgnn_block1_struct_rows(int G, int N);
int fgnn_block1_struct_fwd(const unsigned *bits, const int *nvalid, int G, int N, const float *tables, const float *gnw1, const float *gnb1,
                           const float *gnw2, const float *gnb2, float eps, float *nrm1, float *nrm2, float *mult, long long gstride,
                           long long ldp, float *xdeg , float *ws,
                           const float *const *tW1, const float *const *tb1, const float *const *tW2, const float *const *tb2
                           ,
                           void *stream);
int fgnn_block1_struct_bwd(const unsigned *bits, const int *nvalid, int G, int N, const float *tables, const float *const *W1,
                           const float *const *W2, const float *nrm1, const float *nrm2, const float *gnb1, const float *gnb2,
                           const float *dmult, long long gstride, long long ldp, float *ws, float *wpart1, float *wpart2, float *s12_1,
                           float *s12_2, void *stream);
int fgnn_block1_struct_fwd_pack(const unsigned *bits, const int *nvalid, int G, int N, const float *tables, const float *gnw1, const float *gnb1,
                                const float *gnw2, const float *gnb2, float eps, float *nrm1, float *nrm2, float *mult, long long gstride,
                                long long ldp, float *xdeg, float *ws, const float *const *tW1, const float *const *tb1,
                                const float *const *tW2, const float *const *tb2, const fgnn_pack_job *jobs, int njobs, void *stream);
int fgnn_block1_struct_fwd16(const unsigned *bits, const int *nvalid, int G, int N, int ldr, const float *tables, const float *gnw1,
                             const float *gnb1, const float *gnw2, const float *gnb2, float eps, float *nrm1, float *nrm2,
                             void *mult , long long gstride, long long ldp, void *x16 , float *ws,
                             const float *const *tW1, const float *const *tb1, const float *const *tW2, const float *const *tb2, void *stream);
int fgnn_block1_struct_fwd16_pack(const unsigned *bits, const int *nvalid, int G, int N, int ldr, const float *tables, const float *gnw1,
                                  const float *gnb1, const float *gnw2, const float *gnb2, float eps, float *nrm1, float *nrm2, void *mult,
                                  long long gstride, long long ldp, void *x16, float *ws, const float *const *tW1, const float *const *tb1,
                                  const float *const *tW2, const float *const *tb2, const fgnn_pack_job *jobs, int njobs, void *stream);
int fgnn_block1_struct_bwd16(const unsigned *bits, const int *nvalid, int G, int N, int ldr, const float *tables, const float *const *W1,
                             const float *const *W2, const float *nrm1, const float *nrm2, const float *gnb1, const float *gnb2,
                             const void *dmult , long long gstride, long long ldp, float *ws, float *wpart1, float *wpart2,
                             float *s12_1, float *s12_2, void *stream);

int fgnn_expand_adjacency(const unsigned *bits, const int *nvalid, int G, int N, float *x, void *stream);
int fgnn_pack_adjacency(const float *x, const int *nvalid, int G, int N, unsigned *bits, int *bad, void *stream);
int fgnn_pack_adjacency_ld(const float *x, const int *nvalid, int G, int Nin, int N, unsigned *bits, int *bad, void *stream);
int fgnn_pack_adjacency_pair(const float *x1, const float *x2, const int *nvalid1, const int *nvalid2, int B, int Nin, int N, unsigned *bits,
                             int *nv_out, float *inv_out, int *bad, void *stream);
int fgnn_adjacency_degree(const unsigned *bits, const int *nvalid, int G, int N, float *deg, void *stream);

#define FGNN_RANGE_WG 256
int fgnn_ragged_tile_ranges(const int *nvalid, int G, int N, int *ranges , void *stream);
int fgnn_ragged_tile_ranges_order(const int *nvalid, int G, int N, int *ranges , int *order ,
                                  void *stream);
int fgnn_ragged_tile_ranges16(const int *nvalid, int G, int N, int ldr, int *ranges , void *stream);

int fgnn_sum_scale(const float *in, int rows, int cols, float scale, float *out, void *stream);

typedef struct {
    const void *ptr;
    long long gstride;
    long long ldp;
    int C;
    const float *nrm;
    const float *beta;
} fgnn_slab16;
int fgnn_tiles_per_graph16(int N, int ldr);

int fgnn_to_bf16(const float *x, const int *nvalid, int G, int C, int N, int ldr, void *y, long long gstride, long long ldp,
                 void *stream);
int fgnn_from_bf16(const void *y, long long gstride, long long ldp, int G, int C, int N, int ldr, float *x, void *stream);
int fgnn_to_bf16_pad(const float *x, const int *nvalid, int G, int c, int CP, int N, int ldr, void *y, long long ldp, void *stream);

int fgnn_pack16_floats(int kind, int ca, int cb, int depth, int nmlp);
int fgnn_pack16_operands(const fgnn_pack_job *jobs, int njobs, void *stream);

typedef struct {
    int G, N, ldr, depth, nmlp;
    const int *nvalid;
    fgnn_slab16 a, b;
    void *z[2];
    long long ldz;
    float *part[2];
    float *cnt;
    const void *packed;
    const int *ranges;
} fgnn_mlp_fwd16_args;
int fgnn_mlp_fwd16(const fgnn_mlp_fwd16_args *args, void *stream);
int fgnn_debug_mlp_fwd16_masks(const fgnn_mlp_fwd16_args *args, unsigned *masks0, unsigned *masks1, void *stream);

int fgnn_gn_finalize_tpg(const float *part, const float *cnt, const float *gn_weight, const int *nvalid, int G, int C, int N,
                         int tpg, float eps, float *nrm, void *stream);
int fgnn_gn_finalize2_tpg(const float *part0, const float *part1, const float *cnt, const float *gn_weight0,
                          const float *gn_weight1, const int *nvalid, int G, int C, int N, int tpg, float eps, float *nrm0,
                          float *nrm1, void *stream);
int fgnn_gn_bwd_coef_tiles_tpg(const float *s12part, const float *nrm, const int *nvalid, int G, int C, int N, int tpg,
                               float *s12, float *coef, void *stream);

int fgnn_chan_matmul_fwd16(const fgnn_slab16 *ya, const fgnn_slab16 *yb, const int *nvalid, int G, int N, int ldr,
                           void *out, long long ogstride, long long ldo, void *stream);
int fgnn_chan_matmul_fwd16_fin(const fgnn_slab16 *ya, const fgnn_slab16 *yb, const float *part_a, const float *part_b,
                               const float *cnt, const float *gn_weight_a, const float *gn_weight_b, float eps, int tpg,
                               const int *nvalid, int G, int N, int ldr, void *out, long long ogstride, long long ldo,
                               void *stream);
int fgnn_chan_matmul_bwd16(const fgnn_slab16 *ya, const fgnn_slab16 *yb, const void *dm, long long dmgstride, long long ldm,
                           const int *nvalid, int G, int N, int ldr, void *da, void *db, long long ogstride, long long ldo,
                           float *s12a, float *s12b, void *stream);

int fgnn_chan_matmul_bwd16_t(const fgnn_slab16 *ya, const fgnn_slab16 *yb, const void *dm, long long dmgstride, long long ldm,
                             const float *tpart, int tpg, const int *nvalid, int G, int N, int ldr, void *da, void *db,
                             long long ogstride, long long ldo, float *s12a, float *s12b, void *stream);

int fgnn_chan_matmul_bwd16_tc(const fgnn_slab16 *ya, const fgnn_slab16 *yb, const void *dm, long long dmgstride, long long ldm,
                              const float *tpart, int tpg, const int *nvalid, int G, int N, int ldr, void *da, void *db,
                              long long ogstride, long long ldo, float *s12a, float *s12b, float *coefa, float *coefb,
                              void *stream);
int fgnn_colmax_fwd16(const fgnn_slab16 *y, const int *nvalid, int G, int N, int ldr, float *e, int *idx, void *stream);
int fgnn_colmax_bwd16(const float *de, const int *idx, const int *nvalid, int G, int C, int N, int ldr, void *dy,
                      long long gstride, long long ldp, const fgnn_slab16 *y, float *s12, void *stream);
int fgnn_colmax_bwd16_coef(const float *de, const int *idx, const int *nvalid, int G, int C, int N, int ldr, void *dy,
                           long long gstride, long long ldp, const fgnn_slab16 *y, float *s12, float *coef, void *stream);

typedef struct {
    int G, N, ldr, depth;
    const int *nvalid;
    fgnn_slab16 a, b;
    const void *dy;  long long dgstride, ldd;
    const void *z;   long long zgstride, ldz;
    const float *coef;
    void *dxa; long long dxa_gstride, dxa_ld;
    void *dxb; long long dxb_gstride, dxb_ld;
    int accumulate_a, accumulate_b;
    float *wpart;
    float *s12part;
    const void *packed;
    const int *ranges;
} fgnn_mlp_bwd16_args;
int fgnn_mlp_bwd16(const fgnn_mlp_bwd16_args *args, void *stream);
int fgnn_mlp_bwd16_pair(const fgnn_mlp_bwd16_args *m1, const fgnn_mlp_bwd16_args *m2, void *stream);
// ... 99 lines not shown
```

Before: 42400.

## Form normalisation backward dz in chan-matmul backward and hand it to pair MLP bwd

The channel-matmul backward kernel gets a DZ variant. When one workgroup covers a whole channel matrix (N <= TM), it reduces the s12 sums in-block, builds the norm coefficients and writes the normalised pre-activation gradient dz directly instead of the raw dy. The pair t16 MLP backward then takes dz as given: it skips loading z and the coef records and skips the per-element dz formula. This removes one read of z and some arithmetic in the MLP backward. In exchange the matmul epilogue does more work, the path is limited to small N and the t16 pair kernel, and another set of template instantiations is added.

```diff
diff --git a/graph_neural_net_amd/_lib.py b/graph_neural_net_amd/_lib.py
--- a/graph_neural_net_amd/_lib.py
+++ b/graph_neural_net_amd/_lib.py
@@ -86,7 +86,7 @@
                 ('accumulate_a', C.c_int), ('accumulate_b', C.c_int),
                 ('wpart', C.c_void_p), ('s12part', C.c_void_p), ('packed', C.c_void_p),
                 ('s12tiles', C.c_void_p), ('s12_out', C.c_void_p), ('xbits', C.c_void_p), ('xdeg', C.c_void_p),
-                ('ranges', C.c_void_p), ('cu_share', C.c_int)]
+                ('ranges', C.c_void_p), ('cu_share', C.c_int), ('dy_is_dz', C.c_int)]
 
 
 class Slab16(C.Structure):
@@ -240,6 +240,8 @@
     'fgnn_reduce_partials': [_VP, _I, _I, _VP, _VP],
     'fgnn_chan_matmul_bwd': [C.POINTER(Slab), C.POINTER(Slab), _VP, _LL, _LL, _VP, _I, _I, _VP, _VP, _LL, _LL, _VP, _VP, _VP],
     'fgnn_chan_matmul_bwd_ord': [C.POINTER(Slab), C.POINTER(Slab), _VP, _LL, _LL, _VP, _I, _I, _VP, _VP, _LL, _LL, _VP, _VP, _VP, _I, _VP],
+    'fgnn_chan_matmul_bwd_dz_supported': [_I],
+    'fgnn_chan_matmul_bwd_dz_ord': [C.POINTER(Slab), C.POINTER(Slab), _VP, _LL, _LL, _VP, _I, _I, _VP, _VP, _LL, _LL, _VP, _VP, _VP, _I, _VP],
     'fgnn_sum_scale': [_VP, _I, _I, _F, _VP, _VP],
     'fgnn_adam_step': [_VP, _VP, _VP, _VP, _I, C.c_double, C.c_double, C.c_double, C.c_double, _I, C.c_double, _VP],
     'fgnn_adam_step_dev': [_VP, _VP, _VP, _VP, _I, _VP, _VP, _VP],
diff --git a/graph_neural_net_amd/csrc/fgnn_bwd32.h b/graph_neural_net_amd/csrc/fgnn_bwd32.h
--- a/graph_neural_net_amd/csrc/fgnn_bwd32.h
+++ b/graph_neural_net_amd/csrc/fgnn_bwd32.h
@@ -1,5 +1,6 @@
 #pragma once
 #include "fgnn_common.h"
+#include "fgnn_norm.h"
 
 namespace {
 
@@ -8,15 +9,6 @@
 constexpr int NP = 4;
 static_assert(BWD_WG == FGNN_RANGE_WG, "fgnn_ragged_tile_ranges splits for the backward grid");
 
-DEVI float4 coef_from_sums(const float4 n, const float2 sv, float nv) {
-    const float m = nv * nv;
-    float4 k;
-    k.x = n.x;
-    k.y = n.y;
-    k.z = m > 0.f ? -n.y * sv.y * n.w / m : 0.f;
-    k.w = m > 0.f ? -n.y * sv.x / m : 0.f;
-    return k;
-}
 DEVI float4 coef_record(const fgnn_mlp_bwd_args &A, int g, int ch, int nv) {
     if (A.coef) return reinterpret_cast<const float4 *>(A.coef)[(long long)g * FGNN_H + ch];
     const float4 n = reinterpret_cast<const float4 *>(A.znrm)[(long long)g * FGNN_H + ch];
@@ -83,8 +75,11 @@
     FGNN_CHECK(BWD_WG == fgnn_mlp_bwd_num_workgroups(), "%s: workgroup count differs from fgnn_mlp_bwd", fn);
     return 0;
 }
-inline int check_pair_common(const fgnn_mlp_bwd_args *a1, const fgnn_mlp_bwd_args *a2, const char *fn, int tile_bits, bool dense_only) {
+inline int check_pair_common(const fgnn_mlp_bwd_args *a1, const fgnn_mlp_bwd_args *a2, const char *fn, int tile_bits, bool dense_only,
+                             bool dz_built = false) {
     FGNN_CHECK(a1 && a2, "%s: null args", fn);
+    FGNN_CHECK(dz_built || (!a1->dy_is_dz && !a2->dy_is_dz),
+               "%s: dy_is_dz (dz handed over by fgnn_chan_matmul_bwd_dz_ord) is built in fgnn_mlp_bwd_pair_t16 only", fn);
     FGNN_CHECK(BWD_WG == fgnn_mlp_bwd_num_workgroups(), "%s: workgroup count differs from fgnn_mlp_bwd", fn);
     FGNN_CHECK(a1->G > 0 && a1->N > 0 && a1->G == a2->G && a1->N == a2->N && a1->depth == a2->depth,
                "%s: the two MLPs must share G, N and depth", fn);
diff --git a/graph_neural_net_amd/csrc/fgnn_bwd_t16.h b/graph_neural_net_amd/csrc/fgnn_bwd_t16.h
--- a/graph_neural_net_amd/csrc/fgnn_bwd_t16.h
+++ b/graph_neural_net_amd/csrc/fgnn_bwd_t16.h
@@ -37,6 +37,15 @@
         }                                                           \
     }
 
+#define FGNN_T16_READ_NORM(norm)                                    \
+    _Pragma("unroll") for (int s = 0; s < 8; ++s) {                 \
+        if (norm) {                                                 \
+            const float4 n = rec[32 + chan_s(s) + chan_q(q)];       \
+            mean[s] = n.x;                                          \
+            av[s] = n.y;                                            \
+        }                                                           \
+    }
+
 #define FGNN_T16_RECOMPUTE_HIDDEN(acc, h1, h2)                                              \
     _Pragma("unroll") for (int s = 0; s < 8; ++s) h1[s] = relu1(acc[s >> 2][s & 3]);        \
     stage8(S0, lane_base, h1);                                                              \
@@ -47,6 +56,12 @@
 
 #define FGNN_T16_DZ(dpre)                                                                                                   \
     _Pragma("unroll") for (int s = 0; s < 8; ++s) dpre[s] = fmaf(kz[s], zr[s] - kx[s], fmaf(ky[s], dyr[s], kw[s]));         \
+    if (!full) {                                                                                                            \
+        _Pragma("unroll") for (int s = 0; s < 8; ++s) dpre[s] = valid ? dpre[s] : 0.f;                                      \
+    }
+
+#define FGNN_T16_DZ_GIVEN(dpre)                                                                                             \
+    _Pragma("unroll") for (int s = 0; s < 8; ++s) dpre[s] = dyr[s];                                                         \
     if (!full) {                                                                                                            \
         _Pragma("unroll") for (int s = 0; s < 8; ++s) dpre[s] = valid ? dpre[s] : 0.f;                                      \
     }
diff --git a/graph_neural_net_amd/csrc/fgnn_norm.h b/graph_neural_net_amd/csrc/fgnn_norm.h
--- a/graph_neural_net_amd/csrc/fgnn_norm.h
+++ b/graph_neural_net_amd/csrc/fgnn_norm.h
@@ -11,6 +11,16 @@
     o.z = q;
     o.w = 1.f / ve;
     return o;
+}
+
+DEVI float4 coef_from_sums(const float4 n, const float2 sv, float nv) {
+    const float m = nv * nv;
+    float4 k;
+    k.x = n.x;
+    k.y = n.y;
+    k.z = m > 0.f ? -n.y * sv.y * n.w / m : 0.f;
+    k.w = m > 0.f ? -n.y * sv.x / m : 0.f;
+    return k;
 }
 
 struct TilePartials {
diff --git a/graph_neural_net_amd/csrc/matmul.hip b/graph_neural_net_amd/csrc/matmul.hip
--- a/graph_neural_net_amd/csrc/matmul.hip
+++ b/graph_neural_net_amd/csrc/matmul.hip
@@ -226,6 +226,23 @@
             s2 += t * u[k];
         }
     }
+}
+DEVI void tile_sums(float (&t)[16], const float *lds, const float (&u)[16], float &s1, float &s2, int tid) {
+    const int c = tid & 63, r0 = __builtin_amdgcn_readfirstlane(tid >> 6);
+    const float *lp = lds + r0 * LDS_LD + c;
+#pragma unroll
+    for (int k = 0; k < 16; ++k) {
+        t[k] = lp[4 * k * LDS_LD];
+        s1 += t[k];
+        s2 += t[k] * u[k];
+    }
+}
+DEVI void dz_to_global(const View &ov, int mat_off4, const float (&t)[16], const float (&u)[16], const float4 k4, int N, int tid) {
+    const int c = tid & 63, r0 = __builtin_amdgcn_readfirstlane(tid >> 6);
+    const int voff = c < N ? (r0 * N + c) * 4 : OOB_OFF;
+#pragma unroll
+    for (int k = 0; k < 16; ++k)
+        buf_store(fmaf(k4.z, u[k], fmaf(k4.y, t[k], k4.w)), ov, r0 + 4 * k < N ? voff : OOB_OFF, mat_off4 + k * 16 * N);
 }
 
 DEVI void load_tile_raw(float (&x)[16], const View &v, int mat_off4, int N, int nv, int tid) {
@@ -321,6 +338,7 @@
     }
 }
 
+template <bool DZ>
 __global__ __launch_bounds__(256, 4) void chan_matmul_bwd1_kernel(const fgnn_slab ya, const fgnn_slab yb,
                                                                const float *dm, long long dmg, long long ldm,
                                                                const int *nvalid, int N, int M, float *da, float *db,
@@ -384,7 +402,19 @@
         frag_to_lds(Bs, 32 * qi, 32 * qj, accB, lane);
         __syncthreads();
         float sa1 = 0.f, sa2 = 0.f, sb1 = 0.f, sb2 = 0.f;
-        if (s12a) {
+        if constexpr (DZ) {
+            float ta[16], tb[16];
+            tile_sums(ta, Ds, ua, sa1, sa2, tid);
+            tile_sums(tb, Bs, ub, sb1, sb2, tid);
+            s12_epilogue(red, sa1, sa2, sb1, sb2, s12a, s12b, gc, tid);
+            float tot[4];
+#pragma unroll
+            for (int i = 0; i < 4; ++i) tot[i] = (red[0][i] + red[1][i]) + (red[2][i] + red[3][i]);
+            const float4 ka = coef_from_sums(reinterpret_cast<const float4 *>(ya.nrm)[gc], make_float2(tot[0], tot[1]), (float)nv);
+            const float4 kb = coef_from_sums(reinterpret_cast<const float4 *>(yb.nrm)[gc], make_float2(tot[2], tot[3]), (float)nv);
+            dz_to_global(vOA, o_off, ta, ua, ka, N, tid);
+            dz_to_global(vOB, o_off, tb, ub, kb, N, tid);
+        } else if (s12a) {
             tile_to_global<true>(vOA, o_off, Ds, N, ua, sa1, sa2, tid);
             tile_to_global<true>(vOB, o_off, Bs, N, ub, sb1, sb2, tid);
             s12_epilogue(red, sa1, sa2, sb1, sb2, s12a, s12b, gc, tid);
@@ -1069,7 +1099,7 @@
         if (check_2gib("fgnn_chan_matmul_bwd", G, ya->gstride, yb->gstride, dmgstride)) return 1;
         FGNN_CHECK((long long)G * ogstride < 0x7fffffffll / 4, "fgnn_chan_matmul_bwd: output exceeds 2 GiB");
         const int M = G * ya->C;
-        hipLaunchKernelGGL(chan_matmul_bwd1_kernel, dim3(M), dim3(256), 0, (hipStream_t)stream, *ya, *yb, dm,
+        hipLaunchKernelGGL(chan_matmul_bwd1_kernel<false>, dim3(M), dim3(256), 0, (hipStream_t)stream, *ya, *yb, dm,
                            dmgstride, ldm, nvalid, N, M, da, db, ogstride, ldo, s12a, s12b);
         FGNN_LAUNCH_CHECK();
         return 0;
@@ -1102,3 +1132,25 @@
     }
     return 0;
 }
+
+extern "C" int fgnn_chan_matmul_bwd_dz_supported(int N) { return (N > 0 && N <= TM) ? 1 : 0; }
+
+extern "C" int fgnn_chan_matmul_bwd_dz_ord(const fgnn_slab *ya, const fgnn_slab *yb, const float *dm, long long dmgstride,
+                                           long long ldm, const int *nvalid, int G, int N, float *dza, float *dzb,
+                                           long long ogstride, long long ldo, float *s12a, float *s12b, const int *order,
+                                           int fill, void *stream) {
+    (void)fill;
+    FGNN_CHECK(!order || nvalid, "fgnn_chan_matmul_bwd_dz_ord: an order needs the nvalid it was derived from");
+    FGNN_CHECK(ya && yb && dm && dza && dzb && ya->ptr && yb->ptr, "fgnn_chan_matmul_bwd_dz_ord: null argument");
+    FGNN_CHECK(ya->C == yb->C && ya->C > 0 && G > 0 && N > 0, "fgnn_chan_matmul_bwd_dz_ord: bad shapes");
+    FGNN_CHECK(fgnn_chan_matmul_bwd_dz_supported(N), "fgnn_chan_matmul_bwd_dz_ord: N=%d > %d (use fgnn_chan_matmul_bwd_ord: the MLP backward forms dz)",
+               N, TM);
+    FGNN_CHECK(s12a && s12b && ya->nrm && yb->nrm, "fgnn_chan_matmul_bwd_dz_ord: dz needs s12a, s12b and normalised slabs");
+    if (check_2gib("fgnn_chan_matmul_bwd_dz_ord", G, ya->gstride, yb->gstride, dmgstride)) return 1;
+    FGNN_CHECK((long long)G * ogstride < 0x7fffffffll / 4, "fgnn_chan_matmul_bwd_dz_ord: output exceeds 2 GiB");
+    const int M = G * ya->C;
+    hipLaunchKernelGGL(chan_matmul_bwd1_kernel<true>, dim3(M), dim3(256), 0, (hipStream_t)stream, *ya, *yb, dm, dmgstride, ldm,
+                       nvalid, N, M, dza, dzb, ogstride, ldo, s12a, s12b);
+    FGNN_LAUNCH_CHECK();
+    return 0;
+}
diff --git a/graph_neural_net_amd/csrc/mlp_bwd.hip b/graph_neural_net_amd/csrc/mlp_bwd.hip
--- a/graph_neural_net_amd/csrc/mlp_bwd.hip
+++ b/graph_neural_net_amd/csrc/mlp_bwd.hip
@@ -571,6 +571,7 @@
 
 extern "C" int fgnn_mlp_bwd(const fgnn_mlp_bwd_args *a, void *stream) {
     FGNN_CHECK(a != nullptr, "fgnn_mlp_bwd: null args");
+    FGNN_CHECK(!a->dy_is_dz, "fgnn_mlp_bwd: dy_is_dz (dz handed over by fgnn_chan_matmul_bwd_dz_ord) is built in fgnn_mlp_bwd_pair_t16 only");
     FGNN_CHECK(a->G > 0 && a->N > 0, "fgnn_mlp_bwd: bad G=%d N=%d", a->G, a->N);
     FGNN_CHECK(a->depth >= 1 && a->depth <= FGNN_MAX_DEPTH, "fgnn_mlp_bwd: depth %d not in 1..%d", a->depth, FGNN_MAX_DEPTH);
     const bool pk_a = a->xbits && a->a.C == 2, pk_b = a->xbits && a->b.C == 2;
diff --git a/graph_neural_net_amd/csrc/mlp_bwd_pair_t16.hip b/graph_neural_net_amd/csrc/mlp_bwd_pair_t16.hip
--- a/graph_neural_net_amd/csrc/mlp_bwd_pair_t16.hip
+++ b/graph_neural_net_amd/csrc/mlp_bwd_pair_t16.hip
@@ -23,7 +23,7 @@
     static constexpr int LDS_F = MAIN_F > RED_F ? MAIN_F : RED_F;
 };
 
-template <bool SKIP, bool HAS_DX>
+template <bool SKIP, bool HAS_DX, bool DZ>
 __global__ __launch_bounds__(64 * NW, 2) void mlp_bwd_pair_t16_kernel(const PairArgs P, const int tpg, const int total_tiles) {
     extern __shared__ __attribute__((aligned(16))) float smem[];
     using L = PairLayout16;
@@ -77,11 +77,17 @@
     float4 *rec = reinterpret_cast<float4 *>(smem + L::REC_OFF) + wv * 64;
     auto fetch_records = [&](int g, int nv) {
         if (lane < 32) {
-            rec[lane] = coef_record(A, g, lane, nv);
+            if constexpr (!DZ) rec[lane] = coef_record(A, g, lane, nv);
             if (normA) rec[32 + lane] = reinterpret_cast<const float4 *>(A.a.nrm)[(long long)g * A.a.C + lane];
         }
     };
-    auto read_records = [&]() { FGNN_T16_READ_RECORDS(normA) };
+    auto read_records = [&]() {
+        if constexpr (DZ) {
+            FGNN_T16_READ_NORM(normA)
+        } else {
+            FGNN_T16_READ_RECORDS(normA)
+        }
+    };
 
     float xa[8], dyr[8], zr[8], oldr[8];
 #pragma unroll
@@ -117,7 +123,7 @@
         const int p = (act ? tile - g * tpg : 0) * 32 + px;
         const bool inb0 = act && p < P2;
         load8(dyr, vdy, lane_voff(vdy, q, p, inb0), g * vdy.gs4);
-        load8(zr, vz, lane_voff(vz, q, p, inb0), g * vz.gs4);
+        if constexpr (!DZ) load8(zr, vz, lane_voff(vz, q, p, inb0), g * vz.gs4);
         if (has_dx) load8(oldr, vdx, lane_voff(vdx, q, p, inb0 && rmw && role == 0), g * vdx.gs4);
     }
     if (cached_g >= 0) read_records();
@@ -187,10 +193,14 @@
             }
             PH(1)
             float dpre[8];
-            FGNN_T16_DZ(dpre)
+            if constexpr (DZ) {
+                FGNN_T16_DZ_GIVEN(dpre)
+            } else {
+                FGNN_T16_DZ(dpre)
+            }
             stage8(S2, lane_base, dpre);
             load8(dyr, vdy, lane_voff(vdy, q, np, ninb), ng * vdy.gs4);
-            load8(zr, vz, lane_voff(vz, q, np, ninb), ng * vz.gs4);
+            if constexpr (!DZ) load8(zr, vz, lane_voff(vz, q, np, ninb), ng * vz.gs4);
             PH(2)
             __builtin_amdgcn_sched_barrier(0);
             FGNN_T16_HIDDEN_BWD(L::OFF_WT2, dpre, dW2, db2, S2, S1, h2)
@@ -313,16 +323,16 @@
     PH_FLUSH
 }
 
-template <bool SKIP, bool HAS_DX>
+template <bool SKIP, bool HAS_DX, bool DZ>
 int launch_pair16(const fgnn_mlp_bwd_args *a1, const fgnn_mlp_bwd_args *a2, int tpg, int total, hipStream_t st) {
     constexpr int LDS = PairLayout16::LDS_F * 4;
     static_assert(LDS <= 160 * 1024, "LDS budget");
     static LdsAttrCache attr_cache;
-    (void)fgnn_raise_lds(attr_cache, (const void *)mlp_bwd_pair_t16_kernel<SKIP, HAS_DX>, LDS);
+    (void)fgnn_raise_lds(attr_cache, (const void *)mlp_bwd_pair_t16_kernel<SKIP, HAS_DX, DZ>, LDS);
     PairArgs P;
     P.m[0] = *a1;
     P.m[1] = *a2;
-    hipLaunchKernelGGL((mlp_bwd_pair_t16_kernel<SKIP, HAS_DX>), dim3(a1->cu_share == 2 && !SKIP ? BWD_WG / 2 : BWD_WG), dim3(64 * NW), LDS, st, P, tpg,
+    hipLaunchKernelGGL((mlp_bwd_pair_t16_kernel<SKIP, HAS_DX, DZ>), dim3(a1->cu_share == 2 && !SKIP ? BWD_WG / 2 : BWD_WG), dim3(64 * NW), LDS, st, P, tpg,
                        total);
     FGNN_LAUNCH_CHECK();
     return 0;
@@ -335,7 +345,7 @@
 #endif
 
 extern "C" int fgnn_mlp_bwd_pair_t16(const fgnn_mlp_bwd_args *a1, const fgnn_mlp_bwd_args *a2, void *stream) {
-    if (check_pair_common(a1, a2, "fgnn_mlp_bwd_pair_t16", 29, true)) return 1;
+    if (check_pair_common(a1, a2, "fgnn_mlp_bwd_pair_t16", 29, true, true)) return 1;
     FGNN_CHECK(a1->depth == 3 && a1->a.C == 32 && a1->b.C == 0 && a2->b.C == 0 && !a1->xbits && !a2->xbits,
                "fgnn_mlp_bwd_pair_t16: built for depth 3 and ONE dense input slab of 32 channels (got depth %d, %d + %d); use fgnn_mlp_bwd_pair",
                a1->depth, a1->a.C, a1->b.C);
@@ -345,6 +355,12 @@
     const int tpg = fgnn_tiles_per_graph(a1->N);
     const long long total = (long long)a1->G * tpg;
     hipStream_t st = (hipStream_t)stream;
-    if (a2->dxa) return a1->ranges ? launch_pair16<true, true>(a1, a2, tpg, (int)total, st) : launch_pair16<false, true>(a1, a2, tpg, (int)total, st);
-    return a1->ranges ? launch_pair16<true, false>(a1, a2, tpg, (int)total, st) : launch_pair16<false, false>(a1, a2, tpg, (int)total, st);
+    FGNN_CHECK(a1->dy_is_dz == a2->dy_is_dz, "fgnn_mlp_bwd_pair_t16: dy_is_dz is set for both MLPs or for neither");
+    if (a1->dy_is_dz) {
+        if (a2->dxa)
+            return a1->ranges ? launch_pair16<true, true, true>(a1, a2, tpg, (int)total, st) : launch_pair16<false, true, true>(a1, a2, tpg, (int)total, st);
+        return a1->ranges ? launch_pair16<true, false, true>(a1, a2, tpg, (int)total, st) : launch_pair16<false, false, true>(a1, a2, tpg, (int)total, st);
+    }
+    if (a2->dxa) return a1->ranges ? launch_pair16<true, true, false>(a1, a2, tpg, (int)total, st) : launch_pair16<false, true, false>(a1, a2, tpg, (int)total, st);
+    return a1->ranges ? launch_pair16<true, false, false>(a1, a2, tpg, (int)total, st) : launch_pair16<false, false, false>(a1, a2, tpg, (int)total, st);
 }
diff --git a/graph_neural_net_amd/csrc/mlp_bwd_t16.hip b/graph_neural_net_amd/csrc/mlp_bwd_t16.hip
--- a/graph_neural_net_amd/csrc/mlp_bwd_t16.hip
+++ b/graph_neural_net_amd/csrc/mlp_bwd_t16.hip
@@ -363,6 +363,7 @@
 
 extern "C" int fgnn_mlp_bwd_t16(const fgnn_mlp_bwd_args *a, void *stream) {
     FGNN_CHECK(a != nullptr, "fgnn_mlp_bwd_t16: null args");
+    FGNN_CHECK(!a->dy_is_dz, "fgnn_mlp_bwd_t16: dy_is_dz (dz handed over by fgnn_chan_matmul_bwd_dz_ord) is built in fgnn_mlp_bwd_pair_t16 only");
     FGNN_CHECK(fgnn_mlp_bwd_t16_supported(a), "fgnn_mlp_bwd_t16: built for depth 3, slab a = 32 raw channels with dx stored, slab b = 32 normalised "
                "channels with dx stored or 2 raw channels without dx, an operand image of kind 5, N <= 256; use fgnn_mlp_bwd");
     FGNN_CHECK(a->G > 0 && a->N > 0 && a->a.ptr && (a->b.ptr || (a->xbits && a->b.C == 2)), "fgnn_mlp_bwd_t16: bad G / N / slabs");
diff --git a/graph_neural_net_amd/csrc/mlp_bwd_x3.hip b/graph_neural_net_amd/csrc/mlp_bwd_x3.hip
--- a/graph_neural_net_amd/csrc/mlp_bwd_x3.hip
+++ b/graph_neural_net_amd/csrc/mlp_bwd_x3.hip
@@ -511,6 +511,7 @@
 
 extern "C" int fgnn_mlp_bwd_x3(const fgnn_mlp_bwd_args *a, void *stream) {
     FGNN_CHECK(a != nullptr, "fgnn_mlp_bwd_x3: null args");
+    FGNN_CHECK(!a->dy_is_dz, "fgnn_mlp_bwd_x3: dy_is_dz (dz handed over by fgnn_chan_matmul_bwd_dz_ord) is built in fgnn_mlp_bwd_pair_t16 only");
     FGNN_CHECK(a->G > 0 && a->N > 0, "fgnn_mlp_bwd_x3: bad G=%d N=%d", a->G, a->N);
     FGNN_CHECK(mlp_x3_supported(a->a.C, a->b.C, a->depth, 1),
                "fgnn_mlp_bwd_x3: built for depth 3 and 2, 32, 32+2, 32+32 input channels (got depth %d, %d + %d); use fgnn_mlp_bwd",
diff --git a/graph_neural_net_amd/engine.py b/graph_neural_net_amd/engine.py
--- a/graph_neural_net_amd/engine.py
+++ b/graph_neural_net_amd/engine.py
@@ -138,6 +138,7 @@
     PAIR_BWD = os.environ.get('FGNN_PAIR_BWD', '1') != '0'
     PACK_IN_STRUCT = os.environ.get('FGNN_PACK_IN_STRUCT', '1') != '0'
     T16 = os.environ.get('FGNN_T16', 'pair,bwd')
+    DZ_HANDOVER = os.environ.get('FGNN_DZ_HANDOVER', '1') != '0'
 
     MFMA = os.environ.get('FGNN_MFMA', 'f32')
 
@@ -366,11 +367,16 @@
                   tag='mlp_bwd[cin=%d,dx=%d]' % (a.C + (b.C if b is not None else 0),
                                                 (a.C if dxa is not None else 0) + (b.C if (b is not None and dxb is not None) else 0)))
 
-    def _mlp_bwd_pair(self, params, k, sin, din, emit):
+    def _dz_handover(self, cin, dxs):
+        return (self.DZ_HANDOVER and dxs is None and self._t16_pair(cin)
+                and bool(_lib.load().fgnn_chan_matmul_bwd_dz_supported(self.N)))
+
+    def _mlp_bwd_pair(self, params, k, sin, din, emit, dz=False):
         W = self._bwd
         a1 = self._mlp_bwd_args(params, k, 1, sin, None, W['dy1'], None, None, None, False, False, False, None)
         a2 = self._mlp_bwd_args(params, k, 2, sin, None, W['dy2'], None, din, None, True, False, emit, None)
         entry = 'fgnn_mlp_bwd_pair_x3' if self.x3 else ('fgnn_mlp_bwd_pair_t16' if self._t16_pair(sin.C) else 'fgnn_mlp_bwd_pair')
+        a1.dy_is_dz = a2.dy_is_dz = int(dz)
         _lib.call(entry, C.byref(a1), C.byref(a2), _lib.stream_ptr(),
                   tag='mlp_bwd_pair[cin=%d,dx=%d]' % (sin.C, sin.C if din is not None else 0))
 
@@ -445,14 +451,15 @@
                 dy = din
                 continue
             ya, yb = self._slab_z(k, 1, params), self._slab_z(k, 2, params)
-            _lib.call('fgnn_chan_matmul_bwd_ord', C.byref(ya), C.byref(yb), _lib.ptr(W['dmult']), gs, self.ldp,
+            dz = self._dz_handover(sin.C, dxs)
+            _lib.call('fgnn_chan_matmul_bwd_dz_ord' if dz else 'fgnn_chan_matmul_bwd_ord', C.byref(ya), C.byref(yb), _lib.ptr(W['dmult']), gs, self.ldp,
                       self._nv(), self.G, self.N, _lib.ptr(W['dy1']), _lib.ptr(W['dy2']), gs, self.ldp,
                       _lib.ptr(W['s12'][(k, 1)]), _lib.ptr(W['s12'][(k, 2)]),
                       _lib.ptr(self.mm_order) if self.mm_order is not None else None, self._fill(), st, tag='fgnn_chan_matmul_bwd')
             if first:
                 W['struct_rows'] = 0
             if self.PAIR_BWD and dxs is None and L.depth == 3 and sin.C in (2, 32):
-                self._mlp_bwd_pair(params, k, sin, din, emit=not first)
+                self._mlp_bwd_pair(params, k, sin, din, emit=not first, dz=dz)
             else:
                 self._mlp_bwd(params, k, 1, sin, None, W['dy1'], None, din, None, True, False, dx_strides=dxs)
                 self._mlp_bwd(params, k, 2, sin, None, W['dy2'], None, din, None, True, False, emit=not first, dx_strides=dxs)
diff --git a/include/fgnn_hip.h b/include/fgnn_hip.h
--- a/include/fgnn_hip.h
+++ b/include/fgnn_hip.h
@@ -232,6 +232,7 @@
     const float *xdeg;
     const int *ranges;
     int cu_share;
+    int dy_is_dz;
 } fgnn_mlp_bwd_args;
 int fgnn_mlp_bwd(const fgnn_mlp_bwd_args *args, void *stream);
 int fgnn_mlp_bwd_x3(const fgnn_mlp_bwd_args *args, void *stream);
@@ -264,6 +265,10 @@
 int fgnn_chan_matmul_bwd_ord(const fgnn_slab *ya, const fgnn_slab *yb, const float *dm, long long dmgstride, long long ldm,
                              const int *nvalid, int G, int N, float *da, float *db, long long ogstride, long long ldo,
                              float *s12a, float *s12b, const int *order, int fill , void *stream);
+int fgnn_chan_matmul_bwd_dz_supported(int N);
+int fgnn_chan_matmul_bwd_dz_ord(const fgnn_slab *ya, const fgnn_slab *yb, const float *dm, long long dmgstride, long long ldm,
+                                const int *nvalid, int G, int N, float *dza, float *dzb, long long ogstride, long long ldo,
+                                float *s12a, float *s12b, const int *order, int fill, void *stream);
 
 int fgnn_adam_step(float *params, const float *grads, float *exp_avg, float *exp_avg_sq, int n, double lr,
                    double beta1, double beta2, double eps, int step, double grad_scale, void *stream);
```

Result: no change. 42620, median of 6 (+0.5%).
